# lgalke/aae-recommender

Measured on AMD Instinct MI355X. Metric: train docs/sec at |items|=100k h=200, higher is better.
Workload: dtype f32; 1 GPU; C3 PubMed-scale synthetic Bags: |items|=100000, hidden=200, code=50, fp32, batch=100 docs/GPU/step, full partial_fit (ae+disc+gen, 4 Adam) inside the AdversarialAutoEncoder.fit epoch loop (permutation batches of a corpus resident in HBM); n_items=100000, n_hidden=200, n_code=50, batch_per_gpu=100, global_batch=100, cond_inc=0, rng=device, parallelism=dp1

## Files before the change

### aae-recommender_amd/aaerec/_hip.py

```python
import ctypes as C
import itertools
import weakref
import os

import numpy as np
import torch

_HERE = os.path.dirname(os.path.abspath(__file__))
LIB_PATH = os.environ.get("AAE_HIP_LIB") or os.path.join(_HERE, "libaaerec_hip.so")

ABI_VERSION = 4
ACTIVATIONS = {"ReLU": 0, "SELU": 1, "Tanh": 2, "Sigmoid": 3, "ELU": 4, "LeakyReLU": 5,
               "Softplus": 6, "Hardtanh": 7, "ReLU6": 8, "CELU": 9, "Softsign": 10, "Hardsigmoid": 11, "LogSigmoid": 12,
               "Softshrink": 13, "Hardshrink": 14, "Identity": 15, "GELU": 16, "SiLU": 17, "Mish": 18, "Hardswish": 19}
FINALS = {"linear": 0, "softmax": 1, "sigmoid": 2}
OPTIMIZERS = {"adam": 0, "sgd": 1}
PRIORS = {"gauss": 0, "categorical": 1, "bernoulli": 2}
RNG_INJECT, RNG_DEVICE = 0, 1
RANK_K_MAX = 1024
COOC_TILE = 16384
SPGEMM_HASH_PRODUCTS = 4096
SPGEMM_STAGE = 512
SPTRANS_LDS = 4096
LOWRANK_DIMS_MAX = 4096
# ... 5 lines not shown
GRAD_FUSED, GRAD_EXPORT = 0, 1


class _NullCtx:
    def __enter__(self):
        return None

    def __exit__(self, *a):
        return False


_NULL_CTX = _NullCtx()

T_ENC_W1T, T_ENC_B1, T_ENC_W2, T_ENC_W3, T_DEC_V1, T_DEC_V2, T_DEC_V3, T_DISC_D1, T_DISC_D2, T_DISC_D3 = range(10)
T_ADAM_ENC, T_ADAM_GEN, T_ADAM_DEC, T_ADAM_DISC, T_GRAD = 16, 32, 48, 64, 80
T_ACT_Z, T_ACT_LOSSES, T_ACT_A1, T_ACT_DZC, T_ACT_DH2, T_ACT_DA2 = 96, 97, 98, 99, 100, 101
T_ACT_GA1 = 102
CAT_SUM, CAT_MEAN = 0, 1
CAT_SPARSE_ADAM, CAT_ADAM = 0, 1
O_ENC, O_DEC, O_GEN, O_DISC = 0, 1, 2, 3
MODEL_AAE, MODEL_AE, MODEL_VAE = 0, 1, 3
DTYPE_F32, DTYPE_BF16 = 0, 1


class AaeConfig(C.Structure):
    _fields_ = [("abi_version", C.c_int32), ("n_items", C.c_int32), ("n_hidden", C.c_int32),
                ("n_code", C.c_int32), ("cond_inc", C.c_int32), ("max_batch", C.c_int32),
                ("max_nnz", C.c_int32), ("activation", C.c_int32), ("enc_final", C.c_int32),
                ("optimizer", C.c_int32), ("normalize_inputs", C.c_int32), ("rng_mode", C.c_int32),
                ("prior", C.c_int32), ("grad_mode", C.c_int32), ("dropout1", C.c_float),
                ("dropout2", C.c_float), ("gen_lr", C.c_float), ("reg_lr", C.c_float),
                ("prior_scale", C.c_float), ("has_prior_scale", C.c_int32), ("seed", C.c_uint64),
                ("unfused_decoder", C.c_int32), ("dp_world", C.c_int32), ("model_kind", C.c_int32),
                ("dtype", C.c_int32), ("blocked_output", C.c_int32), ("dense_noise", C.c_int32),
                ("reserved", C.c_int32 * 2)]


class AaeBatch(C.Structure):
    _fields_ = [("indptr_dev", C.c_void_p), ("indices_dev", C.c_void_p), ("values_dev", C.c_void_p),
                ("rows_dev", C.c_void_p), ("row_start", C.c_int32), ("n_rows", C.c_int32),
                ("nnz_bound", C.c_int32), ("max_row_nnz", C.c_int32), ("generation", C.c_int64)]


class AaeRngInject(C.Structure):
    _fields_ = [("masks_dev", C.c_void_p * 12), ("z_real_dev", C.c_void_p)]


_COLL_AG = C.CFUNCTYPE(C.c_int, C.c_void_p, C.c_void_p, C.c_void_p, C.c_int64, C.c_void_p)
_COLL_AR = C.CFUNCTYPE(C.c_int, C.c_void_p, C.c_void_p, C.c_int64, C.c_void_p)


class AaeCollectives(C.Structure):
    _fields_ = [("ctx", C.c_void_p), ("all_gather", _COLL_AG), ("reduce_scatter", _COLL_AG), ("all_reduce", _COLL_AR),
                ("world", C.c_int32), ("rank", C.c_int32)]


class AaeTensor(C.Structure):
    _fields_ = [("byte_offset", C.c_size_t), ("rows", C.c_int64), ("cols", C.c_int64), ("ld", C.c_int64)]


class AaeCooc(C.Structure):
    _fields_ = [("indptr_dev", C.c_void_p), ("indices_dev", C.c_void_p), ("values_dev", C.c_void_p), ("n_rows", C.c_int32)]


class AaePopular(C.Structure):
    _fields_ = [("counts_dev", C.c_void_p), ("order_dev", C.c_void_p), ("pos_dev", C.c_void_p), ("n_items", C.c_int32)]


class AaeMetricSpec(C.Structure):
    _fields_ = [("kind", C.c_int32), ("k", C.c_int32)]


class AaeRankRows(C.Structure):
    _fields_ = [("indptr_dev", C.c_void_p), ("ranks_dev", C.c_void_p), ("n_rows", C.c_int32)]


class AaeLowRank(C.Structure):
    _fields_ = [("vt_dev", C.c_void_p), ("ld", C.c_int64), ("n_features", C.c_int32), ("dims", C.c_int32)]


_PROTOS = {
    "aae_abi_version": (C.c_int, []),
    "aae_set_option": (C.c_int, [C.c_char_p, C.c_char_p]),
    "aae_last_error": (C.c_char_p, []),
    "aae_arena_bytes": (C.c_int, [C.POINTER(AaeConfig), C.POINTER(C.c_size_t)]),
    "aae_create": (C.c_int, [C.POINTER(AaeConfig), C.c_void_p, C.c_size_t, C.c_void_p, C.POINTER(C.c_void_p)]),
    "aae_destroy": (C.c_int, [C.c_void_p]),
    "aae_tensor_info": (C.c_int, [C.c_void_p, C.c_int, C.POINTER(AaeTensor)]),
    "aae_set_lr": (C.c_int, [C.c_void_p, C.c_double, C.c_double]),
    "aae_params_changed": (C.c_int, [C.c_void_p]),
    "aae_set_rng_rows": (C.c_int, [C.c_void_p, C.c_int64, C.c_int64]),
    "aae_sync": (C.c_int, [C.c_void_p, C.c_void_p]),
    "aae_load_linear": (C.c_int, [C.c_void_p, C.c_int, C.c_int, C.c_void_p, C.c_void_p]),
    "aae_store_linear": (C.c_int, [C.c_void_p, C.c_int, C.c_int, C.c_void_p, C.c_void_p]),
    "aae_load_adam": (C.c_int, [C.c_void_p, C.c_int, C.c_int, C.c_void_p, C.c_void_p, C.c_void_p, C.c_void_p, C.c_int64]),
    "aae_store_adam": (C.c_int, [C.c_void_p, C.c_int, C.c_int, C.c_void_p, C.c_void_p, C.c_void_p, C.c_void_p, C.POINTER(C.c_int64)]),
    "aae_step": (C.c_int, [C.c_void_p, C.POINTER(AaeBatch), C.c_void_p, C.POINTER(AaeRngInject), C.c_void_p]),
    "aae_ae_encode": (C.c_int, [C.c_void_p, C.POINTER(AaeBatch), C.POINTER(AaeRngInject), C.c_void_p, C.c_void_p]),
    "aae_ae_decode_backward": (C.c_int, [C.c_void_p, C.c_void_p, C.c_int64, C.POINTER(AaeRngInject), C.c_void_p, C.c_void_p]),
    "aae_vae_step": (C.c_int, [C.c_void_p, C.POINTER(AaeBatch), C.c_void_p, C.c_void_p, C.c_void_p]),
    "aae_vae_predict": (C.c_int, [C.c_void_p, C.POINTER(AaeBatch), C.c_void_p, C.c_void_p, C.c_void_p, C.c_int64,
                                  C.c_void_p]),
    "aae_vae_encode": (C.c_int, [C.c_void_p, C.POINTER(AaeBatch), C.c_void_p, C.c_void_p, C.c_int32, C.c_void_p]),
    "aae_vae_decode_backward": (C.c_int, [C.c_void_p, C.c_void_p, C.c_int64, C.c_void_p, C.c_void_p]),
    "aae_vae_encoder_backward": (C.c_int, [C.c_void_p, C.c_void_p, C.c_int64, C.c_void_p]),
    "aae_decoder_step": (C.c_int, [C.c_void_p, C.POINTER(AaeBatch), C.c_void_p, C.c_int64, C.POINTER(AaeRngInject),
                                   C.c_void_p, C.c_void_p]),
    "aae_ae_encoder_backward": (C.c_int, [C.c_void_p, C.c_void_p, C.c_int64, C.c_void_p]),
    "aae_disc_gen": (C.c_int, [C.c_void_p, C.POINTER(AaeRngInject), C.c_void_p]),
    "aae_disc_step": (C.c_int, [C.c_void_p, C.POINTER(AaeRngInject), C.c_void_p]),
    "aae_gen_step": (C.c_int, [C.c_void_p, C.POINTER(AaeRngInject), C.c_void_p]),
    "aae_read_losses": (C.c_int, [C.c_void_p, C.POINTER(C.c_float * 3), C.c_void_p]),
    "aae_predict": (C.c_int, [C.c_void_p, C.POINTER(AaeBatch), C.c_void_p, C.c_void_p, C.c_int64, C.c_void_p]),
    "aae_predict_topk": (C.c_int, [C.c_void_p, C.POINTER(AaeBatch), C.c_void_p, C.c_int32, C.c_int32, C.c_void_p, C.c_void_p, C.c_void_p]),
    "aae_rank_max_rows": (C.c_int, [C.c_void_p, C.c_int32, C.POINTER(C.c_int32)]),
    "aae_rank_long_stats": (C.c_int, [C.c_void_p, C.POINTER(C.c_int64)]),
    "aae_predict_ranks": (C.c_int, [C.c_void_p, C.POINTER(AaeBatch), C.c_void_p, C.POINTER(AaeBatch), C.c_int32, C.c_void_p, C.c_void_p]),
    "aae_decode_ranks": (C.c_int, [C.c_void_p, C.c_void_p, C.c_int64, C.POINTER(AaeBatch), C.POINTER(AaeBatch), C.c_int32, C.c_void_p,
                                   C.c_void_p]),
    "aae_rank_full_max_rows": (C.c_int, [C.c_void_p, C.POINTER(C.c_int32)]),
    "aae_decode_topk": (C.c_int, [C.c_void_p, C.c_void_p, C.c_int64, C.POINTER(AaeBatch), C.c_int32, C.c_int32, C.c_void_p,
                                  C.c_void_p, C.c_void_p]),
    "aae_vae_predict_topk": (C.c_int, [C.c_void_p, C.POINTER(AaeBatch), C.c_void_p, C.c_void_p, C.c_int32, C.c_int32, C.c_void_p,
                                       C.c_void_p, C.c_void_p]),
    "aae_vae_predict_ranks": (C.c_int, [C.c_void_p, C.POINTER(AaeBatch), C.c_void_p, C.c_void_p, C.POINTER(AaeBatch), C.c_int32,
                                        C.c_void_p, C.c_void_p]),
    "aae_vae_decode_topk": (C.c_int, [C.c_void_p, C.c_void_p, C.c_int64, C.POINTER(AaeBatch), C.c_int32, C.c_int32, C.c_void_p,
                                      C.c_void_p, C.c_void_p]),
    "aae_vae_decode_ranks": (C.c_int, [C.c_void_p, C.c_void_p, C.c_int64, C.POINTER(AaeBatch), C.POINTER(AaeBatch), C.c_int32,
                                       C.c_void_p, C.c_void_p]),
    "aae_vae_rank_max_rows": (C.c_int, [C.c_void_p, C.c_int32, C.POINTER(C.c_int32)]),
    "aae_vae_rank_full_max_rows": (C.c_int, [C.c_void_p, C.POINTER(C.c_int32)]),
    "aae_encode": (C.c_int, [C.c_void_p, C.POINTER(AaeBatch), C.c_void_p, C.c_void_p]),
    "aae_decode": (C.c_int, [C.c_void_p, C.c_void_p, C.c_int64, C.c_int32, C.c_void_p, C.c_int64, C.c_void_p]),
    "aae_apply_updates": (C.c_int, [C.c_void_p, C.c_int, C.c_void_p]),
    "aae_apply_updates_except": (C.c_int, [C.c_void_p, C.c_int, C.c_int, C.c_void_p]),
    "aae_apply_shard": (C.c_int, [C.c_void_p, C.c_int, C.c_int64, C.c_int64, C.c_void_p, C.c_int, C.c_void_p]),
    "aae_w1_export": (C.c_int, [C.c_void_p, C.c_void_p, C.c_void_p, C.c_int32, C.c_void_p]),
    "aae_w1_packet_floats": (C.c_int, [C.c_void_p, C.c_int32, C.POINTER(C.c_int64), C.POINTER(C.c_int64)]),
    "aae_w1_import": (C.c_int, [C.c_void_p, C.c_void_p, C.c_void_p, C.c_int32, C.c_int32, C.c_int64, C.c_int, C.c_void_p]),
    "aae_set_grad_scale": (C.c_int, [C.c_void_p, C.c_float]),
    "aae_ae_forward": (C.c_int, [C.c_void_p, C.POINTER(AaeBatch), C.c_void_p, C.POINTER(AaeRngInject), C.c_void_p]),
    "aae_output_layer_step": (C.c_int, [C.c_void_p, C.POINTER(AaeBatch), C.c_void_p]),
    "aae_ae_backward": (C.c_int, [C.c_void_p, C.c_void_p, C.c_int64, C.c_void_p]),
    "aae_set_doc_l1": (C.c_int, [C.c_void_p, C.c_void_p]),
    "aae_set_first_layer_external": (C.c_int, [C.c_void_p, C.c_int]),
    "aae_first_layer_forward": (C.c_int, [C.c_void_p, C.POINTER(AaeBatch), C.c_void_p, C.c_void_p]),
    "aae_first_layer_update": (C.c_int, [C.c_void_p, C.c_void_p, C.c_int64, C.c_int32, C.c_int64, C.c_int, C.c_void_p]),
    "aae_apply_gathered": (C.c_int, [C.c_void_p, C.c_int, C.c_int, C.c_void_p, C.c_int64, C.c_int32, C.c_int64, C.c_void_p]),
    "aae_cat_encode": (C.c_int, [C.c_void_p, C.c_int32, C.c_int32, C.c_void_p, C.c_int32, C.c_int32, C.c_int32, C.c_void_p,
                                 C.c_int64, C.c_void_p]),
    "aae_cat_update": (C.c_int, [C.c_void_p, C.c_void_p, C.c_void_p, C.c_void_p, C.c_int32, C.c_int32, C.c_void_p, C.c_int32,
                                 C.c_int32, C.c_int32, C.c_void_p, C.c_int64, C.c_int32, C.c_double, C.c_int64, C.c_void_p]),
    "aae_csr_embed": (C.c_int, [C.c_void_p, C.c_void_p, C.c_void_p, C.c_int32, C.c_void_p, C.c_int32, C.c_int32, C.c_int64,
                                C.c_void_p, C.c_int64, C.c_void_p]),
    "aae_cooc_scores": (C.c_int, [C.POINTER(AaeCooc), C.c_int32, C.POINTER(AaeBatch), C.c_void_p, C.c_int64, C.c_void_p]),
    "aae_cooc_topk": (C.c_int, [C.POINTER(AaeCooc), C.c_int32, C.POINTER(AaeBatch), C.c_int32, C.c_int32, C.c_void_p, C.c_int64,
                                C.c_void_p, C.c_void_p, C.c_void_p]),
    "aae_cooc_ranks": (C.c_int, [C.POINTER(AaeCooc), C.c_int32, C.POINTER(AaeBatch), C.POINTER(AaeBatch), C.c_int32, C.c_void_p,
                                 C.c_int64, C.c_void_p, C.c_void_p]),
    "aae_cooc_scores_i32": (C.c_int, [C.POINTER(AaeCooc), C.c_int32, C.POINTER(AaeBatch), C.c_void_p, C.c_int64, C.c_void_p]),
    "aae_cooc_topk_i32": (C.c_int, [C.POINTER(AaeCooc), C.c_int32, C.POINTER(AaeBatch), C.c_int32, C.c_int32, C.c_void_p, C.c_int64,
                                    C.c_void_p, C.c_void_p, C.c_void_p]),
    "aae_cooc_ranks_i32": (C.c_int, [C.POINTER(AaeCooc), C.c_int32, C.POINTER(AaeBatch), C.POINTER(AaeBatch), C.c_int32, C.c_void_p,
                                     C.c_int64, C.c_void_p, C.c_void_p]),
    "aae_spgemm_i32_bound": (C.c_int, [C.POINTER(AaeCooc), C.POINTER(AaeCooc), C.c_int32, C.c_void_p, C.c_void_p]),
# ... 1149 lines not shown
                                             C.byref(inj) if inj else None, _ptr(dz), self._stream()))
        return dz

    def vae_step(self, csr, row_start, n_rows, rows=None, cond=None, eps=None):
        b = self._batch(csr, row_start, n_rows, rows)
        keep = []
        if cond is not None:
            cond = upload(cond, self.device, torch.float32).contiguous(); keep.append(cond)
        if eps is not None:
            eps = torch.as_tensor(eps, dtype=torch.float32).to(self.device).contiguous(); keep.append(eps)
        self._keep = keep
        with self._on_device():
            _check(self.lib.aae_vae_step(self.handle, C.byref(b), _ptr(cond), _ptr(eps), self._stream()))

    def vae_encode(self, csr, row_start, n_rows, rows=None, eps=None, train=True):
        b = self._batch(csr, row_start, n_rows, rows)
        if eps is not None:
            eps = torch.as_tensor(eps, dtype=torch.float32).to(self.device).contiguous()
        z = torch.empty(n_rows, self.c, dtype=torch.float32, device=self.device)
        self._keep = [eps, z]
        with self._on_device():
            _check(self.lib.aae_vae_encode(self.handle, C.byref(b), _ptr(eps), _ptr(z), int(bool(train)), self._stream()))
        return z

    def vae_decode_backward(self, zc):
        zc = zc.detach().to(self.device, torch.float32).contiguous()
        dzc = torch.empty_like(zc)
        self._keep = self._keep + [zc, dzc]
        with self._on_device():
            _check(self.lib.aae_vae_decode_backward(self.handle, _ptr(zc), zc.shape[1], _ptr(dzc), self._stream()))
        return dzc

    def vae_encoder_backward(self, dz):
        dz = dz.detach().to(self.device, torch.float32).contiguous()
        self._keep = self._keep + [dz]
        with self._on_device():
            _check(self.lib.aae_vae_encoder_backward(self.handle, _ptr(dz), dz.shape[1], self._stream()))

    def vae_predict(self, csr, row_start, n_rows, cond=None, eps=None):
        b = self._batch(csr, row_start, n_rows)
        out = self._out_buffer(n_rows)
        if cond is not None:
            cond = upload(cond, self.device, torch.float32).contiguous()
        if eps is not None:
            eps = torch.as_tensor(eps, dtype=torch.float32).to(self.device).contiguous()
        with self._on_device():
            _check(self.lib.aae_vae_predict(self.handle, C.byref(b), _ptr(cond), _ptr(eps), _ptr(out), out.shape[1],
                                            self._stream()))
        return out[:, :self.N]

    def ae_encoder_backward(self, dz):
        dz = dz.detach().to(self.device, torch.float32).contiguous()
        self._keep.append(dz)
        with self._on_device():
            _check(self.lib.aae_ae_encoder_backward(self.handle, _ptr(dz), dz.shape[1], self._stream()))

    def disc_gen(self):
        with self._on_device():
            _check(self.lib.aae_disc_gen(self.handle, None, self._stream()))

    def disc_step(self):
        with self._on_device():
            _check(self.lib.aae_disc_step(self.handle, None, self._stream()))

    def gen_step(self):
        with self._on_device():
            _check(self.lib.aae_gen_step(self.handle, None, self._stream()))

    def apply_updates(self, which, skip=-1):
        with self._on_device():
            _check(self.lib.aae_apply_updates_except(self.handle, which, skip, self._stream()))

    def apply_shard(self, tid, row_begin, row_end, grad_shard, which):
        self._keep.append(grad_shard)
        with self._on_device():
            _check(self.lib.aae_apply_shard(self.handle, tid, row_begin, row_end, C.c_void_p(grad_shard.data_ptr()),
                                            which, self._stream()))

    big_tensor_id = T_DEC_V3

    def big_grad(self):
        return T_DEC_V3, self.tensor(T_GRAD + T_DEC_V3, padded=True), self.tensor(T_DEC_V3, padded=True)

    def _w1_layout(self, cap):
        if self._w1_packet is None:
            hw, tot = C.c_int64(), C.c_int64()
            _check(self.lib.aae_w1_packet_floats(self.handle, self.w1_cap, C.byref(hw), C.byref(tot)))
            assert hw.value == self._w1_hdr
            self._w1_small = tot.value - hw.value - self.w1_cap * self.h
            self._w1_packet = torch.zeros(tot.value, dtype=torch.float32, device=self.device)
        cap = self.w1_cap if cap is None else max(1, min(int(cap), self.w1_cap))
        hdr = (1 + cap + 3) & ~3
        return cap, hdr, hdr + cap * self.h + self._w1_small

    def w1_export(self, cap=None):
        cap, hdr, total = self._w1_layout(cap)
        pk = self._w1_packet[:total]
        with self._on_device():
            _check(self.lib.aae_w1_export(self.handle, C.c_void_p(pk.data_ptr()), C.c_void_p(pk.data_ptr() + 4 * hdr), cap,
                                          self._stream()))
        return pk

    def w1_import(self, packets, n_peers, which, cap=None, stride_floats=None):
        cap, hdr, total = self._w1_layout(cap)
        stride = total if stride_floats is None else int(stride_floats)
        assert stride >= total and packets.numel() >= (n_peers - 1) * stride + total
        self._keep.append(packets)
        with self._on_device():
            _check(self.lib.aae_w1_import(self.handle, C.c_void_p(packets.data_ptr()),
                                          C.c_void_p(packets.data_ptr() + 4 * hdr), cap, n_peers, 4 * stride, which,
                                          self._stream()))

    def set_rng_rows(self, row_offset, global_rows):
        _check(self.lib.aae_set_rng_rows(self.handle, int(row_offset), int(global_rows)))

    def set_grad_scale(self, scale):
        _check(self.lib.aae_set_grad_scale(self.handle, float(scale)))

    def profile_enable(self, on=True, kernels=None):
        if on and kernels is not None:
            on = sum(1 << (k + 1) for k in kernels)
        _check(self.lib.aae_profile_enable(self.handle, int(on)))

    def profile_read(self, kernel_id):
        ms, n = C.c_double(), C.c_int64()
        _check(self.lib.aae_profile_read(self.handle, kernel_id, C.byref(ms), C.byref(n)))
        return ms.value, n.value

    def losses(self):
        out = (C.c_float * 3)()
        with self._on_device():
            _check(self.lib.aae_read_losses(self.handle, C.byref(out), self._stream()))
        return float(out[0]), float(out[1]), float(out[2])

    def _out_buffer(self, n_rows):
        ld = (self.N + 3) & ~3
        return torch.empty(n_rows, ld, dtype=torch.float32, device=self.device)

    def predict(self, csr, row_start, n_rows, cond=None):
        b = self._batch(csr, row_start, n_rows)
        out = self._out_buffer(n_rows)
        if cond is not None:
            cond = upload(cond, self.device, torch.float32).contiguous()
        with self._on_device():
            _check(self.lib.aae_predict(self.handle, C.byref(b), _ptr(cond), _ptr(out), out.shape[1], self._stream()))
        return out[:, :self.N]

    def rank_max_rows(self, k=10):
        return self._max_rows(int(k), self.lib.aae_rank_max_rows, int(k))

    def _max_rows(self, key, entry, *args):
        if key not in self._rank_rows:
            out = C.c_int32()
            _check(entry(self.handle, *args, C.byref(out)))
            self._rank_rows[key] = int(out.value)
        return self._rank_rows[key]

    def rank_long_stats(self):
        out = (C.c_int64 * 5)()
        _check(self.lib.aae_rank_long_stats(self.handle, out))
        return dict(zip(("calls", "rows", "overflow_rows", "entries", "max_entries"), (int(v) for v in out)))

    def predict_topk(self, csr, row_start, n_rows, k, cond=None, exclude_known=True):
        return self._topk(self.lib.aae_predict_topk, csr, row_start, n_rows, k, exclude_known, (self._cond_rows(cond),))

    def _cond_rows(self, cond):
# ... 93 lines not shown
```

### aae-recommender_amd/csrc/aae_abi.hip

```cpp
#include <hip/hip_runtime.h>
#include <hip/hip_ext.h>
#include <math.h>
#include <stdio.h>
#include <stdlib.h>
#include <string.h>

#include <algorithm>
#include <string>
#include <vector>

#include "../../include/aaerec_hip.h"
#include "gemm_f32.h"
#include "kernels.h"
#include "dec_fused.h"
#include "dec_fused_bf16.h"
#include "dec_crit_x3.h"
#include "rank_x3.h"
#include "rank_long.h"
#include "rank_full.h"
#include "cooc.h"
#include "spgemm.h"
#include "sptrans.h"
#include "mutinfo.h"
#include "popular.h"
#include "rank_metrics.h"
#include "lowrank.h"
#include "chain.h"
#include "chain4.h"
#include "chain16x3.h"
#include "cond_embed.h"
#include "w1_update.h"
#include "dae_corrupt.h"

using namespace aae;

#include "kernel_pick.h"

#include <map>
static std::map<std::string, std::string> g_options;
const char* option_value(const char* name) {
    auto it = g_options.find(name);
    if (it != g_options.end()) return it->second.c_str();
    return getenv((std::string("AAE_") + name).c_str());
}

#include "abi_model.h"
#include "abi_layers.h"
#include "abi_chains.h"
#include "abi_rank.h"

extern "C" {

int aae_abi_version(void) { return AAE_ABI_VERSION; }

int aae_set_option(const char* name, const char* value) {
    if (!name || !*name) return fail(AAE_EINVAL, "option name is empty");
    static const char* known[] = {"NO_CHAIN", "CHAIN16", "SPLIT_ANY", "BLOCKED_ANY", "EARLY_ANY", "NO_LATE_JOIN", "NO_ITEM_COUNT", "W1_SERIAL",
                                  "NO_RANK_FUSED", "CHAIN_KSLICES", "X16_ROWS", "DW_KSPLIT_ROWS", "DEC_TS", "CHAIN_TS", "DW_TS", "DEC_SKIP", "CHAIN_SKIP", "RANK_SKIP",
                                  "RANK_COLLECT_CAP"};
    bool ok = false;
    for (const char* k : known) ok = ok || strcmp(k, name) == 0;
    if (!ok) return fail(AAE_EINVAL, "unknown option (aae_options, csrc/abi_model.h, lists them)");
    if (value && strcmp(name, "RANK_COLLECT_CAP") == 0) {
        char* end = nullptr;
        const long v = strtol(value, &end, 10);
        if (end == value || *end || v < 1 || v > kLongCap) return fail(AAE_EINVAL, "RANK_COLLECT_CAP must be a whole number in [1, 4096]");
    }
    if (value) g_options[name] = value; else g_options.erase(name);
    return AAE_OK;
}
const char* aae_last_error(void) { return g_err.c_str(); }

int aae_arena_bytes(const aae_config* cfg, size_t* bytes_out) {
    TRY(validate(cfg));
    if (!bytes_out) return fail(AAE_EINVAL, "bytes_out is NULL");
    aae_model tmp; memset((void*)&tmp, 0, sizeof(tmp)); tmp.cfg = *cfg;
    read_options(tmp.opt);
    *bytes_out = layout(&tmp, nullptr, true);
    return AAE_OK;
}

int aae_create(const aae_config* cfg, void* arena_dev, size_t arena_bytes, void* stream, aae_handle* out) {
    TRY(validate(cfg));
    if (!arena_dev || !out) return fail(AAE_EINVAL, "arena/out is NULL");
    if (reinterpret_cast<uintptr_t>(arena_dev) & 255) return fail(AAE_EINVAL, "arena must be 256-byte aligned");
    aae_model* m = new aae_model();
    memset((void*)m, 0, sizeof(*m));
    m->cfg = *cfg;
    read_options(m->opt);
    size_t need = layout(m, static_cast<char*>(arena_dev), false);
    if (need > arena_bytes) { delete m; return fail(AAE_ENOMEM, "arena smaller than aae_arena_bytes()"); }
    m->base = static_cast<char*>(arena_dev); m->bytes = need;
    m->alpha_mode = cfg->activation == AAE_ACT_SELU;
    m->vae = cfg->model_kind == 3; m->vae_bwd = false; m->vae_cut = false;
    m->bf16 = cfg->dtype == 1;
    m->blocked_ok = cfg->blocked_output == 1;
    m->blocked_any = m->opt.blocked_any;
    m->split_any = m->opt.split_any;
    m->x3_gemm = !m->bf16;
    m->noise_next = nullptr; m->noise_ld = 0; m->dense_step = false; m->noise_gen_next = false; m->noise_gen_scale = 0.f;
    m->ae_only = cfg->model_kind == 1 || m->vae;
    m->lazy = true;
    auto limit = [](bool& ok, size_t bytes) { return [&ok, bytes](auto kernel) { ok = ok && raise_lds_limit(kernel, bytes); }; };
    const int maxlds = 160 * 1024;
    {
        int dev = 0, cus = 0;
        if (hipGetDevice(&dev) != hipSuccess ||
            hipDeviceGetAttribute(&cus, hipDeviceAttributeMultiprocessorCount, dev) != hipSuccess || cus < 1) {
            delete m; return fail(AAE_EHIP, "no HIP device");
        }
        m->n_cu = std::min(cus, 304);
        const int nb = (m->h + 1 + 15) / 16;
        m->fused_nb = nb <= 4 ? 4 : nb <= 7 ? 7 : nb <= 13 ? 13 : 0;
        m->fused_ok = m->fused_nb != 0 && fused_width_ok(m->h, m->ldh);
        m->use_chain = (m->h + 1 <= 208) && (m->c + 1 <= 208) && (m->cp + 1 <= (cfg->model_kind == 3 ? 208 : 2 * 208)) &&
                       !m->opt.no_chain;
        const size_t chain_lds = kCSlots * kCR * kCL * sizeof(float);
        if (m->use_chain) each_chain(false, limit(m->use_chain, chain_lds));
        m->act_nm = cfg->activation > AAE_ACT_LEAKYRELU;
        if (m->use_chain && m->act_nm) each_chain(true, limit(m->use_chain, chain_lds));
        m->use_chain4 = m->use_chain && !m->act_nm && !m->opt.chain16;
        if (m->use_chain4) each_chain4(limit(m->use_chain4, chain_lds));
        if (m->use_chain && m->cp + 1 > 208 && !m->use_chain4) m->use_chain = false;
        m->x16_rows = m->opt.x16_rows;
        m->dw_ksplit_rows = 256;
        if (m->opt.dw_ksplit_rows >= 0) m->dw_ksplit_rows = m->opt.dw_ksplit_rows;
        if (!m->opt.no_item_count) {
            void* hp = nullptr; void* dp = nullptr;
            if (hipHostMalloc(&hp, 64, hipHostMallocMapped) == hipSuccess && hipHostGetDevicePointer(&dp, hp, 0) == hipSuccess) {
                m->cnt_host = static_cast<int*>(hp); m->cnt_host_dev = static_cast<int*>(dp); *m->cnt_host = 0;
            } else { if (hp) (void)hipHostFree(hp); (void)hipGetLastError(); }
        }
        m->x16_ok = m->use_chain4 && m->FXi[P_W2] != nullptr;
        if (m->x16_ok) each_chain16x3(limit(m->x16_ok, kX16Lds));
        m->force_unfused = cfg->unfused_decoder == 1;
        if (m->fused_ok) {
            each_dec_fused(kDecFused, limit(m->fused_ok, maxlds));
            if (m->bf16) each_dec_fused_bf16(kDecFused, limit(m->fused_ok, maxlds));
            if (!raise_lds_limit(tile_bucket_kernel, maxlds - 2048)) m->fused_ok = false;
            m->bucket_wide_ok = raise_lds_limit(tile_bucket_wide_kernel, maxlds - 16384);
            {
                hipFuncAttributes fa;
                static bool told = false;
                if (m->bucket_wide_ok && !told && hipFuncGetAttributes(&fa, reinterpret_cast<const void*>(tile_bucket_wide_kernel)) == hipSuccess && fa.numRegs < 121) {
                    told = true;
                    fprintf(stderr, "aaerec: tile_bucket_wide_kernel allocates %d vector registers, not the 128 it claims to keep its CU to itself (buckets.h)\n", fa.numRegs);
                }
                (void)hipGetLastError();
            }
        }
    }
    m->late_enabled = !m->opt.no_late_join;
    m->early_enabled = true;
    m->early_any = m->opt.early_any;
    m->rank_ok = m->fused_ok && m->use_chain4 && !m->vae && !m->opt.no_rank_fused;
    m->vae_rank_ok = m->vae && m->fused_ok && m->use_chain4 && !m->opt.no_rank_fused;
    if (m->vae_rank_ok) each_chain4_vae(limit(m->vae_rank_ok, kCSlots * kCR * kCL * sizeof(float)));
    bool& rank_ok = m->vae ? m->vae_rank_ok : m->rank_ok;
    if (rank_ok) each_rank_x3([&](RankKernel k, int nb) { rank_ok = rank_ok && raise_lds_limit(k, rank_x3_lds_bytes(nb)); });
    if (rank_ok) each_rank_x3v2([&](RankKernel k, int nb) { rank_ok = rank_ok && raise_lds_limit(k, rank_x3v2_lds_bytes(nb)); });
    m->w1_big_lds = raise_lds_limit(w1_item_update_kernel, sizeof(int) * w1_items_lds_words(16384));
    (void)hipGetLastError();
    m->grad_scale = 1.f;
    m->rng_row0 = 0; m->rng_global = 0;
    m->Gt = m->G.p;
    m->split_ok = false; m->opt_pending = false; m->side = nullptr; m->ev_crit = m->ev_opt = nullptr;
    m->split_wgs = std::max(1, (m->n_cu * 5) / 8);
    m->pf_armed = m->pf_built = m->pf_pending = false; m->pf_step = -1; m->hstep = 0; m->flushed_hstep = -1; m->ev_head = m->ev_pf = nullptr;
    bool side_ok = false;
    if (cfg->grad_mode == AAE_GRAD_FUSED) {
        int lo = 0, hi = 0;
        const unsigned evflags = hipEventDisableTiming | hipEventDisableSystemFence;
        side_ok = hipDeviceGetStreamPriorityRange(&lo, &hi) == hipSuccess &&
                  hipStreamCreateWithPriority(&m->side, hipStreamNonBlocking, lo) == hipSuccess &&
                  hipEventCreateWithFlags(&m->ev_crit, evflags) == hipSuccess &&
                  hipEventCreateWithFlags(&m->ev_opt, evflags) == hipSuccess &&
                  hipEventCreateWithFlags(&m->ev_head, evflags) == hipSuccess &&
                  hipEventCreateWithFlags(&m->ev_pf, evflags) == hipSuccess &&
                  hipEventCreateWithFlags(&m->ev_bk, evflags) == hipSuccess &&
                  hipEventCreateWithFlags(&m->ev_end, evflags) == hipSuccess;
        if (!side_ok) {
            if (m->side) (void)hipStreamDestroy(m->side);
            m->side = nullptr;
        }
        (void)hipGetLastError();
    }
    if (side_ok && m->fused_ok && m->bf16 && m->split_wgs > 0 &&
        (size_t)((m->N + kBU - 1) / kBU) * kBU * bf_stride(4) <= (size_t)m->R * m->ldn) {
        m->split_ok = true;
        for (int mode : {kDecCrit, kDecOpt}) each_dec_fused_bf16(mode, limit(m->split_ok, maxlds));
        (void)hipGetLastError();
    }
    if (side_ok && m->fused_ok && m->split_wgs > 0 && 
        (size_t)((m->N + kTI - 1) / kTI) * kTI * (size_t)std::min(m->R, 16 * kMB) * sizeof(float) < (size_t)0x7FFFFFF0u) {
        bool ok = true;
        for (int mode : {kDecCrit, kDecOpt, kDecOptAcc}) each_dec_fused(mode, limit(ok, maxlds));
        each_dec_opt_blocks(limit(ok, maxlds));
        if (!m->bf16) m->split_ok = ok;
        m->x3_ok = ok;
        each_dec_crit_x3(false, limit(m->x3_ok, maxlds));
        each_dec_opt_blocks_x3(limit(m->x3_ok, maxlds));
        each_dec_opt_x3(false, limit(m->x3_ok, maxlds));
        (void)hipGetLastError();
        if (m->bf16) {
            m->bf16_x3 = m->x3_ok && ok;
            if (!m->bf16_x3) m->x3_ok = false;
            else m->split_ok = true;
            m->bf16_one = m->bf16_x3;
            each_dec_crit_x3(true, limit(m->bf16_one, maxlds));
            each_dec_opt_x3(true, limit(m->bf16_one, maxlds));
            (void)hipGetLastError();
        }
        if (m->x3_ok) {
            const int ntiles = (m->N + 31) / 32;
            const double t_tile = (2.2 + 0.0096 * m->h) * (m->bf16_one ? 0.98 : 1.0);
            int w = (int)(ntiles * t_tile / (m->bf16_one ? 127.0 : 57.0) / 8.0 + 0.5) * 8;
            w = std::max(w, std::min(ntiles, m->bf16_one ? 40 : 64));
            const int cap = m->late_enabled ? m->n_cu * 7 / 16 : m->n_cu * 9 / 16;
            m->split_wgs = std::max(1, std::min(w, cap));
        }
    }
    hipStream_t s = S(stream);
    hipError_t e = hipMemsetAsync(arena_dev, 0, need, s);
    if (e != hipSuccess) { delete m; return fail(AAE_EHIP, std::string("hipMemsetAsync: ") + hipGetErrorString(e)); }
    struct { Ten* t; int col; } ones[] = {{&m->eh1, m->h}, {&m->eh2, m->h}, {&m->zc, m->cp}, {&m->dh1, m->h},
                                           {&m->dh2, m->h}, {&m->zin, m->c}, {&m->xh1, m->h}, {&m->xh2, m->h}};
    for (auto& o : ones)
        hipLaunchKernelGGL(fill_col_kernel, dim3(((int)o.t->rows + 255) / 256), dim3(256), 0, s, o.t->p, (int)o.t->ld,
                           (int)o.t->rows, o.col, 1.0f);
    OptScalars hs[4]; memset(hs, 0, sizeof(hs));
    for (int i = 0; i < 4; ++i) {
        hs[i].t = 0; hs[i].is_sgd = cfg->optimizer == AAE_OPT_SGD;
        hs[i].lr = (i == O_ENC || i == O_DEC) ? (double)cfg->gen_lr : (double)cfg->reg_lr;
        hs[i].neg_step_size = 0.f; hs[i].bc2_sqrt = 1.f; hs[i].inv_bc2_sqrt = 1.f;
    }
    e = hipMemcpyAsync(m->sc, hs, sizeof(hs), hipMemcpyHostToDevice, s);
    if (e == hipSuccess) e = hipStreamSynchronize(s);
    if (e != hipSuccess) { delete m; return fail(AAE_EHIP, std::string("init: ") + hipGetErrorString(e)); }
    *out = m;
    return AAE_OK;
}

#ifdef W1_TS
int aae_debug_w1_ts(unsigned long long* out, int n) {
    return (int)hipMemcpyFromSymbol(out, HIP_SYMBOL(aae::w1_ts), sizeof(unsigned long long) * (size_t)n);
}
#endif
int aae_destroy(aae_handle h) {
    if (!h) return AAE_OK;
    if (h->side) {
        (void)hipStreamSynchronize(h->side);
        (void)hipStreamDestroy(h->side);
    }
    if (h->dp_scratch) (void)hipFree(h->dp_scratch);
    if (h->cnt_host) (void)hipHostFree(h->cnt_host);
    for (hipEvent_t e : {h->ev_crit, h->ev_opt, h->ev_head, h->ev_pf, h->ev_bk, h->ev_end}) if (e) (void)hipEventDestroy(e);
    if (h->prof_ev) {
        for (int k = 0; k < AAE_K_N; ++k)
            for (auto& pr : h->prof_ev[k]) { (void)hipEventDestroy(pr.first); (void)hipEventDestroy(pr.second); }
        delete[] h->prof_ev;
    }
    delete h;
    return AAE_OK;
}


int aae_profile_enable(aae_handle h, int on) {
    if (!h) return fail(AAE_EINVAL, "handle is NULL");
    if (on && !h->prof_ev) h->prof_ev = new std::vector<std::pair<hipEvent_t, hipEvent_t>>[AAE_K_N];
    h->prof_on = on != 0;
    h->prof_mask = on == 1 ? ~0u : ((unsigned)on >> 1);
    return AAE_OK;
}

int aae_profile_read(aae_handle h, int kernel_id, double* total_ms, int64_t* launches) {
    if (!h || !total_ms || !launches) return fail(AAE_EINVAL, "NULL argument");
    if (kernel_id < 0 || kernel_id >= AAE_K_N) return fail(AAE_EINVAL, "bad kernel id");
    *total_ms = 0.0; *launches = 0;
    if (!h->prof_ev) return AAE_OK;
    auto& v = h->prof_ev[kernel_id];
    for (size_t i = 0; i < h->prof_used[kernel_id]; ++i) {
        HIPCHK(hipEventSynchronize(v[i].second));
        float ms = 0.f;
        HIPCHK(hipEventElapsedTime(&ms, v[i].first, v[i].second));
        *total_ms += ms; *launches += 1;
    }
    h->prof_used[kernel_id] = 0;
    return AAE_OK;
}

int aae_prefetch_batch(aae_handle h, const aae_batch* next) {
    if (!h || !next) return fail(AAE_EINVAL, "NULL argument");
    if (!next->indptr_dev || !next->indices_dev || !next->values_dev) return fail(AAE_EINVAL, "batch pointers are NULL");
    if (next->n_rows < 1 || next->n_rows > h->R) return fail(AAE_EINVAL, "batch n_rows outside [1, max_batch]");
    if (next->nnz_bound > h->cfg.max_nnz) return fail(AAE_EINVAL, "batch nnz_bound > max_nnz");
    if (next->generation == 0) { h->pf_armed = false; return AAE_OK; }
    h->pf_batch = *next;
    h->pf_armed = true;
    return AAE_OK;
}

int aae_set_input_noise(aae_handle h, const float* noise_dev, int64_t noise_ld) {
    if (!h) return fail(AAE_EINVAL, "handle is NULL");
    if (!h->Xn.p) return fail(AAE_ESTATE, "aae_set_input_noise: the model was not created with cfg.dense_noise = 1");
    if (noise_dev && noise_ld < h->N) return fail(AAE_EINVAL, "noise_ld < n_items");
    h->noise_next = noise_dev; h->noise_ld = noise_ld;
    h->noise_gen_next = false;
    return AAE_OK;
}

int aae_join_output_layer(aae_handle h, void* stream) {
    if (!h) return fail(AAE_EINVAL, "handle is NULL");
    if (h->opt_pending) {
        HIPCHK(hipStreamWaitEvent(S(stream), h->ev_opt, 0));
        h->opt_pending = false;
        if (!h->pf_after_opt) h->pf_pending = false;
    }
    return AAE_OK;
}

int aae_join(aae_handle h, void* stream) {
    if (!h) return fail(AAE_EINVAL, "handle is NULL");
    return join_deferred(h, S(stream));
}

int aae_set_split(aae_handle h, int32_t workgroups) {
    if (!h) return fail(AAE_EINVAL, "handle is NULL");
    if (workgroups < 0) return fail(AAE_EINVAL, "workgroups must be >= 0");
    if (h->opt_pending) return fail(AAE_ESTATE, "aae_set_split with a deferred launch pending: call aae_join / aae_sync first");
    h->split_wgs = workgroups;
// ... 90 lines not shown
```

### aae-recommender_amd/csrc/abi_chains.h

```cpp
#pragma once

namespace {

ChainOp cop(int kind, int src, int dst, int N) {
    ChainOp o; memset(&o, 0, sizeof(o));
    o.kind = kind; o.src = src; o.dst = dst; o.N = N; o.one_col = -1; o.scale = 1.f; o.yslot = 0; o.fake_slot = -1;
    return o;
}
ChainOp cop_load(const float* g, int ld, int dst, int N, int row0 = 0) {
    ChainOp o = cop(COP_LOAD, 0, dst, N); o.W = g; o.ldw = ld; o.out_row0 = row0; return o;
}
ChainOp cop_linear(int kind, int src, int dst, const Ten& W, int K, int N, int epi) {
    ChainOp o = cop(kind, src, dst, N); o.W = W.p; o.ldw = (int)W.ld; o.K = K; o.epi = epi;
    if (kind == COP_LINEAR_DX) { o.Wkn = W.p; o.ldkn = (int)W.ld; }
    return o;
}
void cop_out(ChainOp& o, float* out, int ld, int row0 = 0) { o.out = out; o.ldo = ld; o.out_row0 = row0; }

W4Copies w4_of(const aae_model* m, int pid) {
    return W4Copies{m->PT[pid].p, m->D4[pid].p, (int)m->P[pid].rows, (int)m->P[pid].cols, m->FXi[pid], m->DXi[pid], m->FXBi[pid], kCWide};
}
float* ga1_ptr(const aae_model* m) {
    return (m->ext_first && m->ga1x.p) ? m->ga1x.p + (size_t)(m->R - m->rows) * m->ldh : m->gb3.p;
}
// ... 281 lines not shown
            } else
            if (!no_wave && m->rows > 16 * kMB && m->hot_list && (int64_t)m->N >= 40ll * m->rows) {
                w.wave_form = 1;
                w.nitem = (w.nitem + 3) / 4;
                const int set = m->hot_flip; m->hot_flip ^= 1;
                w.hot = m->hot_list + (size_t)set * m->hot_cap; w.hot_count = m->hot_count + set; w.hot_zero = m->hot_count + (set ^ 1);
                m->w1_hot_pending = true; m->w1_hot_set = set; m->w1_hot_which = which; m->w1_hot_ga1 = ga1;
                mh = m;
            }
            w.cnt_out = nullptr;
            constexpr bool hyb_count = true;
            if ((w.wave_form != 2 || hyb_count) && m->cnt_host) {
                w.cnt_out = m->cnt_host_dev;
                const int seen = *reinterpret_cast<volatile int*>(m->cnt_host);
                if (seen > 0) {
                    const int per = w.wave_form ? 4 : 1;
                    int want = ((seen + seen / 4 + per - 1) / per + 63) & ~63;
                    if (w.wave_form == 2) want = std::max(want, (int)((std::min<int64_t>(m->cfg.max_nnz, m->N) + 2047) / 2048));
                    w.nitem = std::min(w.nitem, std::max(256, want));
                }
            }
        }
        return AAE_OK;
    }
    void add_loss(aae_model* m, int n, int slot) { g.loss.enabled = 1; g.loss.terms = m->adv_terms; g.loss.n = n; g.loss.out = m->losses + slot; }
    int launch(hipStream_t s, hipEvent_t done = nullptr, bool* marked = nullptr) {
        int blocks = tiles;
        if (g.w1.enabled) { g.w1.blk0 = tiles; blocks += g.w1.ncol + g.w1.nitem; }
        if (g.loss.enabled) blocks += 1;
        if (marked) *marked = done && !mh;
        g.ksplit = ksplit_rows;
        const int ts_from = dw_ts;
        static int ts_seen = 0;
        static unsigned long long* ts_dev = nullptr;
        constexpr int kTsCap = 1 << 16;
        const bool ts_now = ts_from >= 0 && ts_seen >= ts_from && ts_seen < ts_from + 6;
        if (ts_from >= 0) {
            ++ts_seen;
            if (!ts_dev) HIPCHK(hipMalloc(&ts_dev, sizeof(unsigned long long) * 2 * kTsCap));
        }
        if (ts_now) { HIPCHK(hipMemsetAsync(ts_dev, 0, sizeof(unsigned long long) * 2 * kTsCap, s)); g.ts = ts_dev; g.ts_cap = kTsCap; }
        if (done && !mh) hipExtLaunchKernelGGL(grouped_dw_kernel, dim3(blocks), dim3(256), 0, s, nullptr, done, 0, g);
        else
        hipLaunchKernelGGL(grouped_dw_kernel, dim3(blocks), dim3(256), 0, s, g);
        LAUNCHCHK("grouped_dw_kernel");
        if (ts_now) {
            HIPCHK(hipStreamSynchronize(s));
            const int nb = std::min(blocks, kTsCap);
            std::vector<unsigned long long> h(2 * (size_t)nb);
            HIPCHK(hipMemcpy(h.data(), ts_dev, sizeof(unsigned long long) * 2 * nb, hipMemcpyDeviceToHost));
            unsigned long long t_lo = ~0ull, t_hi = 0;
            for (int b = 0; b < nb; ++b) if (h[2 * b]) { t_lo = std::min(t_lo, h[2 * b]); t_hi = std::max(t_hi, h[2 * b + 1]); }
            const int ncol = g.w1.enabled ? g.w1.ncol : 0, nitem = g.w1.enabled ? g.w1.nitem : 0;
            int max_rows = 0;
            for (int q = 0; q < g.njobs; ++q) max_rows = std::max(max_rows, g.jobs[q].rows);
            fprintf(stderr, "[grouped_dw launch %d: %d workgroups = %d tiles (rows %d) + %d column-sum + %d item (form %d) + %d loss; first start -> last end %.2f us]\n",
                    ts_seen - 1, blocks, tiles, max_rows, ncol, nitem, g.w1.wave_form, g.loss.enabled, (t_hi - t_lo) * 0.01);
            const struct { const char* name; int lo, hi; } kinds[] = {{"tiles", 0, tiles}, {"column sums", tiles, tiles + ncol}, {"items", tiles + ncol, tiles + ncol + nitem}};
            for (const auto& k : kinds) {
                if (k.hi <= k.lo) continue;
                unsigned long long first = ~0ull, last = 0, worst = 0; int worst_b = -1, busy = 0; double sum = 0;
                for (int b = k.lo; b < std::min(k.hi, nb); ++b) {
                    if (!h[2 * b]) continue;
                    const unsigned long long d = h[2 * b + 1] - h[2 * b];
                    first = std::min(first, h[2 * b]); last = std::max(last, h[2 * b + 1]);
                    if (d > worst) { worst = d; worst_b = b - k.lo; }
                    if (d > 150) ++busy;
                    sum += d * 0.01;
                }
                fprintf(stderr, "   %-12s start %.2f us after the launch's first, end %.2f; longest workgroup %.2f us (#%d); %d of %d ran longer than 1.5 us, mean %.2f us\n",
                        k.name, (first - t_lo) * 0.01, (last - t_lo) * 0.01, worst * 0.01, worst_b, busy, k.hi - k.lo, sum / std::max(1, k.hi - k.lo));
            }
        }
        if (mh) TRY(launch_w1_hot(mh, s));
        return AAE_OK;
    }
};

int launch_w1_hot(aae_model* m, hipStream_t s) {
    if (!m->w1_hot_pending) return AAE_OK;
    m->w1_hot_pending = false;
    W1Items a = w1_items_args(m, m->w1_hot_ga1, 0, 0, m->w1_hot_which);
    a.ulist = m->hot_list + (size_t)m->w1_hot_set * m->hot_cap; a.ucount = m->hot_count + m->w1_hot_set;
    const size_t lds = sizeof(int) * w1_items_lds_words(m->rows);
    hipLaunchKernelGGL(w1_item_update_kernel, dim3(std::min(m->hot_cap, 256)), dim3(256), lds, s, a);
    LAUNCHCHK("w1_item_update (hot list)");
    return AAE_OK;
}

void chain_encoder_tail(aae_model* m, ChainBuilder& cb, bool train, const uint8_t* mk2, uint32_t sid2, int rows,
                        float* eh2_out, hipStream_t s, const uint8_t* mk1 = nullptr, uint32_t sid1 = 0) {
    const int h = m->h;
    if (m->ext_first) {
        cb.add(cop_load(m->a1.p, m->ldh, 3, h));
        ChainOp& e1 = cb.add(cop(COP_DROPACT, 3, 0, h));
        e1.d = make_drop(m, 0, train, mk1, nullptr, rows, h, sid1); e1.one_col = h; cop_out(e1, m->eh1.p, m->ldh);
    } else {
        ChainOp& l = cb.add(cop_load(m->eh1.p, m->ldh, 0, h)); l.one_col = h;
    }
    ChainOp& a = cb.add(cop_fwd(m, P_W2, 0, 1, h + 1, h, CEPI_DROPACT, s));
    a.d = make_drop(m, 1, train, mk2, nullptr, rows, h, sid2); a.one_col = h;
    if (eh2_out) cop_out(a, eh2_out, m->ldh);
    cb.add(cop_fwd(m, P_W3, 1, 2, h + 1, m->c, CEPI_NONE, s));
}

static int row_blocks(const aae_model* m) { return m->rows <= 16 * kMB ? 1 : (m->rows + kRowBlock - 1) / kRowBlock; }
static size_t fused_span_limit(const aae_model* m) {
    const int bits = out_bf16(m) ? 31 : 32;
    return ((size_t)1 << bits) - ((size_t)1 << 24);
}
static bool fused_decoder_applies(const aae_model* m) {
    const bool one = m->rows <= 16 * kMB;
    const bool bf_blocks_ok = !m->bf16 || (m->x3_ok && m->dh2f.p && true);
    const bool blocked = !one && m->blocked_ok && !out_bf16(m) && bf_blocks_ok && m->split_ok && m->split_wgs > 0 && m->Gacc.p && row_blocks(m) <= kMaxRowBlocks &&
                         m->cfg.grad_mode == AAE_GRAD_FUSED &&
                         (m->blocked_any || (size_t)m->rows * m->N <= ((size_t)32 << 20) || (m->x3_ok && m->dh2f.p));
    return m->fused_ok && !m->force_unfused && (one || blocked) &&
           ((size_t)m->N + 2 * kTI) * m->ldh * sizeof(float) < fused_span_limit(m) &&
           ((size_t)m->N + 2 * kTI) * (size_t)((m->rows + row_blocks(m) - 1) / row_blocks(m)) * sizeof(float) < ((size_t)1 << 31) &&
           (m->bf16 ? dec_fused_bf16_lds_bytes(m->fused_nb) : dec_fused_lds_bytes((m->rows + row_blocks(m) - 1) / row_blocks(m), m->h)) <= 160 * 1024;
}
static void flip_bucket_set(aae_model* m) {
    std::swap(m->tstart, m->tstart2); std::swap(m->teb, m->teb2); std::swap(m->ten, m->ten2); std::swap(m->tev, m->tev2);
}
int build_tile_buckets(aae_model* m, hipStream_t s) {
    const int ntiles = (m->N + kTI - 1) / kTI, B = m->rows;
    flip_bucket_set(m);
    const size_t lds1 = sizeof(int) * ((size_t)ntiles + 1 + kBucketMaxDocs + 1 + 1024);
    if (ntiles <= kBucketMaxTiles && B <= kBucketMaxDocs && (m->fused_ok || lds1 <= 48 * 1024)) {
        hipLaunchKernelGGL(tile_bucket_kernel, dim3(1), dim3(1024), lds1, s, m->bv, ntiles, m->tstart, m->teb, m->ten, m->tev);
    } else if (ntiles <= kBucketMaxTiles && B <= kBucketWideDocs && m->bucket_wide_ok) {
        size_t lds = sizeof(int) * ((size_t)ntiles + 1 + kBucketWideDocs + 1 + 1024);
        constexpr bool bk_claim = true;
        if (bk_claim) lds = std::max(lds, (size_t)(160 * 1024 - 16384));
        hipLaunchKernelGGL(tile_bucket_wide_kernel, dim3(1), dim3(1024), lds, s, m->bv, ntiles, m->tstart, m->teb, m->ten, m->tev);
    } else {
        const int gy = std::max(1, std::min(16, m->chunks / 16 + 1));
        hipLaunchKernelGGL(zero_int_kernel, dim3(std::min(64, ntiles / 256 + 1)), dim3(256), 0, s, m->tcount, ntiles + 1);
        hipLaunchKernelGGL(tile_hist_kernel, dim3(B, gy), dim3(256), 0, s, m->bv, m->tcount);
        hipLaunchKernelGGL(tile_scan_kernel, dim3(1), dim3(1024), 0, s, m->tcount, m->tstart, ntiles);
        hipLaunchKernelGGL(tile_fill_kernel, dim3(B, gy), dim3(256), 0, s, m->bv, m->tstart, m->tcount, m->teb, m->ten, m->tev);
    }
    LAUNCHCHK("tile buckets");
    m->buckets_valid = true;
    return AAE_OK;
}
int ensure_buckets(aae_model* m, hipStream_t s) {
    if (m->bk_pending) {
        HIPCHK(hipStreamWaitEvent(s, m->ev_bk, 0));
        m->bk_pending = false;
    }
    if (!m->buckets_valid) TRY(build_tile_buckets(m, s));
    return AAE_OK;
}

W1Items w1_items_args(aae_model* m, const float* ga1, int rpb, size_t bstride, int which) {
    const int set = (which == O_GEN) ? 1 : 0;
    W1Items a;
    a.ulist = m->ulist; a.ucount = m->ucount;
    a.tstart = m->tstart; a.eb = m->teb; a.en = m->ten; a.ev = m->tev;
    a.ga1 = ga1; a.ld = m->ldh; a.rpb = rpb; a.bstride = bstride;
    a.rscale = m->rscale; a.rows = m->rows; a.h = m->h;
    a.W = m->P[P_W1T].p; a.M = m->M[set][P_W1T].p; a.V = m->V[set][P_W1T].p; a.ldw = m->ldw1;
    a.gout = m->cfg.grad_mode == AAE_GRAD_EXPORT ? m->Gr[P_W1T].p : nullptr;
    a.sc = m->sc + which; a.tsync = m->tsync; a.step_ctr = m->step_ctr;
    a.mark_synced = (which == O_GEN || m->ae_only) ? 1 : 0;
    return a;
}
int launch_w1_items(aae_model* m, const float* ga1, int rpb, size_t bstride, int which, hipStream_t s) {
    TRY(ensure_buckets(m, s));
    const W1Items a = w1_items_args(m, ga1, rpb, bstride, which);
    const size_t lds = sizeof(int) * w1_items_lds_words(m->rows);
    if (lds > 64 * 1024 && !m->w1_big_lds) return fail(AAE_ESTATE, "first-layer update: batch too large for the LDS row lists");
    ProfScope ps(m, AAE_K_ENC_W1_ADAM, s);
    const int items = std::max(1, std::min(std::min(m->cfg.max_nnz, std::max(256, m->rows * 32)), m->N));
    hipLaunchKernelGGL(w1_item_update_kernel, dim3(items), dim3(256), lds, s, a);
    LAUNCHCHK("w1_item_update");
    return AAE_OK;
}

static void piggyback_buckets(aae_model* m, ChainBuilder& cb) {
    const int ntiles = (m->N + kTI - 1) / kTI;
    const size_t need = sizeof(int) * ((size_t)ntiles + 1 + kBucketMaxDocs + 1 + 1024);
    if (m->x16_ok && m->rows >= m->x16_rows) return;
    if (m->buckets_valid || !fused_decoder_applies(m) || ntiles > kBucketMaxTiles || m->rows > kBucketMaxDocs ||
        need > (size_t)kCSlots * kCR * kCL * sizeof(float))
        return;
    flip_bucket_set(m);
    BucketJob& b = cb.P.bk;
    b.bv = m->bv; b.ntiles = ntiles; b.tstart = m->tstart; b.eb = m->teb; b.en = m->ten; b.ev = m->tev; b.enabled = 1;
    m->buckets_valid = true;
}

int chain_ae_forward(aae_model* m, bool with_dec, const float* cond_dev, float* z_out, hipStream_t s) {
    const int B = m->rows, h = m->h, c = m->c, cp = m->cp;
    const aae_rng_inject& I = m->inj;
    ChainBuilder cb(m, B);
    piggyback_buckets(m, cb);
    chain_encoder_tail(m, cb, true, I.masks_dev[1], 1, B, m->eh2.p, s, I.masks_dev[0], 0);
    ChainOp& f = m->cfg.enc_final == AAE_FINAL_LINEAR ? cb.P.ops[cb.P.nops - 1] : cb.add(cop(COP_FINAL_FWD, 2, 2, c));
    f.aux = m->cfg.enc_final;
    cop_out(f, m->zc.p, m->ldc); f.out2 = m->zsave.p; f.ldo2 = m->ldz;
    if (z_out) { ChainOp& st = cb.add(cop(COP_STORE, 2, 2, c)); cop_out(st, z_out, c); }
    if (with_dec) {
        if (wide_dec_in(m)) {
            const int nA = kCWide - c, ci = m->cfg.cond_inc;
            ChainOp& ca = cb.add(cop_load(cond_dev, ci, 2, nA)); ca.dst_col0 = c;
            ChainOp& cl = cb.add(cop_load(cond_dev + nA, ci, 5, ci - nA)); cl.one_col = cp - kCWide;
        } else if (m->cfg.cond_inc > 0) {
            ChainOp& cl = cb.add(cop_load(cond_dev, m->cfg.cond_inc, 2, m->cfg.cond_inc)); cl.dst_col0 = c; cl.one_col = cp;
        } else {
            f.one_col = cp;
        }
        ChainOp& v1 = add_dec_in_fwd(cb, m, 2, 5, 3, s);
        v1.d = make_drop(m, 0, true, I.masks_dev[2], nullptr, B, h, 2); v1.one_col = h; cop_out(v1, m->dh1.p, m->ldh);
        ChainOp& v2 = cb.add(cop_fwd(m, P_V2, 3, 4, h + 1, h, CEPI_DROPACT, s));
        v2.d = make_drop(m, 1, true, I.masks_dev[3], nullptr, B, h, 3); v2.one_col = h; cop_out(v2, m->dh2.p, m->ldh);
    }
    m->dec_hidden_done = with_dec;
    return launch_chain(m, cb, s);
}

int chain_dec_hidden(aae_model* m, bool train, int rows, hipStream_t s) {
    const int h = m->h, cp = m->cp;
    const aae_rng_inject& I = m->inj;
    ChainBuilder cb(m, rows);
    if (wide_dec_in(m)) {
        cb.add(cop_load(m->zc.p, m->ldc, 0, kCWide));
        ChainOp& lb = cb.add(cop_load(m->zc.p + kCWide, m->ldc, 3, cp - kCWide)); lb.one_col = cp - kCWide;
    } else {
        ChainOp& l = cb.add(cop_load(m->zc.p, m->ldc, 0, cp)); l.one_col = cp;
    }
    ChainOp& v1 = add_dec_in_fwd(cb, m, 0, 3, 1, s);
    v1.d = make_drop(m, 0, train, I.masks_dev[2], nullptr, rows, h, 2); v1.one_col = h; cop_out(v1, m->dh1.p, m->ldh);
    ChainOp& v2 = cb.add(cop_fwd(m, P_V2, 1, 2, h + 1, h, CEPI_DROPACT, s));
    v2.d = make_drop(m, 1, train, I.masks_dev[3], nullptr, rows, h, 3); v2.one_col = h; cop_out(v2, m->dh2.p, m->ldh);
    return launch_chain(m, cb, s);
}

int chain_ae_backward(aae_model* m, bool dec_part, bool enc_part, const float* part_slabs, size_t slab_stride,
                      const float* gz_ext, int ld_gz, float* dzc_out, int which, hipStream_t s, int nslab = 16) {
    const int B = m->rows, h = m->h, c = m->c, cp = m->cp;
    const aae_rng_inject& I = m->inj;
    ChainBuilder cb(m, B);
    if (dec_part) {
        if (part_slabs) {
            ChainOp& ss = cb.add(cop(COP_SLABSUM, 0, 2, h)); ss.W = part_slabs; ss.ldw = m->ldh; ss.aux = nslab; ss.stride = slab_stride;
            ss.epi = CEPI_ACTBWD; ss.aux_ptr = m->dh2.p; ss.aux_ld = m->ldh;
            ss.d = make_drop(m, 1, true, I.masks_dev[3], nullptr, B, h, 3); cop_out(ss, m->gb0.p, m->ldh);
        } else {
            cb.add(cop_load(m->gb0.p, m->ldh, 2, h));
        }
        if (y_needs_load(m)) cb.add(cop_load(m->dh1.p, m->ldh, 3, h));
        ChainOp& x2 = cb.add(cop_dx(m, P_V2, 2, 4, h, h, CEPI_ACTBWD, s)); set_y(cb, m, x2, m->dh1.p, m->ldh, 3);
        x2.d = make_drop(m, 0, true, I.masks_dev[2], nullptr, B, h, 2); cop_out(x2, m->gb1.p, m->ldh);
        add_dec_in_dx(cb, m, 4, 5, 3, dzc_out, s);
    }
    if (enc_part) {
        if (!dec_part || gz_ext) cb.add(cop_load(gz_ext ? gz_ext : m->gzc.p, gz_ext ? ld_gz : m->ldc, 5, c));
        int sg = 7;
        ChainOp* prod = (dec_part && !gz_ext && cb.P.nops) ? &cb.P.ops[cb.P.nops - 1] : nullptr;
        if (m->cfg.enc_final == AAE_FINAL_LINEAR && prod && cp == c && !prod->out2) {
            prod->out2 = m->ga3.p; prod->ldo2 = m->ldz; sg = 5;
        } else {
            if (m->cfg.enc_final != AAE_FINAL_LINEAR) cb.add(cop_load(m->zsave.p, m->ldz, 6, c));
            ChainOp& fb = cb.add(cop(COP_FINAL_BWD, 5, 7, c)); fb.yslot = 6; fb.aux = m->cfg.enc_final;
            cop_out(fb, m->ga3.p, m->ldz);
        }
        if (y_needs_load(m)) cb.add(cop_load(m->eh2.p, m->ldh, 8, h));
        ChainOp& x3 = cb.add(cop_dx(m, P_W3, sg, 9, c, h, CEPI_ACTBWD, s)); set_y(cb, m, x3, m->eh2.p, m->ldh, 8);
        x3.d = make_drop(m, 1, true, I.masks_dev[which == O_GEN ? 9 : 1], nullptr, B, h, which == O_GEN ? 9 : 1);
        cop_out(x3, m->gb2.p, m->ldh);
        if (y_needs_load(m)) cb.add(cop_load(m->eh1.p, m->ldh, 0, h));
        ChainOp& x2 = cb.add(cop_dx(m, P_W2, 9, 1, h, h, CEPI_ACTBWD, s)); set_y(cb, m, x2, m->eh1.p, m->ldh, 0);
// ... 287 lines not shown
```

### aae-recommender_amd/csrc/abi_model.h

```cpp
#pragma once

static thread_local std::string g_err;
static int fail(int code, const std::string& msg) { g_err = msg; return code; }

#define HIPCHK(expr)                                                                        \
    do {                                                                                    \
        hipError_t e_ = (expr);                                                             \
        if (e_ != hipSuccess)                                                               \
            return fail(AAE_EHIP, std::string(#expr) + ": " + hipGetErrorString(e_));       \
    } while (0)
#define LAUNCHCHK(what)                                                                     \
    do {                                                                                    \
        hipError_t e_ = hipGetLastError();                                                  \
        if (e_ != hipSuccess) return fail(AAE_EHIP, std::string(what) + ": " + hipGetErrorString(e_)); \
    } while (0)
#define TRY(expr) do { int rc_ = (expr); if (rc_ != AAE_OK) return rc_; } while (0)

namespace {

inline int r4(int x) { return (x + 3) & ~3; }

struct Ten {
    float* p = nullptr; size_t off = 0; int64_t rows = 0, cols = 0, ld = 0;
    size_t floats() const { return (size_t)rows * ld; }
};

enum { P_W1T = 0, P_B1, P_W2, P_W3, P_V1, P_V2, P_V3, P_D1, P_D2, P_D3, NP };
enum { O_ENC = 0, O_DEC = 1, O_GEN = 2, O_DISC = 3 };

}

struct aae_options {
    bool no_chain;
    bool chain16;
    bool split_any;
    bool blocked_any;
    bool early_any;
    bool no_late_join;
    bool no_item_count;
    bool w1_serial;
    bool no_rank_fused;
    bool chain_kslices;
    int x16_rows;
    int rank_collect_cap;
    int dw_ksplit_rows;
    char dec_ts[8];
    bool chain_ts;
    int dw_ts;
    int dec_skip, chain_skip, rank_skip;
};
const char* option_value(const char* name);
inline void read_options(aae_options& o) {
    auto on = [](const char* n) { return option_value(n) != nullptr; };
    auto num = [](const char* n, int dflt) { const char* e = option_value(n); return e ? atoi(e) : dflt; };
    o.no_chain = on("NO_CHAIN"); o.chain16 = on("CHAIN16"); o.split_any = on("SPLIT_ANY"); o.blocked_any = on("BLOCKED_ANY");
    o.early_any = on("EARLY_ANY"); o.no_late_join = on("NO_LATE_JOIN"); o.no_item_count = on("NO_ITEM_COUNT");
    o.w1_serial = on("W1_SERIAL"); o.no_rank_fused = on("NO_RANK_FUSED"); o.chain_kslices = on("CHAIN_KSLICES");
    o.x16_rows = num("X16_ROWS", 1024); o.dw_ksplit_rows = num("DW_KSPLIT_ROWS", -1);
    o.rank_collect_cap = std::max(0, std::min(num("RANK_COLLECT_CAP", 0), 4096));
    const char* ts = option_value("DEC_TS");
    snprintf(o.dec_ts, sizeof(o.dec_ts), "%s", ts ? ts : "");
    o.chain_ts = on("CHAIN_TS"); o.dw_ts = num("DW_TS", -1);
    o.dec_skip = num("DEC_SKIP", 0); o.chain_skip = num("CHAIN_SKIP", 0); o.rank_skip = num("RANK_SKIP", 0);
}

struct aae_model {
    aae_config cfg;
    aae_options opt;
    char* base; size_t bytes;
    int N, h, c, cp, R, R2;
    int ldh, ldw1, ldc, ldz, ldn;
    bool alpha_mode;
    float grad_scale;
    int rng_row0, rng_global;
    Ten P[NP], M[2][NP], V[2][NP], Gr[NP];
    unsigned short* FXi[NP]; unsigned short* DXi[NP]; unsigned short* FXBi[NP];
    bool x16_ok; int x16_rows;
    Ten PT[NP]; Ten D4[NP]; bool pt_ok[NP];
    Ten a1, eh1, eh2, zc, dh1, dh2, G, slabs, gb0, gb1, gb2, gb3, gzc, ga3, zin, xh1, xh2, dout, zsave, da2;
    Ten ga1x;
    bool only_output_layer;
    const float* doc_l1;
    bool ext_first;
    bool own_first;
    bool ae_only;
    bool vae;
    bool bf16;
    bool vae_bwd;
    bool vae_cut;
    Ten mulv, gmulv, veps;
    bool use_chain;
    bool use_chain4;
    bool act_nm;
    bool dec_hidden_done;
    bool fuse_enc_bwd;
    bool enc_bwd_done;
    int max_slabs;
    float* bce_partials; int bce_partials_cap;
    float* fix_partials;
    float* rscale;
    bool w1_merged;
    bool w1_items_merged;
    bool buckets_valid;
    bool lazy;
    int n_cu; bool fused_ok; int fused_nb; bool force_unfused;
    int* tcount; int* tstart; int* teb; int* ten; float* tev;
    int* tstart2; int* teb2; int* ten2; float* tev2;
    int* tsync; int* mark; int* ulist; int* ucount; int* stamp; LazyTab* tab;
    int* hot_list = nullptr; int* hot_count = nullptr; int hot_cap = 0, hot_flip = 0;
    bool w1_hot_pending = false; int w1_hot_set = 0, w1_hot_which = 0; const float* w1_hot_ga1 = nullptr;
    int* pslot; int* ptag;
    int chunks;
    float* losses;
    float* adv_terms;
    OptScalars* sc;
    long long* step_ctr;
    BatchView bv; bool have_batch; int rows; int phase;
    aae_rng_inject inj;
    bool prof_on; unsigned prof_mask;
    std::vector<std::pair<hipEvent_t, hipEvent_t>>* prof_ev;
    size_t prof_used[AAE_K_N];
    bool split_ok; int split_wgs; bool opt_pending;
    hipStream_t side; hipEvent_t ev_crit, ev_opt;
    bool bf16_one = false;
    bool bf16_x3 = false;
    float* Gt;
    Ten Xn; const float* noise_next; int64_t noise_ld; bool dense_step;
    bool noise_gen_next; float noise_gen_scale;
    float* noise_l1;
    bool bucket_wide_ok = false;
    bool split_any = false;
    float* dp_scratch = nullptr; size_t dp_scratch_floats = 0;
    bool x3_gemm = false;
    bool x3_ok = false;
    bool w1_big_lds = false;
    bool blocked_any = false;
    Ten dh2f;
    bool blocked_ok; Ten Gacc;
    int* mark2; int* ulist2; int* ucount2; int* stamp2;
    int* cnt_host; int* cnt_host_dev;
    int dw_ksplit_rows;
    aae_batch pf_batch, pf_built_batch; bool pf_armed; bool pf_built; long long pf_step; long long hstep;
    bool pf_pending; hipEvent_t ev_head, ev_pf;
    bool pf_bumped = false;
    bool pf_after_opt = false;
    hipEvent_t ev_bk = nullptr; bool bk_pending = false;
    bool last_out_split = false;
    Ten dh2s; OptScalars* sc_snap = nullptr;
    bool late_enabled = false, late_ok = false;
    hipEvent_t ev_end = nullptr; bool end_marked = false, spec_tab_ok = false, pf_this_step = false, early_enabled = false, early_any = false;
    long long flushed_hstep = -1;
    int64_t long_stats[5] = {0, 0, 0, 0, 0};
    bool rank_ok = false;
    bool vae_rank_ok = false;
    bool side_ordered = false;
};

namespace {

struct Arena {
    char* base; size_t off = 0; bool dry;
    float* take(size_t nfloats, size_t* off_out) {
        off = (off + 255) & ~(size_t)255;
        size_t o = off; off += nfloats * sizeof(float);
        if (off_out) *off_out = o;
        return dry ? nullptr : reinterpret_cast<float*>(base + o);
    }
    Ten mat(int64_t rows, int64_t cols, int64_t ld, int64_t pad_rows = 0) {
        Ten t; t.rows = rows; t.cols = cols; t.ld = ld;
        t.p = take((size_t)(rows + pad_rows) * ld, &t.off);
        return t;
    }
};

constexpr int kRowBlock = 104, kMaxRowBlocks = 16;

inline bool fused_width_ok(int h, int ldh) {
    return (h + 1 + 15) / 16 <= 13 && ldh <= 256 && (ldh % 4) == 0 && ldh <= kSD - 2;
}

int validate(const aae_config* c) {
    if (!c) return fail(AAE_EINVAL, "cfg is NULL");
    if (c->abi_version != AAE_ABI_VERSION) return fail(AAE_EINVAL, "abi_version mismatch");
    if (c->n_items < 1 || c->n_hidden < 1 || c->n_code < 1 || c->cond_inc < 0)
        return fail(AAE_EINVAL, "n_items/n_hidden/n_code must be positive");
    if (c->n_hidden > 4096) return fail(AAE_EINVAL, "n_hidden > 4096 not supported");
    if (c->max_batch < 1 || c->max_nnz < 1) return fail(AAE_EINVAL, "max_batch/max_nnz must be positive");
    if (c->max_batch > 16384) return fail(AAE_EINVAL, "max_batch > 16384 not supported");
    if (c->activation < 0 || c->activation >= AAE_ACT_COUNT) return fail(AAE_EINVAL, "unknown activation");
    if (c->enc_final < 0 || c->enc_final > AAE_FINAL_SIGMOID) return fail(AAE_EINVAL, "unknown enc_final");
// ... 55 lines not shown
        {
            const int64_t M = m->P[pid].rows, Nc = m->P[pid].cols;
            m->PT[pid] = a.mat((Nc + 3) / 4, 4 * M, 4 * M, kW4Pad);
            m->D4[pid] = a.mat((M + 3) / 4, 4 * Nc, 4 * Nc, kW4Pad);
        }
    for (int i = 0; i < NP; ++i) m->FXi[i] = m->DXi[i] = m->FXBi[i] = nullptr;
    if (chain_copies && m->R2 >= m->opt.x16_rows)
        for (int pid : {P_W2, P_W3, P_V1, P_V2, P_D1, P_D2}) {
            const int64_t M = m->P[pid].rows, Nc = m->P[pid].cols, Mp = (M + 15) & ~15, Np = (Nc + 15) & ~15;
            m->FXi[pid] = reinterpret_cast<unsigned short*>(a.take((size_t)(((Nc + 31) / 32) * 3 * Mp * 32 + 1) / 2, nullptr));
            m->DXi[pid] = reinterpret_cast<unsigned short*>(a.take((size_t)(((M + 31) / 32) * 3 * Np * 32 + 1) / 2, nullptr));
            if (Nc > kCWide) m->FXBi[pid] = reinterpret_cast<unsigned short*>(a.take((size_t)(((Nc - kCWide + 31) / 32) * 3 * Mp * 32 + 1) / 2, nullptr));
        }
    const int R = m->R, R2 = m->R2;
    m->a1 = a.mat(R, h, m->ldh);   m->eh1 = a.mat(R, h + 1, m->ldh);  m->eh2 = a.mat(R, h + 1, m->ldh);
    m->zc = a.mat(R, cp + 1, m->ldc);
    m->dh1 = a.mat(R, h + 1, m->ldh); m->dh2 = a.mat(R, h + 1, m->ldh);
    m->G = a.mat(R, N, m->ldn, (32 * (int64_t)R + m->ldn - 1) / m->ldn + 1 + (c.blocked_output ? kMaxRowBlocks : 0));
    {
        int tiles = ((R + 63) / 64) * ((h + 63) / 64);
        m->max_slabs = std::max(1, std::min(128, 2048 / tiles));
        int64_t slab_rows = (int64_t)m->max_slabs * R;
        if (fused_width_ok(h, m->ldh)) slab_rows = std::max(slab_rows, (int64_t)(304 + 16) * std::min(R, 16 * kMB));
        if (fused_width_ok(h, m->ldh) && c.blocked_output && R <= kMaxRowBlocks * kRowBlock) slab_rows = std::max(slab_rows, (int64_t)(304 + 16) * R);
        m->slabs = a.mat(slab_rows, h, m->ldh);
    }
    m->gb0 = a.mat(R2, h + 1, m->ldh); m->gb1 = a.mat(R2, h + 1, m->ldh);
    m->gb2 = a.mat(R2, h + 1, m->ldh); m->gb3 = a.mat(R2, h + 1, m->ldh);
    m->gzc = a.mat(R, cp + 1, m->ldc);
    m->ga3 = a.mat(R2, cc + 1, m->ldz);
    m->zin = a.mat(R2, cc + 1, m->ldz);
    m->xh1 = a.mat(R2, h + 1, m->ldh); m->xh2 = a.mat(R2, h + 1, m->ldh);
    m->dout = a.mat(R2, 1, 4);
    m->zsave = a.mat(R, cc, m->ldz);
    m->da2 = a.mat(R, h + 1, m->ldh);
    m->Xn = Ten();
    if (c.dense_noise == 1) m->Xn = a.mat(R, N, m->ldn);
    m->noise_l1 = c.dense_noise == 1 ? a.take((size_t)R * kDaeChunksMax, nullptr) : nullptr;
    m->Gacc = Ten();
    if (c.blocked_output && c.grad_mode == AAE_GRAD_FUSED && R > 16 * kMB) m->Gacc = a.mat(N, h + 1, m->ldh, 2 * kTI);
    m->dh2f = Ten();
    if (c.blocked_output && c.grad_mode == AAE_GRAD_FUSED && R > 16 * kMB && R <= kMaxRowBlocks * kRowBlock)
        m->dh2f = a.mat((int64_t)((R + kXCH - 1) / kXCH) * 13 * (kXCH / 32) * 3, 256, 256);
    if (c.model_kind == 3) {
        m->mulv = a.mat(R, 2 * cc, r4(2 * cc)); m->gmulv = a.mat(R, 2 * cc, r4(2 * cc)); m->veps = a.mat(R, cc, r4(cc));
    }
    m->bce_partials_cap = std::max(512 * (c.blocked_output ? kMaxRowBlocks : 1), ((N + 31) / 32) * ((R + 31) / 32));
    m->bce_partials = a.take(m->bce_partials_cap, nullptr);
    m->fix_partials = a.take((size_t)R * 64, nullptr);
    m->rscale = a.take(R, nullptr);
    m->tsync = reinterpret_cast<int*>(a.take(N, nullptr));
    m->mark = reinterpret_cast<int*>(a.take(N, nullptr));
    m->ulist = reinterpret_cast<int*>(a.take((size_t)c.max_nnz * (size_t)std::max(1, c.dp_world), nullptr));
    m->pslot = m->ptag = nullptr;
    if (c.grad_mode == AAE_GRAD_EXPORT && c.dp_world > 1) {
        m->pslot = reinterpret_cast<int*>(a.take((size_t)N * c.dp_world, nullptr));
        m->ptag = reinterpret_cast<int*>(a.take((size_t)N * c.dp_world, nullptr));
    }
    m->ucount = reinterpret_cast<int*>(a.take(4, nullptr));
    m->stamp = m->ucount ? m->ucount + 1 : nullptr;
    m->hot_cap = (int)std::max<int64_t>(256, c.max_nnz / kW1WaveRows + 64);
    m->hot_list = reinterpret_cast<int*>(a.take((size_t)2 * m->hot_cap, nullptr));
    m->hot_count = reinterpret_cast<int*>(a.take(4, nullptr));
    m->hot_flip = 0;
    m->mark2 = m->ulist2 = m->ucount2 = m->stamp2 = nullptr;
    if (c.grad_mode == AAE_GRAD_FUSED) {
        m->mark2 = reinterpret_cast<int*>(a.take(N, nullptr));
        m->ulist2 = reinterpret_cast<int*>(a.take((size_t)c.max_nnz, nullptr));
        m->ucount2 = reinterpret_cast<int*>(a.take(4, nullptr));
        m->stamp2 = m->ucount2 ? m->ucount2 + 1 : nullptr;
    }
    m->tab = reinterpret_cast<LazyTab*>(a.take((size_t)kLazyTabCap * 4, nullptr));
    {
        const size_t nt = (size_t)(N + kTI - 1) / kTI + 1;
        m->tcount = reinterpret_cast<int*>(a.take(nt, nullptr));
        m->tstart = reinterpret_cast<int*>(a.take(nt, nullptr));
        m->teb = reinterpret_cast<int*>(a.take((size_t)c.max_nnz, nullptr));
        m->ten = reinterpret_cast<int*>(a.take((size_t)c.max_nnz, nullptr));
        m->tev = a.take((size_t)c.max_nnz, nullptr);
        m->tstart2 = reinterpret_cast<int*>(a.take(nt, nullptr));
        m->teb2 = reinterpret_cast<int*>(a.take((size_t)c.max_nnz, nullptr));
        m->ten2 = reinterpret_cast<int*>(a.take((size_t)c.max_nnz, nullptr));
        m->tev2 = a.take((size_t)c.max_nnz, nullptr);
    }
    m->losses = a.take(4, nullptr);
    m->adv_terms = a.take((size_t)R2, nullptr);
    m->sc = reinterpret_cast<OptScalars*>(a.take(4 * sizeof(OptScalars) / sizeof(float), nullptr));
    m->step_ctr = reinterpret_cast<long long*>(a.take(2, nullptr));
    m->dh2s = Ten(); m->sc_snap = nullptr;
    if (c.grad_mode == AAE_GRAD_FUSED) {
        m->dh2s = a.mat(std::min(R, 16 * kMB), h + 1, m->ldh);
        m->sc_snap = reinterpret_cast<OptScalars*>(a.take((sizeof(OptScalars) + 3) / sizeof(float), nullptr));
    }
    return (a.off + 255) & ~(size_t)255;
}

inline hipStream_t S(void* s) { return reinterpret_cast<hipStream_t>(s); }

struct ProfScope {
    aae_model* m; int k; hipStream_t s; bool on;
    ProfScope(aae_model* m_, int k_, hipStream_t s_) : m(m_), k(k_), s(s_), on(m_->prof_on && ((m_->prof_mask >> k_) & 1)) {
        if (!on) return;
        auto& v = m->prof_ev[k];
        if (m->prof_used[k] == v.size()) {
            hipEvent_t a, b;
            if (hipEventCreate(&a) != hipSuccess || hipEventCreate(&b) != hipSuccess) { on = false; return; }
            v.emplace_back(a, b);
        }
        (void)hipEventRecord(v[m->prof_used[k]].first, s);
    }
    ~ProfScope() {
        if (!on) return;
        (void)hipEventRecord(m->prof_ev[k][m->prof_used[k]].second, s);
        m->prof_used[k]++;
    }
};

bool prof_pair(aae_model* m, int k, hipEvent_t* a, hipEvent_t* b) {
    if (!(m->prof_on && ((m->prof_mask >> k) & 1))) return false;
    auto& v = m->prof_ev[k];
    if (m->prof_used[k] == v.size()) {
        hipEvent_t x, y;
        if (hipEventCreate(&x) != hipSuccess || hipEventCreate(&y) != hipSuccess) return false;
        v.emplace_back(x, y);
    }
    *a = v[m->prof_used[k]].first; *b = v[m->prof_used[k]].second;
    m->prof_used[k]++;
    return true;
}

static inline bool out_bf16(const aae_model* m) { return m->bf16 && !m->bf16_x3; }

int join_deferred(aae_model* m, hipStream_t s) {
    if (m->opt_pending) HIPCHK(hipStreamWaitEvent(s, m->ev_opt, 0));
    if (m->pf_pending && (!m->opt_pending || m->pf_after_opt)) HIPCHK(hipStreamWaitEvent(s, m->ev_pf, 0));
    m->opt_pending = m->pf_pending = m->late_ok = false;
    return AAE_OK;
}

int join_step_open(aae_model* m, hipStream_t s) {
    if (!(m->opt_pending && m->late_ok && !m->pf_after_opt)) return join_deferred(m, s);
    if (m->pf_pending) { HIPCHK(hipStreamWaitEvent(s, m->ev_pf, 0)); m->pf_pending = false; }
    return AAE_OK;
}

int join_output_layer(aae_model* m, hipStream_t s) {
    if (!m->opt_pending) return AAE_OK;
    HIPCHK(hipStreamWaitEvent(s, m->ev_opt, 0));
    m->opt_pending = m->late_ok = false;
    return AAE_OK;
}
int side_done(aae_model* m, hipEvent_t ev) {
    HIPCHK(hipEventRecord(ev, m->side));
    return AAE_OK;
}
int join_host(aae_model* m) {
    if (!m->opt_pending && !m->pf_pending) return AAE_OK;
    HIPCHK(hipStreamSynchronize(m->side));
    m->opt_pending = m->pf_pending = m->late_ok = false;
    return AAE_OK;
}

DropSpec make_drop(const aae_model* m, int layer, bool train, const uint8_t* ma, const uint8_t* mb, int split,
                   int width, uint32_t stream_id) {
    DropSpec d; memset(&d, 0, sizeof(d));
    float p = layer == 0 ? m->cfg.dropout1 : m->cfg.dropout2;
// ... 27 lines not shown
```

### aae-recommender_amd/csrc/buckets.h

```cpp
#pragma once
#include "device_common.h"
#include "kernels.h"

namespace aae {

constexpr int kTI = 32;
constexpr int kMB = 7;

constexpr int kBucketMaxDocs = 16 * kMB;
constexpr int kBucketMaxTiles = 32 * 1024;

constexpr int kBucketWideDocs = 1024;
template <int MAXD = kBucketMaxDocs, int NT = 1024>
__device__ __forceinline__ void tile_bucket_body(const BatchView& bv, int ntiles, int* __restrict__ tstart,
                                                 int* __restrict__ eb, int* __restrict__ en, float* __restrict__ ev,
                                                 int* bk_lds) {
    int* cnt = bk_lds;
    int* dbeg = cnt + ntiles + 1;
    int* part = dbeg + MAXD + 1;
    __shared__ long long dlo[MAXD];
    const int t = threadIdx.x, docs = bv.n_rows;
    for (int i = t; i <= ntiles; i += NT) cnt[i] = 0;
    int len = 0;
    if (t < docs) {
        const int dc = bv.doc(t);
        const long long lo = bv.indptr[dc];
        dlo[t] = lo;
        len = (int)(bv.indptr[dc + 1] - lo);
    }
    part[t] = len;
    __syncthreads();
    for (int o = 1; o < MAXD; o <<= 1) {
        const int v = (t >= o && t < MAXD) ? part[t - o] : 0;
        __syncthreads();
        if (t < MAXD) part[t] += v;
        __syncthreads();
    }
    if (t < docs) dbeg[t] = part[t] - len;
    if (t == 0) dbeg[docs] = part[MAXD - 1];
    __syncthreads();
    const int total = dbeg[docs];
    auto doc_of = [&](int f) {
        int lo = 0, hi = docs - 1;
        while (lo < hi) { const int mid = (lo + hi + 1) >> 1; if (dbeg[mid] <= f) lo = mid; else hi = mid - 1; }
        return lo;
    };
    constexpr int U = MAXD > 16 * kMB ? 8 : 2;
    for (int f0 = t; f0 < total; f0 += NT * U) {
        int idx[U];
#pragma unroll
        for (int u = 0; u < U; ++u) {
            const int f = min(f0 + u * NT, total - 1);
            const int d = doc_of(f);
            idx[u] = bv.indices[dlo[d] + (f - dbeg[d])];
        }
#pragma unroll
        for (int u = 0; u < U; ++u)
            if (f0 + u * NT < total) atomicAdd(&cnt[idx[u] / kTI], 1);
    }
    __syncthreads();
    const int per = (ntiles + NT - 1) / NT;
    const int lo = min(t * per, ntiles), hi = min(ntiles, lo + per);
    int sum = 0;
    for (int i = lo; i < hi; ++i) sum += cnt[i];
    part[t] = sum;
    __syncthreads();
    for (int o = 1; o < NT; o <<= 1) {
        const int v = t >= o ? part[t - o] : 0;
        __syncthreads();
        part[t] += v;
        __syncthreads();
    }
    int run = part[t] - sum;
    for (int i = lo; i < hi; ++i) {
        const int c = cnt[i];
        tstart[i] = run;
        cnt[i] = run;
        run += c;
    }
    if (t == NT - 1) tstart[ntiles] = part[NT - 1];
    __syncthreads();
    for (int f0 = t; f0 < total; f0 += NT * U) {
        int idx[U], dd[U];
        float val[U];
#pragma unroll
        for (int u = 0; u < U; ++u) {
            const int f = min(f0 + u * NT, total - 1);
            const int d = doc_of(f);
            const long long e = dlo[d] + (f - dbeg[d]);
            dd[u] = d; idx[u] = bv.indices[e]; val[u] = bv.values[e];
        }
#pragma unroll
        for (int u = 0; u < U; ++u)
            if (f0 + u * NT < total) {
                const int tile = idx[u] / kTI;
                const int pos = atomicAdd(&cnt[tile], 1);
                eb[pos] = dd[u]; en[pos] = idx[u] - tile * kTI; ev[pos] = val[u];
            }
    }
}

__global__ __launch_bounds__(1024) void tile_bucket_kernel(BatchView bv, int ntiles, int* __restrict__ tstart,
                                                           int* __restrict__ eb, int* __restrict__ en,
                                                           float* __restrict__ ev) {
    extern __shared__ int bk_lds_dyn[];
    tile_bucket_body<kBucketMaxDocs>(bv, ntiles, tstart, eb, en, ev, bk_lds_dyn);
}
__global__ __launch_bounds__(1024) void tile_bucket_wide_kernel(BatchView bv, int ntiles, int* __restrict__ tstart,
                                                                int* __restrict__ eb, int* __restrict__ en,
                                                                float* __restrict__ ev) {
    extern __shared__ int bk_lds_dyn[];
    asm volatile("v_mov_b32 v127, 0" ::: "v127");
    tile_bucket_body<kBucketWideDocs>(bv, ntiles, tstart, eb, en, ev, bk_lds_dyn);
}

struct BucketJob {
    BatchView bv; int ntiles; int* tstart; int* eb; int* en; float* ev; int enabled;
};

}
```

### aae-recommender_amd/csrc/chain.h

```cpp
#pragma once
#include "device_common.h"
#include "gemm_f32.h"
#include "kernels.h"
#include "buckets.h"
#include "w1_update.h"

namespace aae {

constexpr int kCR = 16;
constexpr int kCL = 212;
constexpr int kCSlots = 10;
constexpr int kCWide = 208;
constexpr int kCT = 1024;
constexpr int kCW = kCT / 64;
constexpr int kCQ = (13 + kCW - 1) / kCW;
constexpr int kTPR = kCT / 16;
constexpr int kRS = kCT == 1024 ? 6 : 5;
constexpr int kJ = 64 / kTPR;
constexpr int kCMaxOps = 16;

enum { COP_LOAD = 0,
       COP_LINEAR,
       COP_LINEAR_DX,
       COP_FINAL_FWD,
// ... 183 lines not shown
                acc[1] = __builtin_amdgcn_mfma_f32_16x16x4f32(xa.z, y1[c].z, acc[1], 0, 0, 0);
                acc[1] = __builtin_amdgcn_mfma_f32_16x16x4f32(xa.w, y1[c].w, acc[1], 0, 0, 0);
            }
        }
    }
}

template <int MC, bool TWO>
__device__ __forceinline__ void chain_linear_dx(const ChainOp& op, const float* src, int b0, int b1, int fr, int fk,
                                                f32x4 (&acc)[2]) {
    const int ldw = op.ldw, N = op.N, K = op.K;
    const int kch = (K + 15) >> 4;
    const uint32_t o0 = (uint32_t)(4 * fk * ldw + min(b0 * 16 + fr, N - 1)) * 4u;
    const uint32_t o1 = (uint32_t)(4 * fk * ldw + min(b1 * 16 + fr, N - 1)) * 4u;
    const float* a = src + fr * kCL + 4 * fk;
    float y0[MC * 4], y1[TWO ? MC * 4 : 1];
#pragma unroll
    for (int c = 0; c < MC; ++c) {
#pragma unroll
        for (int e = 0; e < 4; ++e) {
            const char* base = reinterpret_cast<const char*>(op.W + (size_t)(min(c, kch - 1) * 16 + e) * ldw);
            y0[c * 4 + e] = *reinterpret_cast<const float*>(base + o0);
            if (TWO) y1[c * 4 + e] = *reinterpret_cast<const float*>(base + o1);
        }
    }
#pragma unroll
    for (int c = 0; c < MC; ++c) {
        if (c < kch) {
            float4 xa = *reinterpret_cast<const float4*>(a + c * 16);
            const int k0 = c * 16 + 4 * fk;
            if (k0 + 0 >= K) xa.x = 0.f;
            if (k0 + 1 >= K) xa.y = 0.f;
            if (k0 + 2 >= K) xa.z = 0.f;
            if (k0 + 3 >= K) xa.w = 0.f;
            acc[0] = __builtin_amdgcn_mfma_f32_16x16x4f32(xa.x, y0[c * 4 + 0], acc[0], 0, 0, 0);
            acc[0] = __builtin_amdgcn_mfma_f32_16x16x4f32(xa.y, y0[c * 4 + 1], acc[0], 0, 0, 0);
            acc[0] = __builtin_amdgcn_mfma_f32_16x16x4f32(xa.z, y0[c * 4 + 2], acc[0], 0, 0, 0);
            acc[0] = __builtin_amdgcn_mfma_f32_16x16x4f32(xa.w, y0[c * 4 + 3], acc[0], 0, 0, 0);
            if (TWO) {
                acc[1] = __builtin_amdgcn_mfma_f32_16x16x4f32(xa.x, y1[c * 4 + 0], acc[1], 0, 0, 0);
                acc[1] = __builtin_amdgcn_mfma_f32_16x16x4f32(xa.y, y1[c * 4 + 1], acc[1], 0, 0, 0);
                acc[1] = __builtin_amdgcn_mfma_f32_16x16x4f32(xa.z, y1[c * 4 + 2], acc[1], 0, 0, 0);
                acc[1] = __builtin_amdgcn_mfma_f32_16x16x4f32(xa.w, y1[c * 4 + 3], acc[1], 0, 0, 0);
            }
        }
    }
}

typedef __bf16 chain_bf16x8 __attribute__((ext_vector_type(8)));
__device__ __forceinline__ chain_bf16x8 chain_pack8(const float4& lo, const float4& hi) {
    const gemm_u32x4 v = {gemm_pack_bf16(lo.x, lo.y), gemm_pack_bf16(lo.z, lo.w), gemm_pack_bf16(hi.x, hi.y), gemm_pack_bf16(hi.z, hi.w)};
    return __builtin_bit_cast(chain_bf16x8, v);
}
template <int MC>
__device__ __forceinline__ void chain_linear_fwd_bf16(const ChainOp& op, const float* src, int b0, int fr, int fk, f32x4& acc) {
    const int ldw = op.ldw, N = op.N;
    const int kch = (op.K + 31) >> 5;
    const uint32_t o0 = (uint32_t)(min(b0 * 16 + fr, N - 1) * ldw + 4 * fk) * 4u;
    const float* a = src + fr * kCL;
    float4 w0[MC], w1[MC];
#pragma unroll
    for (int c = 0; c < MC; ++c) {
        const char* base = reinterpret_cast<const char*>(op.W + min(c, kch - 1) * 32);
        w0[c] = *reinterpret_cast<const float4*>(base + o0);
        w1[c] = *reinterpret_cast<const float4*>(base + o0 + 64);
    }
#pragma unroll
    for (int c = 0; c < MC; ++c) {
        if (c < kch) {
            const int k0 = 32 * c + 4 * fk, k1 = k0 + 16;
            float4 x0 = *reinterpret_cast<const float4*>(a + min(k0, kCL - 4));
            float4 x1 = *reinterpret_cast<const float4*>(a + min(k1, kCL - 4));
            if (k0 > kCL - 4) x0 = make_float4(0.f, 0.f, 0.f, 0.f);
            if (k1 > kCL - 4) x1 = make_float4(0.f, 0.f, 0.f, 0.f);
            acc = __builtin_amdgcn_mfma_f32_16x16x32_bf16(chain_pack8(x0, x1), chain_pack8(w0[c], w1[c]), acc, 0, 0, 0);
        }
    }
}

template <bool BF, bool NM = false>
__global__ __launch_bounds__(kCT) void chain_kernel(ChainProgram P) {
    extern __shared__ __attribute__((aligned(16))) float slots[];
    if (P.bk.enabled && blockIdx.x == gridDim.x - 1) {
        tile_bucket_body(P.bk.bv, P.bk.ntiles, P.bk.tstart, P.bk.eb, P.bk.en, P.bk.ev, reinterpret_cast<int*>(slots));
        return;
    }
    const int tid = threadIdx.x, lane = tid & 63;
    const int wave = __builtin_amdgcn_readfirstlane(tid >> 6);
    const int fr = lane & 15, fk = lane >> 4;
    const int r0 = blockIdx.x * kCR;
    const int nrows = min(kCR, P.rows - r0);
    const uint64_t key = rng_key(P.seed, (uint64_t)*P.step_ctr, 0);

    for (int oi = 0; oi < P.nops; ++oi) {
        const ChainOp& op = P.ops[oi];
        if (P.ts && blockIdx.x == 0 && tid == 0) P.ts[oi] = wall_clock64();
        float* dst = slots + op.dst * kCR * kCL;
        const float* src = slots + op.src * kCR * kCL;
        const int kind = op.kind;

        if (kind == COP_LINEAR || kind == COP_LINEAR_DX) {
            const int nblk = (op.N + 15) >> 4;
            f32x4 acc[2];
            acc[0] = acc[1] = (f32x4){0.f, 0.f, 0.f, 0.f};
            const int b0 = min(wave, nblk - 1), b1 = min(wave + kCW, nblk - 1);
            const bool two = kCQ > 1 && nblk > kCW;
            const EpiCtx ec = chain_epi_ctx(op.epi, op, P, key, slots);
            const int epiN = chain_pin(op.N);
            if (!(P.dbg & 1) && wave < nblk) {
                if (kind == COP_LINEAR && BF) {
                    static_assert(kCQ == 1, "one block per wave");
                    if (((op.K + 31) >> 5) <= 2) chain_linear_fwd_bf16<2>(op, src, b0, fr, fk, acc[0]);
                    else chain_linear_fwd_bf16<7>(op, src, b0, fr, fk, acc[0]);
                } else if (kind == COP_LINEAR) {
                    const int kch = (op.K + 15) >> 4;
                    if (kch <= 4) { if (two) chain_linear_fwd<4, true>(op, src, b0, b1, fr, fk, acc); else chain_linear_fwd<4, false>(op, src, b0, b1, fr, fk, acc); }
                    else          { if (two) chain_linear_fwd<13, true>(op, src, b0, b1, fr, fk, acc); else chain_linear_fwd<13, false>(op, src, b0, b1, fr, fk, acc); }
                } else {
                    const int kch = (op.K + 15) >> 4;
                    if (kch <= 4) { if (two) chain_linear_dx<4, true>(op, src, b0, b1, fr, fk, acc); else chain_linear_dx<4, false>(op, src, b0, b1, fr, fk, acc); }
                    else          { if (two) chain_linear_dx<13, true>(op, src, b0, b1, fr, fk, acc); else chain_linear_dx<13, false>(op, src, b0, b1, fr, fk, acc); }
                }
            }
            chain_barrier();
#pragma unroll
            for (int q = 0; q < kCQ; ++q) {
                const int blk = wave + kCW * q;
                if (blk < nblk) {
                    const int col = blk * 16 + fr;
#pragma unroll
                    for (int r = 0; r < 4; ++r) {
                        const int lrow = fk * 4 + r;
                        float v = 0.f;
                        if (col < epiN && lrow < nrows) v = chain_epi<NM>(ec, r0 + lrow, lrow, col, acc[q][r]);
                        dst[lrow * kCL + col] = v;
                    }
                }
            }
            {
                const int c0 = nblk * 16, lrow = tid >> kRS;
                for (int col = c0 + (tid & (kTPR - 1)); col < kCL; col += kTPR) dst[lrow * kCL + col] = 0.f;
            }
        } else if (kind == COP_LOAD) {
            chain_load_block(op.W, op.ldw, op.out_row0 + r0, nrows, op.N, dst, op.dst_col0, op.scale);
        } else if (kind == COP_SLABSUM) {
            const int lrow = tid >> kRS, rowc = min(lrow, max(nrows, 1) - 1), nf4 = (op.N + 3) >> 2;
#pragma unroll
            for (int j = 0; j < kJ; ++j) {
                const int c4 = (tid & (kTPR - 1)) + kTPR * j, c4c = min(c4, nf4 - 1);
                float4 v[16];
#pragma unroll
                for (int z = 0; z < 16; ++z)
                    v[z] = *reinterpret_cast<const float4*>(op.W + (size_t)min(z, op.aux - 1) * op.stride +
                                                            (size_t)(r0 + rowc) * op.ldw + c4c * 4);
                float4 acc4 = make_float4(0.f, 0.f, 0.f, 0.f);
#pragma unroll
                for (int z = 0; z < 16; ++z)
                    if (z < op.aux) { acc4.x += v[z].x; acc4.y += v[z].y; acc4.z += v[z].z; acc4.w += v[z].w; }
                if (op.epi == CEPI_ACTBWD) {
                    const EpiCtx sec = chain_epi_ctx(CEPI_ACTBWD, op, P, key, slots);
                    const float4 y4 = *reinterpret_cast<const float4*>(op.aux_ptr + (size_t)(r0 + rowc) * op.aux_ld + c4c * 4);
                    const int gr = r0 + lrow;
                    const bool den = sec.den && lrow < nrows;
                    const float k0 = (den && c4 * 4 + 0 < op.N) ? (chain_keep(sec, gr, c4 * 4 + 0) ? sec.mk : 0.f) : 1.f;
                    const float k1 = (den && c4 * 4 + 1 < op.N) ? (chain_keep(sec, gr, c4 * 4 + 1) ? sec.mk : 0.f) : 1.f;
                    const float k2 = (den && c4 * 4 + 2 < op.N) ? (chain_keep(sec, gr, c4 * 4 + 2) ? sec.mk : 0.f) : 1.f;
                    const float k3 = (den && c4 * 4 + 3 < op.N) ? (chain_keep(sec, gr, c4 * 4 + 3) ? sec.mk : 0.f) : 1.f;
// ... 168 lines not shown
    float* p; float* m; float* v; float* grad; int ld;
    W4Copies w4;
    const OptScalars* sc;
    int tile0;
    int tiles_n;
};
struct W1Job {
    int enabled; const float* ga1; int ld, h, rows;
    float* bp; float* bm; float* bv1; float* bgrad; const OptScalars* sc;
    int blk0, ncol;
    int nitem;
    int wave_form;
    int* hot; int* hot_count; int* hot_zero;
    W1Items items;
    int* cnt_out;
};
struct LossJob { int enabled; const float* terms; int n; float* out; };
struct DwGroup { int njobs; DwJob jobs[4]; W1Job w1; LossJob loss;
                 int ksplit;
                 unsigned long long* ts; int ts_cap; };
constexpr int kDwSmemBytes = 2 * 64 * (32 + 16) * 4;

#ifndef DW_KSPLIT_DEPTH
#define DW_KSPLIT_DEPTH 8
#endif
template <int BK, int LDT>
__device__ __forceinline__ f32x4 dw_slab_products(const float* ap, const float* bp, f32x4 acc) {
#ifdef DW_PLAIN_PRODUCTS
#pragma unroll
    for (int kk = 0; kk < BK; kk += 4) acc = __builtin_amdgcn_mfma_f32_16x16x4f32(ap[kk * LDT], bp[kk * LDT], acc, 0, 0, 0);
    return acc;
#else
    constexpr int Q = 4, NQ = BK / 4 / Q;
    static_assert(BK % (4 * Q) == 0 && NQ >= 2, "dw_slab_products: whole stages");
    float a[2][Q], b[2][Q];
#pragma unroll
    for (int i = 0; i < Q; ++i) { a[0][i] = ap[(4 * i) * LDT]; b[0][i] = bp[(4 * i) * LDT]; }
#pragma unroll
    for (int q = 0; q < NQ; ++q) {
        if (q + 1 < NQ) {
#pragma unroll
            for (int i = 0; i < Q; ++i) { a[(q + 1) & 1][i] = ap[(4 * ((q + 1) * Q + i)) * LDT]; b[(q + 1) & 1][i] = bp[(4 * ((q + 1) * Q + i)) * LDT]; }
        }
        __builtin_amdgcn_sched_barrier(0);
#pragma unroll
        for (int i = 0; i < Q; ++i) acc = __builtin_amdgcn_mfma_f32_16x16x4f32(a[q & 1][i], b[q & 1][i], acc, 0, 0, 0);
        __builtin_amdgcn_sched_barrier(0);
    }
    return acc;
#endif
}

#ifdef DW_TS
__device__ unsigned long long dw_ts[96];
#define DW_STAMP(i) do { if (threadIdx.x == 0 && blockIdx.x == 0) dw_ts[i] = wall_clock64(); } while (0)
#define DW_STAMP_W1(i) do { if (threadIdx.x == 0 && (int)blockIdx.x == grp.w1.blk0) dw_ts[i] = wall_clock64(); } while (0)
#else
#define DW_STAMP(i) do { } while (0)
#define DW_STAMP_W1(i) do { } while (0)
#endif
__device__ __forceinline__ void grouped_dw_body(const DwGroup& grp, float* smem) {
    constexpr int TS = 32, BK = 64, LDT = TS + 16, LDC = TS + 4, NV = TS * BK / 1024;
    static_assert(sizeof(float) * 2 * BK * LDT == kDwSmemBytes, "kDwSmemBytes");
    static_assert(4 * TS * LDC <= 2 * BK * LDT, "the k-split form's four partial tiles");
    DW_STAMP(0);
    if (grp.loss.enabled && blockIdx.x == gridDim.x - 1) {
        float acc = 0.f;
        for (int i = threadIdx.x; i < grp.loss.n; i += 256) acc += grp.loss.terms[i];
        smem[threadIdx.x] = acc;
        __syncthreads();
        for (int o = 128; o > 0; o >>= 1) {
            if ((int)threadIdx.x < o) smem[threadIdx.x] += smem[threadIdx.x + o];
            __syncthreads();
        }
        if (threadIdx.x == 0) *grp.loss.out = smem[0];
        return;
    }
    if (grp.w1.enabled && (int)blockIdx.x >= grp.w1.blk0) {
        const W1Job& w = grp.w1;
        const int id = (int)blockIdx.x - w.blk0;
        DW_STAMP_W1(64);
        if (id == 0 && threadIdx.x == 0 && w.cnt_out && w.nitem > 0) *w.cnt_out = *w.items.ucount;
        if (id < w.ncol) { colsum_adam_body(w.ga1, w.rows, w.h, w.ld, w.bp, w.bm, w.bv1, w.bgrad, w.sc, id, smem); DW_STAMP_W1(65); }
        else if (w.wave_form == 2) w1_item_hybrid_body(w.items, reinterpret_cast<unsigned*>(smem), id - w.ncol, w.nitem);
        else if (w.wave_form) {
            if (id == w.ncol && threadIdx.x == 0) *w.hot_zero = 0;
            w1_item_wave_body(w.items, w.hot, w.hot_count, reinterpret_cast<unsigned*>(smem), (id - w.ncol) * 4 + (int)(threadIdx.x >> 6), w.nitem * 4);
        } else w1_item_update_body(w.items, reinterpret_cast<unsigned*>(smem), id - w.ncol, w.nitem);
        return;
    }
    int j = 0;
    for (int q = 1; q < grp.njobs; ++q) if ((int)blockIdx.x >= grp.jobs[q].tile0) j = q;
    DW_STAMP(52);
    const DwJob& J = grp.jobs[j];
    const int t = blockIdx.x - J.tile0;
    const int m0 = (t / J.tiles_n) * TS, n0 = (t % J.tiles_n) * TS;
    DW_STAMP(53);
    float* As = smem; float* Bs = smem + BK * LDT;
    const int tid = threadIdx.x, lane = tid & 63, wave = tid >> 6;
    const int wm = (wave >> 1) * 16, wn = (wave & 1) * 16;
    f32x4 acc = (f32x4){0.f, 0.f, 0.f, 0.f};
    const int K = J.rows;
    const int mmax4 = ((J.M + 3) & ~3) - 4, nmax4 = ((J.N + 3) & ~3) - 4;
    float4 ra[NV], rb[NV];
    auto request = [&](int k0) {
#pragma unroll
        for (int q = 0; q < NV; ++q) {
            const int f = tid + 256 * q, kr = min(k0 + f / (TS / 4), K - 1), cq = (f % (TS / 4)) * 4;
            ra[q] = *reinterpret_cast<const float4*>(J.G + (size_t)kr * J.ldg + min(m0 + cq, mmax4));
            rb[q] = *reinterpret_cast<const float4*>(J.X + (size_t)kr * J.ldx + min(n0 + cq, nmax4));
        }
    };
    const bool ksplit = grp.ksplit > 0 && K >= grp.ksplit;
    if (!ksplit) request(0);
    DW_STAMP(54);
    const int erow = tid / (TS / 4), ecol = (tid % (TS / 4)) * 4;
    const int egm = m0 + erow, egn = n0 + ecol;
#ifdef DW_NO_OPT_PREFETCH
    const bool epre = false;
#else
    const bool epre = !J.grad && egm < J.M && egn + 3 < J.N;
#endif
    float4 pp0 = make_float4(0.f, 0.f, 0.f, 0.f), mm0 = pp0, vv0 = pp0;
    const OptScalars osc = *J.sc;
    if (epre) {
        const size_t off = (size_t)egm * J.ld + egn;
        pp0 = *reinterpret_cast<const float4*>(J.p + off);
        mm0 = *reinterpret_cast<const float4*>(J.m + off); vv0 = *reinterpret_cast<const float4*>(J.v + off);
    }
    DW_STAMP(1);
    const int row = tid / (TS / 4), col = (tid % (TS / 4)) * 4;
    const int gm = m0 + row, gn = n0 + col;
    float4 g4;
    if (ksplit) {
        constexpr int D = DW_KSPLIT_DEPTH;
        const int fr = lane & 15, fk = lane >> 4;
        const int S = (K + 3) >> 2, Sw = (S + 3) >> 2, s0 = __builtin_amdgcn_readfirstlane(wave) * Sw, s1 = min(S, s0 + Sw);
        const unsigned ca = (unsigned)min(m0 + 2 * fr, ((J.M + 1) & ~1) - 2), cb = (unsigned)min(n0 + 2 * fr, ((J.N + 1) & ~1) - 2);
        f32x4 c00 = (f32x4){0.f, 0.f, 0.f, 0.f}, c01 = c00, c10 = c00, c11 = c00;
        float2 av[D], bv[D];
        auto ld = [&](int st, int i) {
            const unsigned r = (unsigned)min(4 * st + fk, K - 1);
            av[i] = *reinterpret_cast<const float2*>(J.G + (r * (unsigned)J.ldg + ca)); bv[i] = *reinterpret_cast<const float2*>(J.X + (r * (unsigned)J.ldx + cb));
        };
#pragma unroll
        for (int i = 0; i < D; ++i) { ld(s0 + i, i); __builtin_amdgcn_sched_barrier(0); }
        int st = s0;
        const int sfull = min(s1, K >> 2);
        unsigned oa = (unsigned)(4 * (s0 + D) + fk) * (unsigned)J.ldg + ca, ob = (unsigned)(4 * (s0 + D) + fk) * (unsigned)J.ldx + cb;
        const unsigned da = 4u * (unsigned)J.ldg, db = 4u * (unsigned)J.ldx;
        for (; st + 2 * D <= sfull; st += D) {
#pragma unroll
            for (int i = 0; i < D; ++i) {
                c00 = __builtin_amdgcn_mfma_f32_16x16x4f32(av[i].x, bv[i].x, c00, 0, 0, 0);
                c01 = __builtin_amdgcn_mfma_f32_16x16x4f32(av[i].x, bv[i].y, c01, 0, 0, 0);
                c10 = __builtin_amdgcn_mfma_f32_16x16x4f32(av[i].y, bv[i].x, c10, 0, 0, 0);
                c11 = __builtin_amdgcn_mfma_f32_16x16x4f32(av[i].y, bv[i].y, c11, 0, 0, 0);
                av[i] = *reinterpret_cast<const float2*>(J.G + oa); bv[i] = *reinterpret_cast<const float2*>(J.X + ob);
                oa += da; ob += db;
                __builtin_amdgcn_sched_barrier(0);
            }
        }
        for (; st < s1; st += D) {
#pragma unroll
            for (int i = 0; i < D; ++i) {
                const bool ok = st + i < s1 && 4 * (st + i) + fk < K;
                const float a0 = ok ? av[i].x : 0.f, a1 = ok ? av[i].y : 0.f, b0 = bv[i].x, b1 = bv[i].y;
// ... 88 lines not shown
```

### aae-recommender_amd/csrc/chain4.h

```cpp
#pragma once
#include "chain.h"

namespace aae {

constexpr int kR4 = 4;
#ifndef C4_WAVES
#define C4_WAVES 16
#endif
constexpr int kC4W = C4_WAVES;
constexpr int kC4WS = kC4W == 16 ? 4 : 3;
constexpr int kC4T = 64 * kC4W;
constexpr int kC4E = 1024 / kC4T;
constexpr int kC4ER = kC4T / 256;
constexpr int kC4Part = 4096;

__device__ __forceinline__ float chain4_rb(float x) {
    return __builtin_bit_cast(float, gemm_pack_bf16(x, 0.f) << 16);
}

struct Lin4 { int N, K, ldkn, ns4; const float* W4; const float* Wkn; };

template <int MK, bool BF, bool TS = false>
__device__ __forceinline__ void chain4_linear(const Lin4& op, const float* src, float* part, int wave, int lane,
                                              int cgs, int kper, unsigned long long* wts_ = nullptr) {
// ... 62 lines not shown
    f32x4 acc0 = (f32x4){0.f, 0.f, 0.f, 0.f}, acc1 = acc0;
    const float* a = src + (lane & 3) * kCL;
    if (wts && lane == 0) wts[wave] = wall_clock64();
    const int klim = min(min(K, k0 + kper), kCL);
#ifdef C4_NO_A
    auto ldx = [&](int j) { return make_float4(1.f + j, 2.f, 3.f, 4.f + lane); };
#else
    auto ldx = [&](int j) { return *reinterpret_cast<const float4*>(a + min(k0 + 4 * j, kCL - 4)); };
#endif
    float4 xn = ldx(0);
#pragma unroll
    for (int j = 0; j < MK / 4; ++j) {
        if (wts && j == 1 && lane == 0) { asm volatile("s_nop 0" :: "v"(acc0[0])); wts[16 + wave] = wall_clock64(); }
        const int kk = k0 + 4 * j;
        float4 x = xn;
        if (j + 1 < MK / 4) xn = ldx(j + 1);
        if (kk >= klim) continue;
        if (kk + 4 > klim) {
            x.y = kk + 1 < klim ? x.y : 0.f;
            x.z = kk + 2 < klim ? x.z : 0.f;
            x.w = 0.f;
        }
        float w0 = w[4 * j], w1 = w[4 * j + 1], w2 = w[4 * j + 2], w3 = w[4 * j + 3];
        if (BF) {
            x.x = chain4_rb(x.x); x.y = chain4_rb(x.y); x.z = chain4_rb(x.z); x.w = chain4_rb(x.w);
            w0 = chain4_rb(w0); w1 = chain4_rb(w1); w2 = chain4_rb(w2); w3 = chain4_rb(w3);
        }
#ifdef C4_NO_MFMA
        acc0[0] += x.x * w0; acc1[0] += x.y * w1; acc0[1] += x.z * w2; acc1[1] += x.w * w3;
#else
        acc0 = __builtin_amdgcn_mfma_f32_4x4x1f32(x.x, w0, acc0, 0, 0, 0);
        acc1 = __builtin_amdgcn_mfma_f32_4x4x1f32(x.y, w1, acc1, 0, 0, 0);
        acc0 = __builtin_amdgcn_mfma_f32_4x4x1f32(x.z, w2, acc0, 0, 0, 0);
        acc1 = __builtin_amdgcn_mfma_f32_4x4x1f32(x.w, w3, acc1, 0, 0, 0);
#endif
    }
    acc0 += acc1;
    float* pp = part + (size_t)ks * (4 * 64 * cgp) + 64 * cg + lane;
#pragma unroll
#ifndef C4_NO_PART
    for (int r = 0; r < 4; ++r) pp[r * 64 * cgp] = acc0[r];
#else
    if (acc0[0] == 12345.f) pp[0] = acc0[1];
#endif
    if (wts && lane == 0) wts[32 + wave] = wall_clock64();
}

template <int NJ>
__device__ __forceinline__ f32x4 chain4_cols(const float* W4, int ns4, int N, int K, const float* src, int wave, int lane) {
    const int kq = lane >> 4, col = min(16 * wave + (lane & 15), N - 1);
    const unsigned st = (unsigned)ns4 * 16u;
    const __amdgpu_buffer_rsrc_t rw = __builtin_amdgcn_make_buffer_rsrc(const_cast<float*>(W4), 0, (unsigned)(((K + 3) >> 2) + kW4Pad) * st, 0x00020000);
    const unsigned vo = (unsigned)col * 16u + (unsigned)kq * st;
    unsigned so = 0;
    float4 wq[NJ];
#pragma unroll
    for (int j = 0; j < NJ; ++j) { wq[j] = __builtin_bit_cast(float4, __builtin_amdgcn_raw_buffer_load_b128(rw, vo, so, 0)); so += 4u * st; }
    __builtin_amdgcn_sched_barrier(0);
    const float4* a4 = reinterpret_cast<const float4*>(src + (lane & 3) * kCL + 4 * kq);
    f32x4 c0 = (f32x4){0.f, 0.f, 0.f, 0.f}, c1 = c0;
#pragma unroll
    for (int j = 0; j < NJ; ++j) {
        const float4 x = a4[4 * j];
        c0 = __builtin_amdgcn_mfma_f32_4x4x1f32(chain4_rb(x.x), chain4_rb(wq[j].x), c0, 0, 0, 0);
        c1 = __builtin_amdgcn_mfma_f32_4x4x1f32(chain4_rb(x.y), chain4_rb(wq[j].y), c1, 0, 0, 0);
        c0 = __builtin_amdgcn_mfma_f32_4x4x1f32(chain4_rb(x.z), chain4_rb(wq[j].z), c0, 0, 0, 0);
        c1 = __builtin_amdgcn_mfma_f32_4x4x1f32(chain4_rb(x.w), chain4_rb(wq[j].w), c1, 0, 0, 0);
    }
    c0 += c1;
#pragma unroll
    for (int r = 0; r < 4; ++r) {
        const auto a = __builtin_amdgcn_permlane16_swap(__float_as_uint(c0[r]), __float_as_uint(c0[r]), false, false);
        const float y = __uint_as_float(a[0]) + __uint_as_float(a[1]);
        const auto b = __builtin_amdgcn_permlane32_swap(__float_as_uint(y), __float_as_uint(y), false, false);
        c0[r] = __uint_as_float(b[0]) + __uint_as_float(b[1]);
    }
    return c0;
}

template <bool BF, bool TS = false, bool COLS = false, bool VAE = false>
__global__ __launch_bounds__(kC4T) void chain4_kernel(ChainProgram P) {
    extern __shared__ __attribute__((aligned(16))) float slots[];
    if (P.bk.enabled && blockIdx.x == gridDim.x - 1) {
        tile_bucket_body<kBucketMaxDocs, kC4T>(P.bk.bv, P.bk.ntiles, P.bk.tstart, P.bk.eb, P.bk.en, P.bk.ev, reinterpret_cast<int*>(slots));
        return;
    }
    float* part = slots + kCSlots * kR4 * kCL;
    const int tid = threadIdx.x, lane = tid & 63;
    const int wave = __builtin_amdgcn_readfirstlane(tid >> 6);
    const int erow0 = tid >> 8, ecol = tid & 255;
    const int r0 = blockIdx.x * kR4;
    const int nrows = min(kR4, P.rows - r0);
    const uint64_t key = rng_key(P.seed, (uint64_t)*P.step_ctr, 0);

    unsigned long long* tsp = (TS && blockIdx.x == 0) ? P.ts : nullptr;
    int nops = P.nops, kslices = COLS ? P.kslices : 1;
    asm volatile("" : "+s"(tsp), "+s"(nops));
    if constexpr (COLS) asm volatile("" : "+s"(kslices));
    for (int oi = 0; oi < nops; ++oi) {
        const ChainOp& op = P.ops[oi];
        if (TS && tsp && tid == 0) tsp[oi] = wall_clock64();
        int kind = op.kind, src_i = op.src, dst_i = op.dst, row_lo = op.row_lo, one_col = op.one_col, opN = op.N, opK = op.K;
        int ldo = op.ldo, ldo2 = op.ldo2, out_row0 = op.out_row0;
        float* outp = op.out; float* out2p = op.out2;
        Lin4 lin; lin.N = opN; lin.K = opK; lin.ldkn = op.ldkn; lin.ns4 = op.ns4; lin.W4 = op.W4; lin.Wkn = op.Wkn;
        int epi_k = op.epi, yslot_k = op.yslot, acc_in = op.acc_in;
        asm volatile("" : "+s"(kind), "+s"(src_i), "+s"(dst_i), "+s"(row_lo), "+s"(one_col), "+s"(opN), "+s"(opK), "+s"(ldo), "+s"(ldo2),
                          "+s"(out_row0), "+s"(outp), "+s"(out2p), "+s"(epi_k), "+s"(yslot_k), "+s"(acc_in));
        const float* ygp = op.y_glb; int yld = op.y_ld;
        asm volatile("" : "+s"(lin.ldkn), "+s"(lin.ns4), "+s"(lin.W4), "+s"(lin.Wkn), "+s"(ygp), "+s"(yld));
        lin.N = opN; lin.K = opK;
        if (r0 < row_lo) continue;
        float* dst = slots + dst_i * kR4 * kCL;
        const float* src = slots + src_i * kR4 * kCL;

        const float* qW = nullptr; float* qaux_ptr = nullptr; size_t qstride = 0;
        int qldw = 0, qdst_col0 = 0, qaux = 0, qaux_ld = 0, qyslot = 0, qgrow0 = 0, qrow_split = 0, qfake_slot = -1;
        float qscale = 0.f;
        if (kind != COP_LINEAR && kind != COP_LINEAR_DX) {
            qW = op.W; qaux_ptr = op.aux_ptr; qstride = op.stride; qldw = op.ldw; qdst_col0 = op.dst_col0; qaux = op.aux;
            qaux_ld = op.aux_ld; qyslot = op.yslot; qgrow0 = op.grow0; qrow_split = op.row_split; qfake_slot = op.fake_slot; qscale = op.scale;
            asm volatile("" : "+s"(qW), "+s"(qaux_ptr), "+s"(qstride), "+s"(qldw), "+s"(qdst_col0), "+s"(qaux), "+s"(qaux_ld), "+s"(qyslot),
                              "+s"(qgrow0), "+s"(qrow_split), "+s"(qfake_slot), "+s"(qscale));
        }
        bool one_done = false;
        if (kind == COP_LINEAR || kind == COP_LINEAR_DX) {
            const int N = opN, K = opK;
            const int CG = (N + 63) >> 6;
            const int cgs = CG <= 1 ? 0 : CG <= 2 ? 1 : 2, cgp = 1 << cgs;
            const int KS = kC4W >> cgs;
            const int kper = (((K + KS - 1) >> (kC4WS - cgs)) + 3) & ~3;
            unsigned long long* wts = (TS && tsp && oi == 2) ? tsp + 64 : nullptr;
            if (wts && tid == 0) { wts[48] = wall_clock64(); wts[49] = clock64(); }
            bool cols_ok = false;
            if constexpr (BF && COLS && kC4W == 16) cols_ok = !kslices && lin.W4 && K <= kCWide && N <= 16 * kC4W && src_i != dst_i;
            if (cols_ok) {
                const int crow = lane >> 4, ccol = 16 * wave + (lane & 15);
                float yv1 = 0.f;
                if (ygp) {
                    typedef const __attribute__((address_space(1))) float* gf_t;
                    yv1 = (ccol < N && crow < nrows) ? ((gf_t)ygp)[(size_t)(r0 + crow) * yld + ccol] : 0.f;
                }
                f32x4 cs = (f32x4){0.f, 0.f, 0.f, 0.f};
                if (16 * wave < N) {
                    if (K <= 64) cs = chain4_cols<4>(lin.W4, lin.ns4, N, K, src, wave, lane);
                    else if (K <= 112) cs = chain4_cols<7>(lin.W4, lin.ns4, N, K, src, wave, lane);
                    else cs = chain4_cols<13>(lin.W4, lin.ns4, N, K, src, wave, lane);
                }
                if (wts && lane == 0) wts[32 + wave] = wall_clock64();
                one_done = true;
                if (16 * wave < kCL) {
                    const EpiCtx ec = chain_epi_ctx(epi_k, op, P, key, slots);
                    float v = 0.f;
                    if (ccol < N && crow < nrows) {
                        v = crow == 0 ? cs[0] : crow == 1 ? cs[1] : crow == 2 ? cs[2] : cs[3];
                        if (acc_in) v += dst[crow * kCL + ccol];
                        if (ec.epi == CEPI_ACTBWD) {
                            v *= act_grad_from_y<false>(ec.act, ygp ? yv1 : (slots + yslot_k * kR4 * kCL)[crow * kCL + ccol]);
                            if (ec.den) v *= chain_keep(ec, r0 + crow, ccol) ? ec.mk : 0.f;
                        } else {
                            v = chain_epi<false>(ec, r0 + crow, crow, ccol, v);
                        }
                    }
                    if (ccol < kCL) dst[crow * kCL + ccol] = ccol == one_col ? (crow < nrows ? 1.f : 0.f) : v;
                }
            } else {
            float yv[kC4E];
// ... 247 lines not shown
```

### aae-recommender_amd/csrc/w1_update.h

```cpp
#pragma once
#include "buckets.h"

namespace aae {

struct W1Items {
    const int* ulist; const int* ucount;
    const int* tstart; const int* eb; const int* en; const float* ev;
    const float* ga1; int ld;
    int rpb; size_t bstride;
    const float* rscale; int rows; int h;
    float* W; float* M; float* V; int ldw;
    float* gout;
    const OptScalars* sc; int* tsync; const long long* step_ctr; int mark_synced;
};

__host__ __device__ inline size_t w1_items_lds_words(int rows) { return 2 * (size_t)((rows + 31) >> 5) + 2 * (size_t)rows + 4 * 256 + 4; }

__device__ __forceinline__ void w1_item_update_one(const W1Items& a, unsigned* w1_lds, int u, const OptScalars& s, bool upd) {
    const int tid = threadIdx.x, lane = tid & 63;
    const int wave = __builtin_amdgcn_readfirstlane(tid >> 6);
    const int nw = (a.rows + 31) >> 5;
    unsigned* bm = w1_lds;
    int* pre = reinterpret_cast<int*>(bm + nw);
    int* rl = pre + nw;
    float* xl = reinterpret_cast<float*>(rl + a.rows);
    float* part = xl + a.rows;
    int* s_n = reinterpret_cast<int*>(part + 4 * 256);
    {
        const int item = a.ulist[u];
        const int tile = item / kTI, it = item - tile * kTI;
        const int e0 = a.tstart[tile], e1 = a.tstart[tile + 1];
        const size_t o0 = (size_t)item * a.ldw + min(tid, a.ldw - 1);
        float pw = 0.f, pm = 0.f, pv = 0.f;
        if (upd) {
            pw = a.W[o0];
            if (!s.is_sgd) { pm = a.M[o0]; pv = a.V[o0]; }
        }
        for (int i = tid; i < nw; i += 256) bm[i] = 0u;
        __syncthreads();
        int my_r = -1; float my_x = 0.f;
        {
            const int ec = min(e0 + tid, e1 - 1);
            const int en_e = a.en[ec], r = a.eb[ec]; const float x = a.ev[ec];
            if (e0 + tid < e1 && en_e == it) { atomicOr(&bm[r >> 5], 1u << (r & 31)); my_r = r; my_x = x; }
        }
        for (int base = e0 + 256; base < e1; base += 1024) {
            int en4[4], r4[4];
#pragma unroll
            for (int j = 0; j < 4; ++j) { const int ec = min(base + 256 * j + tid, e1 - 1); en4[j] = a.en[ec]; r4[j] = a.eb[ec]; }
#pragma unroll
            for (int j = 0; j < 4; ++j)
                if (base + 256 * j + tid < e1 && en4[j] == it) atomicOr(&bm[r4[j] >> 5], 1u << (r4[j] & 31));
        }
        __syncthreads();
        if (wave == 0) {
            int n = 0;
            for (int base = 0; base < nw; base += 64) {
                const int i = base + lane;
                const int c = i < nw ? __popc(bm[i]) : 0;
                int inc = c;
#pragma unroll
                for (int o = 1; o < 64; o <<= 1) { const int t = __shfl_up(inc, o, 64); if (lane >= o) inc += t; }
                if (i < nw) pre[i] = n + inc - c;
                n += __shfl(inc, 63, 64);
            }
            if (lane == 0) *s_n = n;
        }
        __syncthreads();
        if (my_r >= 0) {
            const int k = pre[my_r >> 5] + __popc(bm[my_r >> 5] & ((1u << (my_r & 31)) - 1u));
            rl[k] = my_r; xl[k] = my_x;
        }
        for (int base = e0 + 256; base < e1; base += 1024) {
            int en4[4], r4[4]; float x4[4];
#pragma unroll
            for (int j = 0; j < 4; ++j) { const int ec = min(base + 256 * j + tid, e1 - 1); en4[j] = a.en[ec]; r4[j] = a.eb[ec]; x4[j] = a.ev[ec]; }
#pragma unroll
            for (int j = 0; j < 4; ++j)
                if (base + 256 * j + tid < e1 && en4[j] == it) {
                    const int r = r4[j];
                    const int k = pre[r >> 5] + __popc(bm[r >> 5] & ((1u << (r & 31)) - 1u));
                    rl[k] = r; xl[k] = x4[j];
                }
        }
        __syncthreads();
        const int n = *s_n;
        const int q = n <= 16 ? n : (n + 3) >> 2;
        const int i_lo = min(wave * q, n), i_hi = min(i_lo + q, n);
        for (int cb = 0; cb < a.h; cb += 256) {
            const int c4 = cb + 4 * lane;
            const int cc = min(c4, a.ld - 4);
            float4 acc = make_float4(0.f, 0.f, 0.f, 0.f);
            constexpr int kU = 16;
            for (int i0 = i_lo; i0 < i_hi; i0 += kU) {
                float4 g[kU]; float x[kU];
#pragma unroll
                for (int j = 0; j < kU; ++j) {
                    const int i = min(i0 + j, i_hi - 1);
                    const int r = rl[i];
                    x[j] = (i0 + j < i_hi ? xl[i] : 0.f) * a.rscale[r];
                    const float* grow = a.rpb > 0 ? a.ga1 + (size_t)(r / a.rpb) * a.bstride + (size_t)(r % a.rpb) * a.ld
                                                  : a.ga1 + (size_t)r * a.ld;
                    g[j] = *reinterpret_cast<const float4*>(grow + cc);
                }
#pragma unroll
                for (int j = 0; j < kU; ++j) {
                    acc.x += x[j] * g[j].x; acc.y += x[j] * g[j].y; acc.z += x[j] * g[j].z; acc.w += x[j] * g[j].w;
                }
            }
            if (c4 >= a.h) acc.x = 0.f;
            if (c4 + 1 >= a.h) acc.y = 0.f;
            if (c4 + 2 >= a.h) acc.z = 0.f;
            if (c4 + 3 >= a.h) acc.w = 0.f;
            *reinterpret_cast<float4*>(part + wave * 256 + 4 * lane) = acc;
            __syncthreads();
            const int c = cb + tid;
            const float g = ((part[tid] + part[256 + tid]) + part[512 + tid]) + part[768 + tid];
            const size_t o = (size_t)item * a.ldw + min(c, a.ldw - 1);
            if (cb > 0 && upd) {
                pw = a.W[o];
                if (!s.is_sgd) { pm = a.M[o]; pv = a.V[o]; }
            }
            if (c < a.ldw) {
                if (!upd) a.gout[o] = g;
                else {
                    adam_update(pw, pm, pv, g, s);
                    a.W[o] = pw;
                    if (!s.is_sgd) { a.M[o] = pm; a.V[o] = pv; }
                }
            }
            __syncthreads();
        }
        if (upd && a.mark_synced && tid == 0) a.tsync[item] = (int)*a.step_ctr;
    }
}
__device__ __forceinline__ void w1_item_update_body(const W1Items& a, unsigned* w1_lds, int vblock, int vgrid) {
    const int cnt = *a.ucount;
    const bool upd = a.gout == nullptr;
    OptScalars s;
    if (upd) s = *a.sc;
    for (int u = vblock; u < cnt; u += vgrid) w1_item_update_one(a, w1_lds, u, s, upd);
}

constexpr int kW1WaveRows = 48;
__host__ __device__ inline size_t w1_wave_lds_words(int waves) { return (size_t)waves * 4 * kW1WaveRows; }

__device__ __forceinline__ void w1_item_wave_body(const W1Items& a, int* __restrict__ hot, int* __restrict__ hot_count,
                                                  unsigned* lds, int vwave, int vwaves) {
    const int lane = threadIdx.x & 63, wv = (threadIdx.x >> 6);
    int* rl = reinterpret_cast<int*>(lds) + wv * 4 * kW1WaveRows;
    float* xl = reinterpret_cast<float*>(rl + kW1WaveRows);
    int* rs = reinterpret_cast<int*>(xl + kW1WaveRows);
    float* xs = reinterpret_cast<float*>(rs + kW1WaveRows);
    const int cnt = *a.ucount;
    const bool upd = a.gout == nullptr;
    OptScalars s;
    if (upd) s = *a.sc;
    for (int u = vwave; u < cnt; u += vwaves) {
        const int item = a.ulist[u];
        const int tile = item / kTI, it = item - tile * kTI;
        const int e0 = a.tstart[tile], e1 = a.tstart[tile + 1];
        const int c4 = 4 * lane;
        const size_t o0 = (size_t)item * a.ldw + min(c4, a.ldw - 4);
        float4 pw = make_float4(0.f, 0.f, 0.f, 0.f), pm = pw, pv = pw;
        if (upd) {
            pw = *reinterpret_cast<const float4*>(a.W + o0);
            if (!s.is_sgd) { pm = *reinterpret_cast<const float4*>(a.M + o0); pv = *reinterpret_cast<const float4*>(a.V + o0); }
        }
        int n = 0;
        for (int base = e0; base < e1; base += 256) {
            int en4[4], r4[4]; float x4[4];
#pragma unroll
            for (int j = 0; j < 4; ++j) { const int ec = min(base + 64 * j + lane, e1 - 1); en4[j] = a.en[ec]; r4[j] = a.eb[ec]; x4[j] = a.ev[ec]; }
#pragma unroll
            for (int j = 0; j < 4; ++j) {
                const bool hit = base + 64 * j + lane < e1 && en4[j] == it;
                const unsigned long long bal = __ballot(hit);
                const int k = n + __popcll(bal & ((1ull << lane) - 1ull));
                if (hit && k < kW1WaveRows) { rl[k] = r4[j]; xl[k] = x4[j]; }
                n += __popcll(bal);
            }
        }
        if (n > kW1WaveRows) {
            if (lane == 0) hot[atomicAdd(hot_count, 1)] = item;
            continue;
        }
        if (lane < n) {
            const int r = rl[lane];
            int k = 0;
            for (int j = 0; j < n; ++j) k += (rl[j] < r || (rl[j] == r && j < lane)) ? 1 : 0;
            rs[k] = r; xs[k] = xl[lane];
        }
        for (int cb = 0; cb < a.h; cb += 256) {
            const int cc = min(cb + c4, a.ld - 4);
            float4 acc = make_float4(0.f, 0.f, 0.f, 0.f);
            constexpr int kU = 8;
            for (int i0 = 0; i0 < n; i0 += kU) {
                float4 g[kU]; float x[kU];
#pragma unroll
                for (int j = 0; j < kU; ++j) {
                    const int i = min(i0 + j, n - 1);
                    const int r = rs[i];
                    x[j] = (i0 + j < n ? xs[i] : 0.f) * a.rscale[r];
                    const float* grow = a.rpb > 0 ? a.ga1 + (size_t)(r / a.rpb) * a.bstride + (size_t)(r % a.rpb) * a.ld
                                                  : a.ga1 + (size_t)r * a.ld;
                    g[j] = *reinterpret_cast<const float4*>(grow + cc);
                }
#pragma unroll
                for (int j = 0; j < kU; ++j) {
                    acc.x += x[j] * g[j].x; acc.y += x[j] * g[j].y; acc.z += x[j] * g[j].z; acc.w += x[j] * g[j].w;
                }
            }
            const int c = cb + c4;
            if (c >= a.h) acc.x = 0.f;
            if (c + 1 >= a.h) acc.y = 0.f;
            if (c + 2 >= a.h) acc.z = 0.f;
            if (c + 3 >= a.h) acc.w = 0.f;
            const size_t o = (size_t)item * a.ldw + min(c, a.ldw - 4);
            if (cb > 0 && upd) {
                pw = *reinterpret_cast<const float4*>(a.W + o);
                if (!s.is_sgd) { pm = *reinterpret_cast<const float4*>(a.M + o); pv = *reinterpret_cast<const float4*>(a.V + o); }
            }
            if (c < a.ldw) {
                if (!upd) *reinterpret_cast<float4*>(a.gout + o) = acc;
                else {
                    adam_update(pw.x, pm.x, pv.x, acc.x, s); adam_update(pw.y, pm.y, pv.y, acc.y, s);
                    adam_update(pw.z, pm.z, pv.z, acc.z, s); adam_update(pw.w, pm.w, pv.w, acc.w, s);
                    *reinterpret_cast<float4*>(a.W + o) = pw;
                    if (!s.is_sgd) { *reinterpret_cast<float4*>(a.M + o) = pm; *reinterpret_cast<float4*>(a.V + o) = pv; }
                }
            }
        }
        if (upd && a.mark_synced && lane == 0) a.tsync[item] = (int)*a.step_ctr;
    }
}

#ifdef W1_TS
__device__ unsigned long long w1_ts[4096 * 4 * 8];
#define W1_STAMP(i) do { if (lane == 0 && vblock < 4096) w1_ts[(vblock * 4 + wv) * 8 + (i)] = wall_clock64(); } while (0)
#else
#define W1_STAMP(i) do { } while (0)
#endif
constexpr int kW1HybRows = 16;
constexpr int kW1HybWords = 64;
__host__ __device__ inline size_t w1_hybrid_lds_words(int rows) {
    const size_t a = w1_items_lds_words(rows), b = 4 * 4 * kW1HybRows;
    return (a > b ? a : b) + kW1HybWords;
}
__device__ __forceinline__ void w1_item_hybrid_body(const W1Items& a, unsigned* lds, int vblock, int vgrid) {
    const int tid = threadIdx.x, lane = tid & 63, wv = __builtin_amdgcn_readfirstlane(tid >> 6);
    unsigned* defer = lds + (w1_hybrid_lds_words(a.rows) - kW1HybWords);
    W1_STAMP(0);
    for (int i = tid; i < kW1HybWords; i += 256) defer[i] = 0u;
    __syncthreads();
    int* rl = reinterpret_cast<int*>(lds) + wv * 4 * kW1HybRows;
    float* xl = reinterpret_cast<float*>(rl + kW1HybRows);
    int* rs = reinterpret_cast<int*>(xl + kW1HybRows);
    float* xs = reinterpret_cast<float*>(rs + kW1HybRows);
    const int cnt = *a.ucount;
    const bool upd = a.gout == nullptr;
    OptScalars s;
    if (upd) s = *a.sc;
    const int ustep = vgrid * 4;
    int round = 0;
    W1_STAMP(1);
    constexpr int kRounds = kW1HybWords * 32 / 4;
    for (int u = vblock + wv * vgrid; u < cnt && round < kRounds; u += ustep, ++round) {
        const int item = a.ulist[u];
        const int tile = item / kTI, it = item - tile * kTI;
        const int e0 = a.tstart[tile], e1 = a.tstart[tile + 1];
        if (round == 0) W1_STAMP(2);
        const int c4 = 4 * lane;
        const size_t o0 = (size_t)item * a.ldw + min(c4, a.ldw - 4);
        float4 pw = make_float4(0.f, 0.f, 0.f, 0.f), pm = pw, pv = pw;
        if (upd) {
            pw = *reinterpret_cast<const float4*>(a.W + o0);
            if (!s.is_sgd) { pm = *reinterpret_cast<const float4*>(a.M + o0); pv = *reinterpret_cast<const float4*>(a.V + o0); }
        }
        int n = 0;
        for (int base = e0; base < e1; base += 256) {
            int en4[4], r4[4]; float x4[4];
#pragma unroll
            for (int j = 0; j < 4; ++j) { const int ec = min(base + 64 * j + lane, e1 - 1); en4[j] = a.en[ec]; r4[j] = a.eb[ec]; x4[j] = a.ev[ec]; }
#pragma unroll
            for (int j = 0; j < 4; ++j) {
                const bool hit = base + 64 * j + lane < e1 && en4[j] == it;
                const unsigned long long bal = __ballot(hit);
                const int k = n + __popcll(bal & ((1ull << lane) - 1ull));
                if (hit && k < kW1HybRows) { rl[k] = r4[j]; xl[k] = x4[j]; }
                n += __popcll(bal);
            }
        }
        if (round == 0) W1_STAMP(3);
        if (n > kW1HybRows) {
            const int b = round * 4 + wv;
            if (lane == 0) atomicOr(&defer[b >> 5], 1u << (b & 31));
            continue;
        }
        if (lane < n) {
            const int r = rl[lane];
            int k = 0;
            for (int j = 0; j < n; ++j) k += (rl[j] < r || (rl[j] == r && j < lane)) ? 1 : 0;
            rs[k] = r; xs[k] = xl[lane];
        }
        for (int cb = 0; cb < a.h; cb += 256) {
            const int cc = min(cb + c4, a.ld - 4);
            float4 acc = make_float4(0.f, 0.f, 0.f, 0.f);
            constexpr int kU = 8;
            for (int i0 = 0; i0 < n; i0 += kU) {
                float4 g[kU]; float x[kU];
#pragma unroll
                for (int j = 0; j < kU; ++j) {
                    const int i = min(i0 + j, n - 1);
                    const int r = rs[i];
                    x[j] = (i0 + j < n ? xs[i] : 0.f) * a.rscale[r];
                    const float* grow = a.rpb > 0 ? a.ga1 + (size_t)(r / a.rpb) * a.bstride + (size_t)(r % a.rpb) * a.ld
                                                  : a.ga1 + (size_t)r * a.ld;
                    g[j] = *reinterpret_cast<const float4*>(grow + cc);
                }
#pragma unroll
                for (int j = 0; j < kU; ++j) {
                    acc.x += x[j] * g[j].x; acc.y += x[j] * g[j].y; acc.z += x[j] * g[j].z; acc.w += x[j] * g[j].w;
                }
            }
            const int c = cb + c4;
            if (c >= a.h) acc.x = 0.f;
            if (c + 1 >= a.h) acc.y = 0.f;
            if (c + 2 >= a.h) acc.z = 0.f;
            if (c + 3 >= a.h) acc.w = 0.f;
            const size_t o = (size_t)item * a.ldw + min(c, a.ldw - 4);
            if (cb > 0 && upd) {
                pw = *reinterpret_cast<const float4*>(a.W + o);
                if (!s.is_sgd) { pm = *reinterpret_cast<const float4*>(a.M + o); pv = *reinterpret_cast<const float4*>(a.V + o); }
            }
            if (c < a.ldw) {
                if (!upd) *reinterpret_cast<float4*>(a.gout + o) = acc;
                else {
                    adam_update(pw.x, pm.x, pv.x, acc.x, s); adam_update(pw.y, pm.y, pv.y, acc.y, s);
                    adam_update(pw.z, pm.z, pv.z, acc.z, s); adam_update(pw.w, pm.w, pv.w, acc.w, s);
                    *reinterpret_cast<float4*>(a.W + o) = pw;
                    if (!s.is_sgd) { *reinterpret_cast<float4*>(a.M + o) = pm; *reinterpret_cast<float4*>(a.V + o) = pv; }
                }
            }
        }
        if (upd && a.mark_synced && lane == 0) a.tsync[item] = (int)*a.step_ctr;
        if (round == 0) W1_STAMP(4);
    }
    W1_STAMP(5);
    __syncthreads();
    W1_STAMP(6);
    const int rounds = vblock < cnt ? (cnt - vblock + ustep - 1) / ustep : 0;
    const int nbits = min(rounds, kRounds) * 4;
    for (int b = 0; b < nbits; ++b) {
        if (!((defer[b >> 5] >> (b & 31)) & 1u)) continue;
        w1_item_update_one(a, lds, vblock + (b & 3) * vgrid + (b >> 2) * ustep, s, upd);
    }
    for (int u = vblock + kRounds * ustep; u < cnt; u += vgrid) w1_item_update_one(a, lds, u, s, upd);
    W1_STAMP(7);
}

__global__ __launch_bounds__(256) void w1_item_wave_kernel(W1Items a, int* hot, int* hot_count) {
    extern __shared__ unsigned w1w_lds_dyn[];
    w1_item_wave_body(a, hot, hot_count, w1w_lds_dyn, (int)(blockIdx.x * 4 + (threadIdx.x >> 6)), (int)gridDim.x * 4);
}

__global__ __launch_bounds__(256) void w1_item_update_kernel(W1Items a) {
    extern __shared__ unsigned w1_lds_dyn[];
    w1_item_update_body(a, w1_lds_dyn, (int)blockIdx.x, (int)gridDim.x);
}

}
```

### include/aaerec_hip.h

```cpp
#ifndef AAEREC_HIP_H
#define AAEREC_HIP_H

#include <stddef.h>
#include <stdint.h>

#ifdef __cplusplus
extern "C" {
#endif

#define AAE_ABI_VERSION 4

#define AAE_OK 0
#define AAE_EINVAL (-1)
#define AAE_ENOMEM (-2)
#define AAE_EHIP (-3)
#define AAE_ESTATE (-4)

enum { AAE_ACT_RELU = 0, AAE_ACT_SELU = 1, AAE_ACT_TANH = 2, AAE_ACT_SIGMOID = 3,
       AAE_ACT_ELU = 4, AAE_ACT_LEAKYRELU = 5,
       AAE_ACT_SOFTPLUS = 6, AAE_ACT_HARDTANH = 7, AAE_ACT_RELU6 = 8, AAE_ACT_CELU = 9, AAE_ACT_SOFTSIGN = 10,
       AAE_ACT_HARDSIGMOID = 11, AAE_ACT_LOGSIGMOID = 12, AAE_ACT_SOFTSHRINK = 13, AAE_ACT_HARDSHRINK = 14,
       AAE_ACT_IDENTITY = 15,
       AAE_ACT_GELU = 16, AAE_ACT_SILU = 17, AAE_ACT_MISH = 18, AAE_ACT_HARDSWISH = 19, AAE_ACT_COUNT = 20 };
enum { AAE_FINAL_LINEAR = 0, AAE_FINAL_SOFTMAX = 1, AAE_FINAL_SIGMOID = 2 };
// ... 5 lines not shown
       AAE_MODEL_AE = 1,
       AAE_MODEL_VAE = 3 };
enum { AAE_DTYPE_F32 = 0,
       AAE_DTYPE_BF16 = 1 };
enum { AAE_GRAD_FUSED = 0,
       AAE_GRAD_EXPORT = 1 };

typedef struct aae_config {
    int32_t abi_version;
    int32_t n_items;
    int32_t n_hidden;
    int32_t n_code;
    int32_t cond_inc;
    int32_t max_batch;
    int32_t max_nnz;
    int32_t activation;
    int32_t enc_final;
    int32_t optimizer;
    int32_t normalize_inputs;
    int32_t rng_mode;
    int32_t prior;
    int32_t grad_mode;
    float dropout1, dropout2;
    float gen_lr, reg_lr;
    float prior_scale;
    int32_t has_prior_scale;
    uint64_t seed;
    int32_t unfused_decoder;
    int32_t dp_world;
    int32_t model_kind;
    int32_t dtype;
    int32_t blocked_output;
    int32_t dense_noise;
    int32_t reserved[2];
} aae_config;

typedef struct aae_model* aae_handle;

typedef struct aae_batch {
    const int64_t* indptr_dev;
    const int32_t* indices_dev;
    const float* values_dev;
    const int32_t* rows_dev;
    int32_t row_start;
    int32_t n_rows;
    int32_t nnz_bound;
    int32_t max_row_nnz;
    int64_t generation;
} aae_batch;

typedef struct aae_rng_inject {
    const uint8_t* masks_dev[12];
    const float* z_real_dev;
} aae_rng_inject;

enum {
    AAE_T_ENC_W1T = 0, AAE_T_ENC_B1, AAE_T_ENC_W2, AAE_T_ENC_W3,
    AAE_T_DEC_V1, AAE_T_DEC_V2, AAE_T_DEC_V3,
    AAE_T_DISC_D1, AAE_T_DISC_D2, AAE_T_DISC_D3,
    AAE_T_N_PARAMS,
    AAE_T_ADAM_ENC = 16,
    AAE_T_ADAM_GEN = 32,
    AAE_T_ADAM_DEC = 48,
    AAE_T_ADAM_DISC = 64,
    AAE_T_GRAD = 80,
    AAE_T_ACT_Z = 96,
    AAE_T_ACT_LOSSES = 97,
    AAE_T_ACT_A1 = 98,
    AAE_T_ACT_DH2 = 100,
    AAE_T_ACT_DA2 = 101,
    AAE_T_ACT_GA1 = 102,
    AAE_T_ACT_DZC = 99
};

typedef struct aae_tensor {
    size_t byte_offset;
    int64_t rows, cols;
    int64_t ld;
} aae_tensor;

int aae_abi_version(void);
const char* aae_last_error(void);
int aae_set_option(const char* name, const char* value);

int aae_arena_bytes(const aae_config* cfg, size_t* bytes_out);
int aae_create(const aae_config* cfg, void* arena_dev, size_t arena_bytes, void* stream,
               aae_handle* out);
int aae_destroy(aae_handle h);
int aae_tensor_info(aae_handle h, int tensor_id, aae_tensor* out);
int aae_sync(aae_handle h, void* stream);
int aae_set_rng_rows(aae_handle h, int64_t row_offset, int64_t global_rows);
int aae_params_changed(aae_handle h);
int aae_set_lr(aae_handle h, double gen_lr, double reg_lr);

int aae_load_linear(aae_handle h, int net, int layer, const float* weight_host,
                    const float* bias_host);
int aae_store_linear(aae_handle h, int net, int layer, float* weight_host, float* bias_host);
int aae_load_adam(aae_handle h, int which, int layer, const float* m_w, const float* v_w,
                  const float* m_b, const float* v_b, int64_t step);
int aae_store_adam(aae_handle h, int which, int layer, float* m_w, float* v_w, float* m_b,
                   float* v_b, int64_t* step);

int aae_step(aae_handle h, const aae_batch* batch, const float* cond_dev,
             const aae_rng_inject* inject, void* stream);

int aae_ae_encode(aae_handle h, const aae_batch* batch, const aae_rng_inject* inject,
                  float* z_out_dev, void* stream);
int aae_ae_decode_backward(aae_handle h, const float* zc_dev, int64_t zc_ld,
                           const aae_rng_inject* inject, float* dzc_out_dev, void* stream);
int aae_ae_encoder_backward(aae_handle h, const float* dz_dev, int64_t dz_ld, void* stream);
int aae_disc_gen(aae_handle h, const aae_rng_inject* inject, void* stream);
int aae_decoder_step(aae_handle h, const aae_batch* batch, const float* zin_dev, int64_t zin_ld,
                     const aae_rng_inject* inject, float* dzin_out_dev, void* stream);
int aae_vae_step(aae_handle h, const aae_batch* batch, const float* cond_dev, const float* eps_dev, void* stream);
int aae_vae_predict(aae_handle h, const aae_batch* batch, const float* cond_dev, const float* eps_dev,
                    float* out_dev, int64_t out_ld, void* stream);
int aae_vae_encode(aae_handle h, const aae_batch* batch, const float* eps_dev, float* z_out_dev, int32_t train, void* stream);
int aae_vae_decode_backward(aae_handle h, const float* zc_dev, int64_t zc_ld, float* dzc_out_dev, void* stream);
int aae_vae_encoder_backward(aae_handle h, const float* dz_dev, int64_t dz_ld, void* stream);
int aae_ae_forward(aae_handle h, const aae_batch* batch, const float* cond_dev, const aae_rng_inject* inject, void* stream);
int aae_output_layer_step(aae_handle h, const aae_batch* batch, void* stream);
int aae_ae_backward(aae_handle h, const float* dA2_dev, int64_t dA2_ld, void* stream);
int aae_set_doc_l1(aae_handle h, const float* doc_l1_dev);
int aae_set_first_layer_external(aae_handle h, int on);
int aae_first_layer_forward(aae_handle h, const aae_batch* batch, const float* bias_dev, void* stream);
int aae_first_layer_update(aae_handle h, const float* ga1_dev, int64_t ld, int32_t rows_per_block, int64_t block_stride,
                           int which, void* stream);
int aae_apply_gathered(aae_handle h, int which_a, int which_b, const float* packets_dev, int64_t peer_stride,
                       int32_t n_peers, int64_t span_offset, void* stream);

enum { AAE_CAT_SUM = 0, AAE_CAT_MEAN = 1 };
enum { AAE_CAT_SPARSE_ADAM = 0, AAE_CAT_ADAM = 1 };
int aae_cat_encode(const float* table_dev, int32_t vocab, int32_t dim, const int32_t* idx_dev, int32_t rows,
                   int32_t width, int32_t reduce, float* out_dev, int64_t out_ld, void* stream);
int aae_cat_update(float* table_dev, float* exp_avg_dev, float* exp_avg_sq_dev, float* grad_scratch_dev, int32_t vocab,
                   int32_t dim, const int32_t* idx_dev, int32_t rows, int32_t width, int32_t reduce,
                   const float* dout_dev, int64_t dout_ld, int32_t optimizer, double lr, int64_t step, void* stream);
int aae_csr_embed(const int64_t* indptr_dev, const int32_t* indices_dev, const float* values_dev, int32_t n_rows,
                  const float* table_dev, int32_t n_table_rows, int32_t dim, int64_t table_ld, float* out_dev,
                  int64_t out_ld, void* stream);
int aae_dense_to_csr(const void* dense_dev, int32_t elem_bytes, int64_t ld, int32_t rows, int32_t n_cols,
                     int64_t* indptr_dev, int32_t* indices_dev, float* values_dev, int64_t capacity,
                     int32_t* scratch_dev, int32_t* stats_out_host, void* stream);
int aae_disc_step(aae_handle h, const aae_rng_inject* inject, void* stream);
int aae_gen_step(aae_handle h, const aae_rng_inject* inject, void* stream);

int aae_read_losses(aae_handle h, float out_host[3], void* stream);

int aae_predict(aae_handle h, const aae_batch* batch, const float* cond_dev, float* out_dev,
                int64_t out_ld, void* stream);
int aae_predict_topk(aae_handle h, const aae_batch* batch, const float* cond_dev, int32_t k,
                     int32_t exclude_known, int32_t* idx_out_dev, float* val_out_dev, void* stream);
int aae_rank_max_rows(aae_handle h, int32_t k, int32_t* rows_out);
int aae_rank_long_stats(aae_handle h, int64_t out[5]);
int aae_decode_topk(aae_handle h, const float* zc_dev, int64_t zc_ld, const aae_batch* batch, int32_t k,
                    int32_t exclude_known, int32_t* idx_out_dev, float* val_out_dev, void* stream);
int aae_predict_ranks(aae_handle h, const aae_batch* batch, const float* cond_dev, const aae_batch* truth,
                      int32_t exclude_known, int32_t* ranks_out_dev, void* stream);
int aae_decode_ranks(aae_handle h, const float* zc_dev, int64_t zc_ld, const aae_batch* batch, const aae_batch* truth,
                     int32_t exclude_known, int32_t* ranks_out_dev, void* stream);
int aae_rank_full_max_rows(aae_handle h, int32_t* rows_out);
int aae_vae_predict_topk(aae_handle h, const aae_batch* batch, const float* cond_dev, const float* eps_dev, int32_t k,
                         int32_t exclude_known, int32_t* idx_out_dev, float* val_out_dev, void* stream);
int aae_vae_predict_ranks(aae_handle h, const aae_batch* batch, const float* cond_dev, const float* eps_dev,
                          const aae_batch* truth, int32_t exclude_known, int32_t* ranks_out_dev, void* stream);
int aae_vae_decode_topk(aae_handle h, const float* zc_dev, int64_t zc_ld, const aae_batch* batch, int32_t k,
// ... 151 lines not shown
```

Baseline: 438,300 docs/s.

## Build per-item row lists in tile bucket kernel and use them for W1 updates

The tile bucketing kernel now also builds, in LDS, per-item lists of (doc row, value) entries. Small items and large items get their records written from opposite ends of a record array, and tiles with many entries go through a bitmap-based placement pass. The W1 item update kernels read these precomputed lists instead of rediscovering each item's rows, and the per-wave sum-and-Adam loop is factored into a shared helper. This aims to cut the work of gathering rows per item in the sparse first-layer update, at the cost of extra LDS use, a larger bucket kernel and more arena memory; an option turns it off and a debug export is added.

```diff
diff --git a/aae-recommender_amd/aaerec/_hip.py b/aae-recommender_amd/aaerec/_hip.py
--- a/aae-recommender_amd/aaerec/_hip.py
+++ b/aae-recommender_amd/aaerec/_hip.py
@@ -111,6 +111,8 @@
 _PROTOS = {
     "aae_abi_version": (C.c_int, []),
     "aae_set_option": (C.c_int, [C.c_char_p, C.c_char_p]),
+    "aae_debug_item_lists": (C.c_int, [C.c_void_p, C.POINTER(C.c_int), C.POINTER(C.c_int), C.c_int, C.POINTER(C.c_int), C.c_int,
+                                       C.POINTER(C.c_int)]),
     "aae_last_error": (C.c_char_p, []),
     "aae_arena_bytes": (C.c_int, [C.POINTER(AaeConfig), C.POINTER(C.c_size_t)]),
     "aae_create": (C.c_int, [C.POINTER(AaeConfig), C.c_void_p, C.c_size_t, C.c_void_p, C.POINTER(C.c_void_p)]),
@@ -1426,6 +1428,19 @@
     def big_grad(self):
         return T_DEC_V3, self.tensor(T_GRAD + T_DEC_V3, padded=True), self.tensor(T_DEC_V3, padded=True)
 
+    def debug_item_lists(self, n_entries):
+        cap = C.c_int()
+        counts = np.zeros(2, dtype=np.int32)
+        ip = C.POINTER(C.c_int)
+        with self._on_device():
+            rc = self.lib.aae_debug_item_lists(self.handle, counts.ctypes.data_as(ip), None, 0, None, 0, C.byref(cap))
+            _check(rc)
+            rec = np.zeros((max(cap.value, 1), 2), dtype=np.int32)
+            ent = np.zeros((max(int(n_entries), 1), 2), dtype=np.int32)
+            _check(self.lib.aae_debug_item_lists(self.handle, counts.ctypes.data_as(ip), rec.ctypes.data_as(ip), cap.value,
+                                                 ent.ctypes.data_as(ip), int(n_entries), C.byref(cap)))
+        return counts, rec[:cap.value], ent[:int(n_entries)]
+
     def _w1_layout(self, cap):
         if self._w1_packet is None:
             hw, tot = C.c_int64(), C.c_int64()
diff --git a/aae-recommender_amd/csrc/aae_abi.hip b/aae-recommender_amd/csrc/aae_abi.hip
--- a/aae-recommender_amd/csrc/aae_abi.hip
+++ b/aae-recommender_amd/csrc/aae_abi.hip
@@ -55,7 +55,7 @@
 
 int aae_set_option(const char* name, const char* value) {
     if (!name || !*name) return fail(AAE_EINVAL, "option name is empty");
-    static const char* known[] = {"NO_CHAIN", "CHAIN16", "SPLIT_ANY", "BLOCKED_ANY", "EARLY_ANY", "NO_LATE_JOIN", "NO_ITEM_COUNT", "W1_SERIAL",
+    static const char* known[] = {"NO_CHAIN", "CHAIN16", "SPLIT_ANY", "BLOCKED_ANY", "EARLY_ANY", "NO_LATE_JOIN", "NO_ITEM_COUNT", "NO_ITEM_LISTS", "W1_SERIAL",
                                   "NO_RANK_FUSED", "CHAIN_KSLICES", "X16_ROWS", "DW_KSPLIT_ROWS", "DEC_TS", "CHAIN_TS", "DW_TS", "DEC_SKIP", "CHAIN_SKIP", "RANK_SKIP",
                                   "RANK_COLLECT_CAP"};
     bool ok = false;
@@ -137,7 +137,7 @@
         if (m->fused_ok) {
             each_dec_fused(kDecFused, limit(m->fused_ok, maxlds));
             if (m->bf16) each_dec_fused_bf16(kDecFused, limit(m->fused_ok, maxlds));
-            if (!raise_lds_limit(tile_bucket_kernel, maxlds - 2048)) m->fused_ok = false;
+            if (!raise_lds_limit(tile_bucket_kernel, kBucketLdsMax)) m->fused_ok = false;
             m->bucket_wide_ok = raise_lds_limit(tile_bucket_wide_kernel, maxlds - 16384);
             {
                 hipFuncAttributes fa;
@@ -246,6 +246,16 @@
     return (int)hipMemcpyFromSymbol(out, HIP_SYMBOL(aae::w1_ts), sizeof(unsigned long long) * (size_t)n);
 }
 #endif
+int aae_debug_item_lists(aae_handle h, int* counts, int* rec, int rec_cap, int* ent, int n_ent, int* cap_out) {
+    if (!h || !counts || !cap_out) return fail(AAE_EINVAL, "handle / counts / cap_out is NULL");
+    *cap_out = h->il_cap;
+    HIPCHK(hipDeviceSynchronize());
+    if (!h->lists_valid || !h->buckets_valid) return fail(AAE_ESTATE, "the running batch has no item lists");
+    HIPCHK(hipMemcpy(counts, h->il_counts, 2 * sizeof(int), hipMemcpyDeviceToHost));
+    if (rec) HIPCHK(hipMemcpy(rec, h->il_rec, sizeof(int2) * (size_t)std::min(rec_cap, h->il_cap), hipMemcpyDeviceToHost));
+    if (ent) HIPCHK(hipMemcpy(ent, h->il_ent, sizeof(int2) * (size_t)std::max<int64_t>(0, std::min<int64_t>(n_ent, std::min<int64_t>(h->cfg.max_nnz, kItemListMaxEntries))), hipMemcpyDeviceToHost));
+    return AAE_OK;
+}
 int aae_destroy(aae_handle h) {
     if (!h) return AAE_OK;
     if (h->side) {
diff --git a/aae-recommender_amd/csrc/abi_chains.h b/aae-recommender_amd/csrc/abi_chains.h
--- a/aae-recommender_amd/csrc/abi_chains.h
+++ b/aae-recommender_amd/csrc/abi_chains.h
@@ -387,6 +387,7 @@
     m->w1_hot_pending = false;
     W1Items a = w1_items_args(m, m->w1_hot_ga1, 0, 0, m->w1_hot_which);
     a.ulist = m->hot_list + (size_t)m->w1_hot_set * m->hot_cap; a.ucount = m->hot_count + m->w1_hot_set;
+    a.rec = nullptr;
     const size_t lds = sizeof(int) * w1_items_lds_words(m->rows);
     hipLaunchKernelGGL(w1_item_update_kernel, dim3(std::min(m->hot_cap, 256)), dim3(256), lds, s, a);
     LAUNCHCHK("w1_item_update (hot list)");
@@ -427,13 +428,25 @@
 }
 static void flip_bucket_set(aae_model* m) {
     std::swap(m->tstart, m->tstart2); std::swap(m->teb, m->teb2); std::swap(m->ten, m->ten2); std::swap(m->tev, m->tev2);
+    std::swap(m->il_rec, m->il_rec2); std::swap(m->il_ent, m->il_ent2); std::swap(m->il_counts, m->il_counts2);
+    m->lists_valid = false;
+}
+static ItemLists item_lists_job(aae_model* m, size_t lds_bytes) {
+    ItemLists il{nullptr, nullptr, nullptr, 0, 0};
+    if (m->il_cap > 0) { il.rec = m->il_rec; il.ent = m->il_ent; il.counts = m->il_counts; il.cap = m->il_cap; il.lds_words = (int)(lds_bytes / sizeof(int)); }
+    return il;
 }
 int build_tile_buckets(aae_model* m, hipStream_t s) {
     const int ntiles = (m->N + kTI - 1) / kTI, B = m->rows;
     flip_bucket_set(m);
     const size_t lds1 = sizeof(int) * ((size_t)ntiles + 1 + kBucketMaxDocs + 1 + 1024);
     if (ntiles <= kBucketMaxTiles && B <= kBucketMaxDocs && (m->fused_ok || lds1 <= 48 * 1024)) {
-        hipLaunchKernelGGL(tile_bucket_kernel, dim3(1), dim3(1024), lds1, s, m->bv, ntiles, m->tstart, m->teb, m->ten, m->tev);
+        size_t lds = lds1;
+        if (m->il_cap > 0)
+            lds = std::min<size_t>(m->fused_ok ? kBucketLdsMax : 48 * 1024, lds1 + sizeof(int) * (4 + 2 * (size_t)std::min<int64_t>(m->cfg.max_nnz, kItemListMaxEntries) + 16 * 256 +
+                                                                       kItemListMaxEntries / kItemListWaveTile + 1));
+        hipLaunchKernelGGL(tile_bucket_kernel, dim3(1), dim3(1024), lds, s, m->bv, ntiles, m->tstart, m->teb, m->ten, m->tev, item_lists_job(m, lds));
+        m->lists_valid = m->il_cap > 0;
     } else if (ntiles <= kBucketMaxTiles && B <= kBucketWideDocs && m->bucket_wide_ok) {
         size_t lds = sizeof(int) * ((size_t)ntiles + 1 + kBucketWideDocs + 1 + 1024);
         constexpr bool bk_claim = true;
@@ -470,6 +483,8 @@
     a.gout = m->cfg.grad_mode == AAE_GRAD_EXPORT ? m->Gr[P_W1T].p : nullptr;
     a.sc = m->sc + which; a.tsync = m->tsync; a.step_ctr = m->step_ctr;
     a.mark_synced = (which == O_GEN || m->ae_only) ? 1 : 0;
+    const bool lists = m->lists_valid && m->buckets_valid && m->rows <= kBucketMaxDocs && rpb == 0;
+    a.rec = lists ? m->il_rec : nullptr; a.ent = m->il_ent; a.lcounts = m->il_counts; a.lcap = m->il_cap;
     return a;
 }
 int launch_w1_items(aae_model* m, const float* ga1, int rpb, size_t bstride, int which, hipStream_t s) {
@@ -494,7 +509,8 @@
     flip_bucket_set(m);
     BucketJob& b = cb.P.bk;
     b.bv = m->bv; b.ntiles = ntiles; b.tstart = m->tstart; b.eb = m->teb; b.en = m->ten; b.ev = m->tev; b.enabled = 1;
-    m->buckets_valid = true;
+    b.il = item_lists_job(m, (size_t)kCSlots * kCR * kCL * sizeof(float));
+    m->buckets_valid = true; m->lists_valid = m->il_cap > 0;
 }
 
 int chain_ae_forward(aae_model* m, bool with_dec, const float* cond_dev, float* z_out, hipStream_t s) {
diff --git a/aae-recommender_amd/csrc/abi_model.h b/aae-recommender_amd/csrc/abi_model.h
--- a/aae-recommender_amd/csrc/abi_model.h
+++ b/aae-recommender_amd/csrc/abi_model.h
@@ -38,6 +38,7 @@
     bool early_any;
     bool no_late_join;
     bool no_item_count;
+    bool no_item_lists;
     bool w1_serial;
     bool no_rank_fused;
     bool chain_kslices;
@@ -55,6 +56,7 @@
     auto num = [](const char* n, int dflt) { const char* e = option_value(n); return e ? atoi(e) : dflt; };
     o.no_chain = on("NO_CHAIN"); o.chain16 = on("CHAIN16"); o.split_any = on("SPLIT_ANY"); o.blocked_any = on("BLOCKED_ANY");
     o.early_any = on("EARLY_ANY"); o.no_late_join = on("NO_LATE_JOIN"); o.no_item_count = on("NO_ITEM_COUNT");
+    o.no_item_lists = on("NO_ITEM_LISTS");
     o.w1_serial = on("W1_SERIAL"); o.no_rank_fused = on("NO_RANK_FUSED"); o.chain_kslices = on("CHAIN_KSLICES");
     o.x16_rows = num("X16_ROWS", 1024); o.dw_ksplit_rows = num("DW_KSPLIT_ROWS", -1);
     o.rank_collect_cap = std::max(0, std::min(num("RANK_COLLECT_CAP", 0), 4096));
@@ -106,6 +108,7 @@
     int n_cu; bool fused_ok; int fused_nb; bool force_unfused;
     int* tcount; int* tstart; int* teb; int* ten; float* tev;
     int* tstart2; int* teb2; int* ten2; float* tev2;
+    int2* il_rec; int2* il_ent; int* il_counts; int2* il_rec2; int2* il_ent2; int* il_counts2; int il_cap; bool lists_valid;
     int* tsync; int* mark; int* ulist; int* ucount; int* stamp; LazyTab* tab;
     int* hot_list = nullptr; int* hot_count = nullptr; int hot_cap = 0, hot_flip = 0;
     bool w1_hot_pending = false; int w1_hot_set = 0, w1_hot_which = 0; const float* w1_hot_ga1 = nullptr;
@@ -327,6 +330,11 @@
         m->teb2 = reinterpret_cast<int*>(a.take((size_t)c.max_nnz, nullptr));
         m->ten2 = reinterpret_cast<int*>(a.take((size_t)c.max_nnz, nullptr));
         m->tev2 = a.take((size_t)c.max_nnz, nullptr);
+        m->il_cap = m->opt.no_item_lists ? 0 : (int)std::min<int64_t>(std::min<int64_t>(c.max_nnz, N), kItemListMaxEntries);
+        const size_t ne = m->il_cap ? (size_t)std::min<int64_t>(c.max_nnz, kItemListMaxEntries) : 0;
+        m->il_rec = reinterpret_cast<int2*>(a.take(2 * (size_t)m->il_cap, nullptr)); m->il_ent = reinterpret_cast<int2*>(a.take(2 * ne, nullptr));
+        m->il_rec2 = reinterpret_cast<int2*>(a.take(2 * (size_t)m->il_cap, nullptr)); m->il_ent2 = reinterpret_cast<int2*>(a.take(2 * ne, nullptr));
+        m->il_counts = reinterpret_cast<int*>(a.take(4, nullptr)); m->il_counts2 = reinterpret_cast<int*>(a.take(4, nullptr));
     }
     m->losses = a.take(4, nullptr);
     m->adv_terms = a.take((size_t)R2, nullptr);
diff --git a/aae-recommender_amd/csrc/buckets.h b/aae-recommender_amd/csrc/buckets.h
--- a/aae-recommender_amd/csrc/buckets.h
+++ b/aae-recommender_amd/csrc/buckets.h
@@ -11,10 +11,21 @@
 constexpr int kBucketMaxTiles = 32 * 1024;
 
 constexpr int kBucketWideDocs = 1024;
+constexpr size_t kBucketLdsMax = 160 * 1024 - 2048;
+
+constexpr int kItemListSmallRows = 16;
+constexpr int kItemListMaxEntries = 20 * 1024;
+constexpr int kItemListWaveTile = 16;
+struct ItemLists {
+    int2* rec; int2* ent; int* counts;
+    int cap;
+    int lds_words;
+};
+
 template <int MAXD = kBucketMaxDocs, int NT = 1024>
 __device__ __forceinline__ void tile_bucket_body(const BatchView& bv, int ntiles, int* __restrict__ tstart,
                                                  int* __restrict__ eb, int* __restrict__ en, float* __restrict__ ev,
-                                                 int* bk_lds) {
+                                                 int* bk_lds, const ItemLists il = ItemLists{nullptr, nullptr, nullptr, 0, 0}) {
     int* cnt = bk_lds;
     int* dbeg = cnt + ntiles + 1;
     int* part = dbeg + MAXD + 1;
@@ -40,6 +51,14 @@
     if (t == 0) dbeg[docs] = part[MAXD - 1];
     __syncthreads();
     const int total = dbeg[docs];
+    int* lcnt = part + NT;
+    int* keys = lcnt + 4;
+    float* vals = reinterpret_cast<float*>(keys + total);
+    unsigned* bms = reinterpret_cast<unsigned*>(vals + total);
+    int* bigt = reinterpret_cast<int*>(bms + (NT / 64) * 256);
+    const bool lists = MAXD <= 128 && il.counts != nullptr && total <= kItemListMaxEntries &&
+                       (ntiles + 1 + MAXD + 1 + NT + 4) + 2 * total + (NT / 64) * 256 + total / kItemListWaveTile + 1 <= il.lds_words;
+    if (lists && t < 4) lcnt[t] = 0;
     auto doc_of = [&](int f) {
         int lo = 0, hi = docs - 1;
         while (lo < hi) { const int mid = (lo + hi + 1) >> 1; if (dbeg[mid] <= f) lo = mid; else hi = mid - 1; }
@@ -77,6 +96,7 @@
         tstart[i] = run;
         cnt[i] = run;
         run += c;
+        if (lists && c > kItemListWaveTile) bigt[atomicAdd(&lcnt[2], 1)] = i;
     }
     if (t == NT - 1) tstart[ntiles] = part[NT - 1];
     __syncthreads();
@@ -96,15 +116,100 @@
                 const int tile = idx[u] / kTI;
                 const int pos = atomicAdd(&cnt[tile], 1);
                 eb[pos] = dd[u]; en[pos] = idx[u] - tile * kTI; ev[pos] = val[u];
-            }
-    }
+                if (lists) { keys[pos] = (idx[u] << 7) | dd[u]; vals[pos] = val[u]; }
+            }
+    }
+    if (MAXD > 128 || il.counts == nullptr) return;
+    if (!lists) { if (t == 0) il.counts[0] = il.counts[1] = -1; return; }
+    __syncthreads();
+    auto put_record = [&](int item, int first, int n) {
+        const bool big = n > kItemListSmallRows;
+        const int slot = atomicAdd(&lcnt[big ? 1 : 0], 1);
+        il.rec[big ? il.cap - 1 - slot : slot] = make_int2(item, (first << 7) | n);
+    };
+    for (int p0 = t & ~63; p0 < total; p0 += NT) {
+        const int p = min(p0 + (t & 63), total - 1);
+        const int key = keys[p], item = key >> 7, tile = item / kTI;
+        const int ts = tile > 0 ? cnt[tile - 1] : 0, te = cnt[tile];
+        const bool mine = p0 + (t & 63) < total && te - ts <= kItemListWaveTile;
+        int rank = 0, same = 0, before = 0;
+        for (int j0 = ts; mine && j0 < te; j0 += 4) {
+            int k4[4];
+#pragma unroll
+            for (int u = 0; u < 4; ++u) k4[u] = keys[min(j0 + u, te - 1)];
+#pragma unroll
+            for (int u = 0; u < 4; ++u) {
+                const int j = j0 + u, k = k4[u];
+                const bool in = j < te, lt = in && (((long long)k << 32) | (unsigned)j) < (((long long)key << 32) | (unsigned)p);
+                const bool sm = in && (unsigned)(k ^ key) < 128u;
+                rank += lt ? 1 : 0; same += sm ? 1 : 0; before += (sm && lt) ? 1 : 0;
+            }
+        }
+        if (mine) il.ent[ts + rank] = make_int2(key & 127, __float_as_int(vals[p]));
+        const bool first = mine && before == 0;
+        const unsigned long long few = __ballot(first && same <= kItemListSmallRows);
+        if (few) {
+            int slot0 = 0;
+            if ((t & 63) == __ffsll((long long)few) - 1) slot0 = atomicAdd(&lcnt[0], __popcll(few));
+            slot0 = __shfl(slot0, __ffsll((long long)few) - 1, 64);
+            if (first && same <= kItemListSmallRows)
+                il.rec[slot0 + __popcll(few & ((1ull << (t & 63)) - 1ull))] = make_int2(item, ((ts + rank) << 7) | same);
+        }
+        if (first && same > kItemListSmallRows) put_record(item, ts + rank, same);
+    }
+    {
+        const int lane = t & 63, wv = t >> 6;
+        unsigned* bm = bms + wv * 256;
+        int* pre = reinterpret_cast<int*>(bm + 128);
+        const int nbig = lcnt[2];
+        for (int b = wv; b < nbig; b += NT / 64) {
+            const int tile = bigt[b];
+            const int ts = tile > 0 ? cnt[tile - 1] : 0, te = cnt[tile];
+            bm[lane] = 0u; bm[lane + 64] = 0u;
+            for (int base = ts; base < te; base += 256) {
+                int k4[4];
+#pragma unroll
+                for (int u = 0; u < 4; ++u) k4[u] = keys[min(base + 64 * u + lane, te - 1)];
+#pragma unroll
+                for (int u = 0; u < 4; ++u)
+                    if (base + 64 * u + lane < te) atomicOr(&bm[((k4[u] >> 7) & 31) * 4 + ((k4[u] & 127) >> 5)], 1u << (k4[u] & 31));
+            }
+            const int li = lane & 31;
+            const int c0 = __popc(bm[li * 4]), c1 = __popc(bm[li * 4 + 1]), c2 = __popc(bm[li * 4 + 2]), c3 = __popc(bm[li * 4 + 3]);
+            const int c = lane < 32 ? c0 + c1 + c2 + c3 : 0;
+            int inc = c;
+#pragma unroll
+            for (int o = 1; o < 32; o <<= 1) { const int v = __shfl_up(inc, o, 64); if (lane >= o) inc += v; }
+            const int off = ts + inc - c;
+            if (lane < 32) {
+                pre[lane * 4] = off; pre[lane * 4 + 1] = off + c0; pre[lane * 4 + 2] = off + c0 + c1; pre[lane * 4 + 3] = off + c0 + c1 + c2;
+                if (c > 0) put_record(tile * kTI + lane, off, c);
+            }
+            for (int base = ts; base < te; base += 256) {
+                int k4[4]; float x4[4];
+#pragma unroll
+                for (int u = 0; u < 4; ++u) { const int j = min(base + 64 * u + lane, te - 1); k4[u] = keys[j]; x4[u] = vals[j]; }
+                int pos[4];
+#pragma unroll
+                for (int u = 0; u < 4; ++u) {
+                    const int w = ((k4[u] >> 7) & 31) * 4 + ((k4[u] & 127) >> 5);
+                    pos[u] = pre[w] + __popc(bm[w] & ((1u << (k4[u] & 31)) - 1u));
+                }
+#pragma unroll
+                for (int u = 0; u < 4; ++u)
+                    if (base + 64 * u + lane < te) il.ent[pos[u]] = make_int2(k4[u] & 127, __float_as_int(x4[u]));
+            }
+        }
+    }
+    __syncthreads();
+    if (t < 2) il.counts[t] = lcnt[t];
 }
 
 __global__ __launch_bounds__(1024) void tile_bucket_kernel(BatchView bv, int ntiles, int* __restrict__ tstart,
                                                            int* __restrict__ eb, int* __restrict__ en,
-                                                           float* __restrict__ ev) {
+                                                           float* __restrict__ ev, ItemLists il) {
     extern __shared__ int bk_lds_dyn[];
-    tile_bucket_body<kBucketMaxDocs>(bv, ntiles, tstart, eb, en, ev, bk_lds_dyn);
+    tile_bucket_body<kBucketMaxDocs>(bv, ntiles, tstart, eb, en, ev, bk_lds_dyn, il);
 }
 __global__ __launch_bounds__(1024) void tile_bucket_wide_kernel(BatchView bv, int ntiles, int* __restrict__ tstart,
                                                                 int* __restrict__ eb, int* __restrict__ en,
@@ -116,6 +221,7 @@
 
 struct BucketJob {
     BatchView bv; int ntiles; int* tstart; int* eb; int* en; float* ev; int enabled;
+    ItemLists il;
 };
 
 }
diff --git a/aae-recommender_amd/csrc/chain.h b/aae-recommender_amd/csrc/chain.h
--- a/aae-recommender_amd/csrc/chain.h
+++ b/aae-recommender_amd/csrc/chain.h
@@ -289,7 +289,7 @@
 __global__ __launch_bounds__(kCT) void chain_kernel(ChainProgram P) {
     extern __shared__ __attribute__((aligned(16))) float slots[];
     if (P.bk.enabled && blockIdx.x == gridDim.x - 1) {
-        tile_bucket_body(P.bk.bv, P.bk.ntiles, P.bk.tstart, P.bk.eb, P.bk.en, P.bk.ev, reinterpret_cast<int*>(slots));
+        tile_bucket_body(P.bk.bv, P.bk.ntiles, P.bk.tstart, P.bk.eb, P.bk.en, P.bk.ev, reinterpret_cast<int*>(slots), P.bk.il);
         return;
     }
     const int tid = threadIdx.x, lane = tid & 63;
@@ -624,7 +624,10 @@
         DW_STAMP_W1(64);
         if (id == 0 && threadIdx.x == 0 && w.cnt_out && w.nitem > 0) *w.cnt_out = *w.items.ucount;
         if (id < w.ncol) { colsum_adam_body(w.ga1, w.rows, w.h, w.ld, w.bp, w.bm, w.bv1, w.bgrad, w.sc, id, smem); DW_STAMP_W1(65); }
-        else if (w.wave_form == 2) w1_item_hybrid_body(w.items, reinterpret_cast<unsigned*>(smem), id - w.ncol, w.nitem);
+        else if (w.wave_form == 2) {
+            if (!(w.items.rec && w1_item_list_body(w.items, reinterpret_cast<unsigned*>(smem), id - w.ncol, w.nitem, true)))
+                w1_item_hybrid_body(w.items, reinterpret_cast<unsigned*>(smem), id - w.ncol, w.nitem);
+        }
         else if (w.wave_form) {
             if (id == w.ncol && threadIdx.x == 0) *w.hot_zero = 0;
             w1_item_wave_body(w.items, w.hot, w.hot_count, reinterpret_cast<unsigned*>(smem), (id - w.ncol) * 4 + (int)(threadIdx.x >> 6), w.nitem * 4);
diff --git a/aae-recommender_amd/csrc/chain4.h b/aae-recommender_amd/csrc/chain4.h
--- a/aae-recommender_amd/csrc/chain4.h
+++ b/aae-recommender_amd/csrc/chain4.h
@@ -168,7 +168,7 @@
 __global__ __launch_bounds__(kC4T) void chain4_kernel(ChainProgram P) {
     extern __shared__ __attribute__((aligned(16))) float slots[];
     if (P.bk.enabled && blockIdx.x == gridDim.x - 1) {
-        tile_bucket_body<kBucketMaxDocs, kC4T>(P.bk.bv, P.bk.ntiles, P.bk.tstart, P.bk.eb, P.bk.en, P.bk.ev, reinterpret_cast<int*>(slots));
+        tile_bucket_body<kBucketMaxDocs, kC4T>(P.bk.bv, P.bk.ntiles, P.bk.tstart, P.bk.eb, P.bk.en, P.bk.ev, reinterpret_cast<int*>(slots), P.bk.il);
         return;
     }
     float* part = slots + kCSlots * kR4 * kCL;
diff --git a/aae-recommender_amd/csrc/w1_update.h b/aae-recommender_amd/csrc/w1_update.h
--- a/aae-recommender_amd/csrc/w1_update.h
+++ b/aae-recommender_amd/csrc/w1_update.h
@@ -12,9 +12,67 @@
     float* W; float* M; float* V; int ldw;
     float* gout;
     const OptScalars* sc; int* tsync; const long long* step_ctr; int mark_synced;
+    const int2* rec; const int2* ent; const int* lcounts; int lcap;
 };
 
 __host__ __device__ inline size_t w1_items_lds_words(int rows) { return 2 * (size_t)((rows + 31) >> 5) + 2 * (size_t)rows + 4 * 256 + 4; }
+
+__device__ __forceinline__ void w1_item_sum_update(const W1Items& a, unsigned* w1_lds, int item, int n, const OptScalars& s, bool upd,
+                                                   float pw, float pm, float pv) {
+    const int tid = threadIdx.x, lane = tid & 63;
+    const int wave = __builtin_amdgcn_readfirstlane(tid >> 6);
+    const int nw = (a.rows + 31) >> 5;
+    const int* rl = reinterpret_cast<const int*>(w1_lds) + 2 * nw;
+    const float* xl = reinterpret_cast<const float*>(rl + a.rows);
+    float* part = const_cast<float*>(xl) + a.rows;
+    const int q = n <= 16 ? n : (n + 3) >> 2;
+    const int i_lo = min(wave * q, n), i_hi = min(i_lo + q, n);
+    for (int cb = 0; cb < a.h; cb += 256) {
+        const int c4 = cb + 4 * lane;
+        const int cc = min(c4, a.ld - 4);
+        float4 acc = make_float4(0.f, 0.f, 0.f, 0.f);
+        constexpr int kU = 16;
+        for (int i0 = i_lo; i0 < i_hi; i0 += kU) {
+            float4 g[kU]; float x[kU];
+#pragma unroll
+            for (int j = 0; j < kU; ++j) {
+                const int i = min(i0 + j, i_hi - 1);
+                const int r = rl[i];
+                x[j] = (i0 + j < i_hi ? xl[i] : 0.f) * a.rscale[r];
+                const float* grow = a.rpb > 0 ? a.ga1 + (size_t)(r / a.rpb) * a.bstride + (size_t)(r % a.rpb) * a.ld
+                                              : a.ga1 + (size_t)r * a.ld;
+                g[j] = *reinterpret_cast<const float4*>(grow + cc);
+            }
+#pragma unroll
+            for (int j = 0; j < kU; ++j) {
+                acc.x += x[j] * g[j].x; acc.y += x[j] * g[j].y; acc.z += x[j] * g[j].z; acc.w += x[j] * g[j].w;
+            }
+        }
+        if (c4 >= a.h) acc.x = 0.f;
+        if (c4 + 1 >= a.h) acc.y = 0.f;
+        if (c4 + 2 >= a.h) acc.z = 0.f;
+        if (c4 + 3 >= a.h) acc.w = 0.f;
+        *reinterpret_cast<float4*>(part + wave * 256 + 4 * lane) = acc;
+        __syncthreads();
+        const int c = cb + tid;
+        const float g = ((part[tid] + part[256 + tid]) + part[512 + tid]) + part[768 + tid];
+        const size_t o = (size_t)item * a.ldw + min(c, a.ldw - 1);
+        if (cb > 0 && upd) {
+            pw = a.W[o];
+            if (!s.is_sgd) { pm = a.M[o]; pv = a.V[o]; }
+        }
+        if (c < a.ldw) {
+            if (!upd) a.gout[o] = g;
+            else {
+                adam_update(pw, pm, pv, g, s);
+                a.W[o] = pw;
+                if (!s.is_sgd) { a.M[o] = pm; a.V[o] = pv; }
+            }
+        }
+        __syncthreads();
+    }
+    if (upd && a.mark_synced && tid == 0) a.tsync[item] = (int)*a.step_ctr;
+}
 
 __device__ __forceinline__ void w1_item_update_one(const W1Items& a, unsigned* w1_lds, int u, const OptScalars& s, bool upd) {
     const int tid = threadIdx.x, lane = tid & 63;
@@ -85,56 +143,12 @@
         }
         __syncthreads();
         const int n = *s_n;
-        const int q = n <= 16 ? n : (n + 3) >> 2;
-        const int i_lo = min(wave * q, n), i_hi = min(i_lo + q, n);
-        for (int cb = 0; cb < a.h; cb += 256) {
-            const int c4 = cb + 4 * lane;
-            const int cc = min(c4, a.ld - 4);
-            float4 acc = make_float4(0.f, 0.f, 0.f, 0.f);
-            constexpr int kU = 16;
-            for (int i0 = i_lo; i0 < i_hi; i0 += kU) {
-                float4 g[kU]; float x[kU];
-#pragma unroll
-                for (int j = 0; j < kU; ++j) {
-                    const int i = min(i0 + j, i_hi - 1);
-                    const int r = rl[i];
-                    x[j] = (i0 + j < i_hi ? xl[i] : 0.f) * a.rscale[r];
-                    const float* grow = a.rpb > 0 ? a.ga1 + (size_t)(r / a.rpb) * a.bstride + (size_t)(r % a.rpb) * a.ld
-                                                  : a.ga1 + (size_t)r * a.ld;
-                    g[j] = *reinterpret_cast<const float4*>(grow + cc);
-                }
-#pragma unroll
-                for (int j = 0; j < kU; ++j) {
-                    acc.x += x[j] * g[j].x; acc.y += x[j] * g[j].y; acc.z += x[j] * g[j].z; acc.w += x[j] * g[j].w;
-                }
-            }
-            if (c4 >= a.h) acc.x = 0.f;
-            if (c4 + 1 >= a.h) acc.y = 0.f;
-            if (c4 + 2 >= a.h) acc.z = 0.f;
-            if (c4 + 3 >= a.h) acc.w = 0.f;
-            *reinterpret_cast<float4*>(part + wave * 256 + 4 * lane) = acc;
-            __syncthreads();
-            const int c = cb + tid;
-            const float g = ((part[tid] + part[256 + tid]) + part[512 + tid]) + part[768 + tid];
-            const size_t o = (size_t)item * a.ldw + min(c, a.ldw - 1);
-            if (cb > 0 && upd) {
-                pw = a.W[o];
-                if (!s.is_sgd) { pm = a.M[o]; pv = a.V[o]; }
-            }
-            if (c < a.ldw) {
-                if (!upd) a.gout[o] = g;
-                else {
-                    adam_update(pw, pm, pv, g, s);
-                    a.W[o] = pw;
-                    if (!s.is_sgd) { a.M[o] = pm; a.V[o] = pv; }
-                }
-            }
-            __syncthreads();
-        }
-        if (upd && a.mark_synced && tid == 0) a.tsync[item] = (int)*a.step_ctr;
-    }
-}
+        w1_item_sum_update(a, w1_lds, item, n, s, upd, pw, pm, pv);
+    }
+}
+__device__ __forceinline__ bool w1_item_list_body(const W1Items& a, unsigned* lds, int vblock, int vgrid, bool four);
 __device__ __forceinline__ void w1_item_update_body(const W1Items& a, unsigned* w1_lds, int vblock, int vgrid) {
+    if (a.rec && w1_item_list_body(a, w1_lds, vblock, vgrid, false)) return;
     const int cnt = *a.ucount;
     const bool upd = a.gout == nullptr;
     OptScalars s;
@@ -246,6 +260,51 @@
 __host__ __device__ inline size_t w1_hybrid_lds_words(int rows) {
     const size_t a = w1_items_lds_words(rows), b = 4 * 4 * kW1HybRows;
     return (a > b ? a : b) + kW1HybWords;
+}
+__device__ __forceinline__ void w1_wave_sum_update(const W1Items& a, const int* rs, const float* xs, int item, int n, const OptScalars& s,
+                                                   bool upd, float4 pw, float4 pm, float4 pv) {
+    const int lane = threadIdx.x & 63, c4 = 4 * lane;
+    for (int cb = 0; cb < a.h; cb += 256) {
+        const int cc = min(cb + c4, a.ld - 4);
+        float4 acc = make_float4(0.f, 0.f, 0.f, 0.f);
+        constexpr int kU = 8;
+        for (int i0 = 0; i0 < n; i0 += kU) {
+            float4 g[kU]; float x[kU];
+#pragma unroll
+            for (int j = 0; j < kU; ++j) {
+                const int i = min(i0 + j, n - 1);
+                const int r = rs[i];
+                x[j] = (i0 + j < n ? xs[i] : 0.f) * a.rscale[r];
+                const float* grow = a.rpb > 0 ? a.ga1 + (size_t)(r / a.rpb) * a.bstride + (size_t)(r % a.rpb) * a.ld
+                                              : a.ga1 + (size_t)r * a.ld;
+                g[j] = *reinterpret_cast<const float4*>(grow + cc);
+            }
+#pragma unroll
+            for (int j = 0; j < kU; ++j) {
+                acc.x += x[j] * g[j].x; acc.y += x[j] * g[j].y; acc.z += x[j] * g[j].z; acc.w += x[j] * g[j].w;
+            }
+        }
+        const int c = cb + c4;
+        if (c >= a.h) acc.x = 0.f;
+        if (c + 1 >= a.h) acc.y = 0.f;
+        if (c + 2 >= a.h) acc.z = 0.f;
+        if (c + 3 >= a.h) acc.w = 0.f;
+        const size_t o = (size_t)item * a.ldw + min(c, a.ldw - 4);
+        if (cb > 0 && upd) {
+            pw = *reinterpret_cast<const float4*>(a.W + o);
+            if (!s.is_sgd) { pm = *reinterpret_cast<const float4*>(a.M + o); pv = *reinterpret_cast<const float4*>(a.V + o); }
+        }
+        if (c < a.ldw) {
+            if (!upd) *reinterpret_cast<float4*>(a.gout + o) = acc;
+            else {
+                adam_update(pw.x, pm.x, pv.x, acc.x, s); adam_update(pw.y, pm.y, pv.y, acc.y, s);
+                adam_update(pw.z, pm.z, pv.z, acc.z, s); adam_update(pw.w, pm.w, pv.w, acc.w, s);
+                *reinterpret_cast<float4*>(a.W + o) = pw;
+                if (!s.is_sgd) { *reinterpret_cast<float4*>(a.M + o) = pm; *reinterpret_cast<float4*>(a.V + o) = pv; }
+            }
+        }
+    }
+    if (upd && a.mark_synced && lane == 0) a.tsync[item] = (int)*a.step_ctr;
 }
 __device__ __forceinline__ void w1_item_hybrid_body(const W1Items& a, unsigned* lds, int vblock, int vgrid) {
     const int tid = threadIdx.x, lane = tid & 63, wv = __builtin_amdgcn_readfirstlane(tid >> 6);
@@ -303,47 +362,7 @@
             for (int j = 0; j < n; ++j) k += (rl[j] < r || (rl[j] == r && j < lane)) ? 1 : 0;
             rs[k] = r; xs[k] = xl[lane];
         }
-        for (int cb = 0; cb < a.h; cb += 256) {
-            const int cc = min(cb + c4, a.ld - 4);
-            float4 acc = make_float4(0.f, 0.f, 0.f, 0.f);
-            constexpr int kU = 8;
-            for (int i0 = 0; i0 < n; i0 += kU) {
-                float4 g[kU]; float x[kU];
-#pragma unroll
-                for (int j = 0; j < kU; ++j) {
-                    const int i = min(i0 + j, n - 1);
-                    const int r = rs[i];
-                    x[j] = (i0 + j < n ? xs[i] : 0.f) * a.rscale[r];
-                    const float* grow = a.rpb > 0 ? a.ga1 + (size_t)(r / a.rpb) * a.bstride + (size_t)(r % a.rpb) * a.ld
-                                                  : a.ga1 + (size_t)r * a.ld;
-                    g[j] = *reinterpret_cast<const float4*>(grow + cc);
-                }
-#pragma unroll
-                for (int j = 0; j < kU; ++j) {
-                    acc.x += x[j] * g[j].x; acc.y += x[j] * g[j].y; acc.z += x[j] * g[j].z; acc.w += x[j] * g[j].w;
-                }
-            }
-            const int c = cb + c4;
-            if (c >= a.h) acc.x = 0.f;
-            if (c + 1 >= a.h) acc.y = 0.f;
-            if (c + 2 >= a.h) acc.z = 0.f;
-            if (c + 3 >= a.h) acc.w = 0.f;
-            const size_t o = (size_t)item * a.ldw + min(c, a.ldw - 4);
-            if (cb > 0 && upd) {
-                pw = *reinterpret_cast<const float4*>(a.W + o);
-                if (!s.is_sgd) { pm = *reinterpret_cast<const float4*>(a.M + o); pv = *reinterpret_cast<const float4*>(a.V + o); }
-            }
-            if (c < a.ldw) {
-                if (!upd) *reinterpret_cast<float4*>(a.gout + o) = acc;
-                else {
-                    adam_update(pw.x, pm.x, pv.x, acc.x, s); adam_update(pw.y, pm.y, pv.y, acc.y, s);
-                    adam_update(pw.z, pm.z, pv.z, acc.z, s); adam_update(pw.w, pm.w, pv.w, acc.w, s);
-                    *reinterpret_cast<float4*>(a.W + o) = pw;
-                    if (!s.is_sgd) { *reinterpret_cast<float4*>(a.M + o) = pm; *reinterpret_cast<float4*>(a.V + o) = pv; }
-                }
-            }
-        }
-        if (upd && a.mark_synced && lane == 0) a.tsync[item] = (int)*a.step_ctr;
+        w1_wave_sum_update(a, rs, xs, item, n, s, upd, pw, pm, pv);
         if (round == 0) W1_STAMP(4);
     }
     W1_STAMP(5);
@@ -359,6 +378,52 @@
     W1_STAMP(7);
 }
 
+__device__ __forceinline__ bool w1_item_list_body(const W1Items& a, unsigned* lds, int vblock, int vgrid, bool four) {
+    const int tid = threadIdx.x, lane = tid & 63, wv = __builtin_amdgcn_readfirstlane(tid >> 6);
+    const bool upd = a.gout == nullptr;
+    const int u0 = four ? vblock + wv * vgrid : vblock;
+    const int cs = a.lcounts[0], cb = a.lcounts[1];
+    const int2 rec0 = a.rec[min(u0, a.lcap - 1)];
+    OptScalars s;
+    if (upd) s = *a.sc;
+    if (cs < 0) return false;
+    const int nw = (a.rows + 31) >> 5;
+    int* rl = reinterpret_cast<int*>(lds) + 2 * nw;
+    float* xl = reinterpret_cast<float*>(rl + a.rows);
+    auto whole = [&](const int2 r) {
+        const int item = r.x, first = r.y >> 7, n = r.y & 127;
+        const size_t o0 = (size_t)item * a.ldw + min(tid, a.ldw - 1);
+        float pw = 0.f, pm = 0.f, pv = 0.f;
+        if (upd) {
+            pw = a.W[o0];
+            if (!s.is_sgd) { pm = a.M[o0]; pv = a.V[o0]; }
+        }
+        if (tid < n) { const int2 e = a.ent[first + tid]; rl[tid] = e.x; xl[tid] = __int_as_float(e.y); }
+        __syncthreads();
+        w1_item_sum_update(a, lds, item, n, s, upd, pw, pm, pv);
+    };
+    if (!four) {
+        for (int u = vblock; u < cs + cb; u += vgrid) whole(u == u0 && u < cs ? rec0 : a.rec[u < cs ? u : a.lcap - 1 - (u - cs)]);
+        return true;
+    }
+    for (int b = vblock; b < cb; b += vgrid) whole(a.rec[a.lcap - 1 - b]);
+    int* rs = reinterpret_cast<int*>(lds) + wv * 2 * kW1HybRows;
+    float* xs = reinterpret_cast<float*>(rs + kW1HybRows);
+    for (int u = u0; u < cs; u += 4 * vgrid) {
+        const int2 r = u == u0 ? rec0 : a.rec[u];
+        const int item = r.x, first = r.y >> 7, n = r.y & 127;
+        const size_t o0 = (size_t)item * a.ldw + min(4 * lane, a.ldw - 4);
+        float4 pw = make_float4(0.f, 0.f, 0.f, 0.f), pm = pw, pv = pw;
+        if (upd) {
+            pw = *reinterpret_cast<const float4*>(a.W + o0);
+            if (!s.is_sgd) { pm = *reinterpret_cast<const float4*>(a.M + o0); pv = *reinterpret_cast<const float4*>(a.V + o0); }
+        }
+        if (lane < n) { const int2 e = a.ent[first + lane]; rs[lane] = e.x; xs[lane] = __int_as_float(e.y); }
+        w1_wave_sum_update(a, rs, xs, item, n, s, upd, pw, pm, pv);
+    }
+    return true;
+}
+
 __global__ __launch_bounds__(256) void w1_item_wave_kernel(W1Items a, int* hot, int* hot_count) {
     extern __shared__ unsigned w1w_lds_dyn[];
     w1_item_wave_body(a, hot, hot_count, w1w_lds_dyn, (int)(blockIdx.x * 4 + (threadIdx.x >> 6)), (int)gridDim.x * 4);
diff --git a/include/aaerec_hip.h b/include/aaerec_hip.h
--- a/include/aaerec_hip.h
+++ b/include/aaerec_hip.h
@@ -111,6 +111,7 @@
 int aae_abi_version(void);
 const char* aae_last_error(void);
 int aae_set_option(const char* name, const char* value);
+int aae_debug_item_lists(aae_handle h, int* counts, int* rec, int rec_cap, int* ent, int n_ent, int* cap_out);
 
 int aae_arena_bytes(const aae_config* cfg, size_t* bytes_out);
 int aae_create(const aae_config* cfg, void* arena_dev, size_t arena_bytes, void* stream,
```

Measured after the change: 441,400 docs/s (median of 6 runs). Within noise of the previous version (+0.7%).
